# imjaegyun/super_resolution

Measured on AMD Instinct MI355X. Metric: SR output megapixels/sec, HAT-S x4, 1280x720 LR in, higher is better.
Workload: dtype bf16; 1 GPU; HAT-S x4, one 3x720x1280 LR frame per GPU, full-frame forward; upscale=4, parallelism=dp1

## Files before the change

include/hat_mi355x.h:

```cpp
#ifndef HAT_MI355X_H
#define HAT_MI355X_H

#include <stdint.h>

#ifdef __cplusplus
extern "C" {
#endif

#define HAT_ABI_VERSION 2

enum { HAT_F32 = 0, HAT_BF16 = 1 };
enum { HAT_EINVAL = -1, HAT_ELDS = -2, HAT_EUNSUPPORTED = -3 };

enum { HAT_ACT_NONE = 0, HAT_ACT_GELU = 1 , HAT_ACT_LRELU = 2 ,
       HAT_ACT_LRELU02 = 3  };
enum { HAT_X_NHWC_T = 0, HAT_X_NHWC_F32 = 1, HAT_X_NCHW_F32_MEAN = 2 };
enum { HAT_O_NHWC_T = 0, HAT_O_NHWC_F32 = 1, HAT_O_PIXSHUF_T = 2, HAT_O_NCHW_F32 = 3 };

typedef struct HatConvDesc {
    const void* x;
    const void* x0;
    const void* w;
    const float* bias;
    void* out;
// ... 21 lines not shown
    float* gap_out;
    void* n16_out;
    int32_t gap_c;
    int32_t reserved0;
} HatConvDesc;

int hat_conv_occupancy(const HatConvDesc* d, int32_t* wgs_per_cu);
int hat_conv_tiles(const HatConvDesc* d, int32_t* tiles_out);
int hat_conv_plan(const HatConvDesc* d, int32_t* waves, int32_t* rows_per_wave, int32_t* tiles, int64_t* lds_bytes);
int hat_conv(const HatConvDesc* d, void* stream);

int hat_linear(const HatConvDesc* d, void* stream);

int hat_conv3x3_small_groups(const HatConvDesc* d, int32_t* groups_out);
int hat_conv3x3_small(const HatConvDesc* d, void* stream);

typedef struct HatCabFoldDesc {
    const void* c1;
    const float* c1_colsum;
    const float* w2;
    const float* b2;
    const float* wk;
    const float* bias_in;
    float* scale;
    void* wf;
    float* bias_out;
    float* tmp;
    int32_t B, H, W, C, mid, ld1, tiles, ldcs, k, ld_scale, dtype;
    float conv_scale;
    const float* stats;
    const float* w2f;
} HatCabFoldDesc;
int hat_cab_fold(const HatCabFoldDesc* d, void* stream);

typedef struct HatAggrCabDesc {
    HatConvDesc lin;
    const void* c1;
    const void* wf;
    const float* bias_b;
} HatAggrCabDesc;
int hat_aggr_cab(const HatAggrCabDesc* d, void* stream);

int hat_layernorm_blocks(void);
int hat_layernorm(const float* x, void* y, const float* gamma, const float* beta, float* gap_partial,
                  int32_t B, int64_t npix, int32_t C, int32_t ldy, int32_t out_f32, int32_t gap_c,
                  int32_t dtype, void* stream);

int hat_add_f32(const float* a, const float* c, float* out, int32_t B, int64_t n, int64_t c_bstride, void* stream);

int hat_esc_weights(const float* gap_partial, int32_t nblk, int64_t npix, const float* w1, const float* b1,
                    const float* w2, const float* b2, const float* plk_packed, void* w_out, int32_t B,
                    int32_t pdim, int32_t ksize, int32_t Kpad, int32_t dtype, void* stream);

int hat_esc_conv13(const void* x, int32_t ldx, const void* wp, int32_t Kpad, void* y16, int32_t B, int32_t H, int32_t W,
                   int32_t dtype, void* stream);

int hat_eca_scale(const float* colsum, int32_t tiles, int32_t ldc, int64_t npix, const float* wk, int32_t k,
                  float conv_scale, float* tmp, float* scale, int32_t B, int32_t C, void* stream);

int hat_dwconv_gate(const void* u, const float* wdw, const float* bdw, void* out, int32_t B, int32_t H,
                    int32_t W, int32_t hid, int32_t ldu, int32_t ldo, int32_t dtype, void* stream);

typedef struct HatMlpDesc {
    const void* x;
    const void* w1f;
    const float* b1;
    const void* w2f;
    const float* b2;
    const float* r1;
    void* out;
    int32_t B, H, W, C, hidden;
    int32_t ldx, ldr1, ldo;
    int32_t out_f32, dtype;
} HatMlpDesc;
int hat_ocab_mlp(const HatMlpDesc* d, void* stream);
int hat_ocab_qkv(const HatMlpDesc* d, void* stream);

int hat_ocab_keybias(const void* sal, int32_t ldsal, const void* kv, int32_t ldkv, float* kb, int32_t B, int32_t H, int32_t W,
                     int32_t C, int32_t ws, int32_t wse, int32_t pad, int32_t k_keep, int32_t dtype, void* stream);
int hat_ocab_attention_kb(const void* q, const void* kv, const float* bias_rot, const float* kb, void* out, int32_t B, int32_t H,
                          int32_t W, int32_t C, int32_t heads, int32_t ws, int32_t wse, int32_t pad, int32_t ldq, int32_t ldkv,
                          int32_t ldo, int32_t dtype, void* stream);

int hat_sgfn_gate(const void* u, const float* wdw, const float* bdw, void* out, int32_t B, int32_t H, int32_t W,
                  int32_t half, int32_t ldu, int32_t ldo, int32_t dtype, void* stream);

int hat_ocab_attention(const void* q, const void* kv, const float* bias_rot, void* out, int32_t B, int32_t H,
                       int32_t W, int32_t C, int32_t heads, int32_t ws, int32_t wse, int32_t ldq,
// ... 96 lines not shown
    float* gap_out;
    int32_t B, H, W, C;
    int32_t chunks;
    int32_t ldn, gap_c;
    int32_t dtype;
    int32_t ldm_in;
    const void* m_in;
    void* n16_out;
} HatFfnDesc;

int hat_ffn_tiles(const HatFfnDesc* d, int32_t* tiles_out);
int hat_ffn(const HatFfnDesc* d, void* stream);

int hat_ffn2(const HatFfnDesc* d, void* stream);

typedef struct HatHabTailDesc {
    HatFfnDesc ffn;
    const void* n;
    const void* y16;
    const void* c1;
    const void* w_aggr;
    const void* wf;
    const float* bias_b;
    int32_t ldn_in;
    int32_t ldr2;
    const void* r2;
    const float* r2scale;
    int32_t r2scale_bstride;
    int32_t reserved1;
} HatHabTailDesc;
int hat_hab_tail(const HatHabTailDesc* d, void* stream);

int hat_hab_tail3(const HatHabTailDesc* d, void* stream);

typedef struct hat_plan hat_plan;
int hat_plan_load(const char* path, hat_plan** out);
int hat_plan_info(const hat_plan* plan, int32_t* dims8, int64_t* n_calls, int64_t* device_bytes);
int hat_plan_forward(const hat_plan* plan, const float* x, float* y, void* stream);
void hat_plan_free(hat_plan* plan);
int hat_plan_forward_u8(const hat_plan* plan, const uint8_t* src, int64_t src_pitch, int32_t h, int32_t w, uint8_t* dst,
                        int64_t dst_pitch, int32_t flags, void* stream);
int hat_plan_forward_yuv420(const hat_plan* plan, const uint8_t* src_y, int64_t src_y_pitch, int64_t src_y_bstride, const uint8_t* src_cb,
                            const uint8_t* src_cr, int64_t src_c_pitch, int32_t src_c_step, int64_t src_c_bstride, int32_t h, int32_t w,
                            uint8_t* dst_y, int64_t dst_y_pitch, int64_t dst_y_bstride, uint8_t* dst_cb, uint8_t* dst_cr, int64_t dst_c_pitch,
                            int32_t dst_c_step, int64_t dst_c_bstride, const float* to_rgb12, const float* from_rgb12, void* stream);
int hat_plan_forward_yuv420_deep(const hat_plan* plan, const void* src_y, int64_t src_y_pitch, int64_t src_y_bstride, const void* src_cb,
                                 const void* src_cr, int64_t src_c_pitch, int32_t src_c_step, int64_t src_c_bstride, int32_t src_depth,
                                 int32_t src_msb, int32_t h, int32_t w, void* dst_y, int64_t dst_y_pitch, int64_t dst_y_bstride, void* dst_cb,
                                 void* dst_cr, int64_t dst_c_pitch, int32_t dst_c_step, int64_t dst_c_bstride, int32_t dst_depth,
                                 int32_t dst_msb, const float* to_rgb12, const float* from_rgb12, void* stream);
int hat_plan_forward_yuv(const hat_plan* plan, const HatYuvSurface* src, const HatYuvSurface* dst, int32_t h, int32_t w,
                         const float* to_rgb12, const float* from_rgb12, void* stream);
int hat_plan_forward_yuv_sited(const hat_plan* plan, const HatYuvSurface* src, int32_t src_siting, const HatYuvSurface* dst,
                               int32_t dst_siting, int32_t h, int32_t w, const float* to_rgb12, const float* from_rgb12, void* stream);

int hat_rect_sum(const void* x, int32_t dtype, int32_t ld, int32_t C, int32_t W, int32_t r0, int32_t r1, int32_t c0, int32_t c1,
                 int64_t bstride, int32_t B, float* out, int32_t ldo, float* tmp, uint32_t* counter, void* stream);

int hat_dihedral_f32(const float* src, float* dst, int32_t planes, int32_t H, int32_t W, int32_t op, int32_t inverse, float alpha,
                     int32_t accumulate, void* stream);

int hat_abi_version(void);
const char* hat_target_arch(void);

int hat_niqe_workspace_bytes(int32_t B, int32_t h, int32_t w, int32_t crop_border, int32_t* H96, int32_t* W96, int64_t* bytes);
int hat_niqe_y_u8(const uint8_t* src, int64_t pitch, int64_t bstride, int32_t B, int32_t h, int32_t w, int32_t crop_border, int32_t bgr,
// ... 79 lines not shown
```

super_resolution_amd/_lib.py:

```python
from __future__ import annotations

import ctypes as C
import os
import threading

_HERE = os.path.dirname(os.path.abspath(__file__))
LIB_PATH = os.environ.get("HAT_MI355X_LIB") or os.path.join(_HERE, "libhat_mi355x.so")

ABI_VERSION = 2
HAT_F32, HAT_BF16 = 0, 1
ACT_NONE, ACT_GELU, ACT_LRELU, ACT_LRELU02 = 0, 1, 2, 3
X_NHWC_T, X_NHWC_F32, X_NCHW_F32_MEAN = 0, 1, 2
O_NHWC_T, O_NHWC_F32, O_PIXSHUF_T, O_NCHW_F32 = 0, 1, 2, 3
METRICS_Y, METRICS_BGR, METRICS_PSNR, METRICS_SSIM = 1, 2, 4, 8

_ERRORS = {-1: "HAT_EINVAL (bad argument)", -2: "HAT_ELDS (tile does not fit in 160 KiB LDS)",
           -3: "HAT_EUNSUPPORTED (shape not instantiated)"}


class HatConvDesc(C.Structure):
    _fields_ = [
        ("x", C.c_void_p), ("x0", C.c_void_p), ("w", C.c_void_p), ("bias", C.c_void_p),
        ("out", C.c_void_p), ("r1", C.c_void_p), ("r2", C.c_void_p), ("r2scale", C.c_void_p), ("colsum", C.c_void_p),
        ("B", C.c_int32), ("H", C.c_int32), ("W", C.c_int32),
# ... 21 lines not shown
        ("r1", C.c_void_p), ("out", C.c_void_p),
        ("B", C.c_int32), ("H", C.c_int32), ("W", C.c_int32), ("C", C.c_int32), ("hidden", C.c_int32),
        ("ldx", C.c_int32), ("ldr1", C.c_int32), ("ldo", C.c_int32),
        ("out_f32", C.c_int32), ("dtype", C.c_int32),
    ]


class HatFfnDesc(C.Structure):
    _fields_ = [
        ("t_in", C.c_void_p), ("t_out", C.c_void_p), ("ln_g", C.c_void_p), ("ln_b", C.c_void_p),
        ("w1f", C.c_void_p), ("b1", C.c_void_p), ("dww", C.c_void_p), ("dwb", C.c_void_p),
        ("w2f", C.c_void_p), ("b2", C.c_void_p), ("ln1_g", C.c_void_p), ("ln1_b", C.c_void_p),
        ("n_out", C.c_void_p), ("gap_out", C.c_void_p),
        ("B", C.c_int32), ("H", C.c_int32), ("W", C.c_int32), ("C", C.c_int32),
        ("chunks", C.c_int32), ("ldn", C.c_int32), ("gap_c", C.c_int32), ("dtype", C.c_int32),
        ("ldm_in", C.c_int32), ("m_in", C.c_void_p), ("n16_out", C.c_void_p),
    ]


class HatHabTailDesc(C.Structure):
    _fields_ = [("ffn", HatFfnDesc), ("n", C.c_void_p), ("y16", C.c_void_p), ("c1", C.c_void_p), ("w_aggr", C.c_void_p),
                ("wf", C.c_void_p), ("bias_b", C.c_void_p), ("ldn_in", C.c_int32), ("ldr2", C.c_int32), ("r2", C.c_void_p),
                ("r2scale", C.c_void_p), ("r2scale_bstride", C.c_int32), ("reserved1", C.c_int32)]


class HatCabFoldDesc(C.Structure):
    _fields_ = [
        ("c1", C.c_void_p), ("c1_colsum", C.c_void_p), ("w2", C.c_void_p), ("b2", C.c_void_p), ("wk", C.c_void_p),
        ("bias_in", C.c_void_p), ("scale", C.c_void_p), ("wf", C.c_void_p), ("bias_out", C.c_void_p), ("tmp", C.c_void_p),
        ("B", C.c_int32), ("H", C.c_int32), ("W", C.c_int32), ("C", C.c_int32), ("mid", C.c_int32), ("ld1", C.c_int32),
        ("tiles", C.c_int32), ("ldcs", C.c_int32), ("k", C.c_int32), ("ld_scale", C.c_int32), ("dtype", C.c_int32),
        ("conv_scale", C.c_float), ("stats", C.c_void_p), ("w2f", C.c_void_p),
    ]


class HatAggrCabDesc(C.Structure):
    _fields_ = [("lin", HatConvDesc), ("c1", C.c_void_p), ("wf", C.c_void_p), ("bias_b", C.c_void_p)]


class HatYuvSurface(C.Structure):
    _fields_ = [("y", C.c_void_p), ("y_pitch", C.c_int64), ("y_bstride", C.c_int64), ("cb", C.c_void_p), ("cr", C.c_void_p),
                ("c_pitch", C.c_int64), ("c_step", C.c_int32), ("c_bstride", C.c_int64),
                ("sub_x", C.c_int32), ("sub_y", C.c_int32), ("depth", C.c_int32), ("msb", C.c_int32)]


class HatNafHalfDesc(C.Structure):
    _fields_ = [("r_in", C.c_void_p), ("gprev", C.c_void_p), ("wf", C.c_void_p), ("bf", C.c_void_p), ("r_out", C.c_void_p),
                ("w1", C.c_void_p), ("b1", C.c_void_p), ("dww", C.c_void_p), ("dwb", C.c_void_p), ("g_out", C.c_void_p),
                ("partials", C.c_void_p), ("wf_bstride", C.c_int64), ("bf_bstride", C.c_int32),
                ("B", C.c_int32), ("H", C.c_int32), ("W", C.c_int32), ("C", C.c_int32), ("ldr", C.c_int32), ("ldg", C.c_int32),
                ("ldo", C.c_int32), ("dtype", C.c_int32), ("reserved0", C.c_int32)]


class HatNafFoldDesc(C.Structure):
    _fields_ = [("partials", C.c_void_p), ("wsca", C.c_void_p), ("bsca", C.c_void_p), ("w2", C.c_void_p), ("b2", C.c_void_p),
                ("beta", C.c_void_p), ("wf", C.c_void_p), ("bf", C.c_void_p), ("npix", C.c_int64),
                ("B", C.c_int32), ("tiles", C.c_int32), ("C", C.c_int32), ("dtype", C.c_int32)]


class HatEscConvFfnDesc(C.Structure):
    _fields_ = [("x", C.c_void_p), ("ln_g", C.c_void_p), ("ln_b", C.c_void_p), ("w1", C.c_void_p), ("b1", C.c_void_p),
                ("dww", C.c_void_p), ("dwb", C.c_void_p), ("w2", C.c_void_p), ("b2", C.c_void_p), ("r", C.c_void_p),
                ("out", C.c_void_p), ("partials", C.c_void_p), ("ln_eps", C.c_float),
                ("B", C.c_int32), ("H", C.c_int32), ("W", C.c_int32), ("hid_p", C.c_int32), ("ldx", C.c_int32), ("ldr", C.c_int32),
                ("ldo", C.c_int32), ("out_f32", C.c_int32), ("dtype", C.c_int32), ("reserved0", C.c_int32)]


_YUV_BLOCK = [C.c_void_p, C.c_int64, C.c_int64, C.c_void_p, C.c_void_p, C.c_int64, C.c_int32, C.c_int64]

SIGNATURES = {
    "hat_abi_version": (C.c_int, []),
    "hat_target_arch": (C.c_char_p, []),
    "hat_conv_tiles": (C.c_int, [C.POINTER(HatConvDesc), C.POINTER(C.c_int32)]),
    "hat_ocab_mlp": (C.c_int, [C.POINTER(HatMlpDesc), C.c_void_p]),
    "hat_ocab_qkv": (C.c_int, [C.POINTER(HatMlpDesc), C.c_void_p]),
    "hat_conv_occupancy": (C.c_int, [C.POINTER(HatConvDesc), C.POINTER(C.c_int32)]),
    "hat_conv_plan": (C.c_int, [C.POINTER(HatConvDesc), C.POINTER(C.c_int32), C.POINTER(C.c_int32), C.POINTER(C.c_int32),
                                C.POINTER(C.c_int64)]),
    "hat_conv": (C.c_int, [C.POINTER(HatConvDesc), C.c_void_p]),
    "hat_linear": (C.c_int, [C.POINTER(HatConvDesc), C.c_void_p]),
    "hat_conv3x3_small_groups": (C.c_int, [C.POINTER(HatConvDesc), C.POINTER(C.c_int32)]),
    "hat_conv3x3_small": (C.c_int, [C.POINTER(HatConvDesc), C.c_void_p]),
    "hat_cab_fold": (C.c_int, [C.POINTER(HatCabFoldDesc), C.c_void_p]),
    "hat_aggr_cab": (C.c_int, [C.POINTER(HatAggrCabDesc), C.c_void_p]),
    "hat_ffn_tiles": (C.c_int, [C.POINTER(HatFfnDesc), C.POINTER(C.c_int32)]),
    "hat_ffn": (C.c_int, [C.POINTER(HatFfnDesc), C.c_void_p]),
    "hat_ffn2": (C.c_int, [C.POINTER(HatFfnDesc), C.c_void_p]),
    "hat_hab_tail": (C.c_int, [C.POINTER(HatHabTailDesc), C.c_void_p]),
    "hat_hab_tail3": (C.c_int, [C.POINTER(HatHabTailDesc), C.c_void_p]),
    "hat_plan_load": (C.c_int, [C.c_char_p, C.POINTER(C.c_void_p)]),
    "hat_plan_info": (C.c_int, [C.c_void_p, C.POINTER(C.c_int32), C.POINTER(C.c_int64), C.POINTER(C.c_int64)]),
    "hat_plan_forward": (C.c_int, [C.c_void_p, C.c_void_p, C.c_void_p, C.c_void_p]),
    "hat_plan_free": (None, [C.c_void_p]),
    "hat_layernorm_blocks": (C.c_int, []),
    "hat_layernorm": (C.c_int, [C.c_void_p, C.c_void_p, C.c_void_p, C.c_void_p, C.c_void_p, C.c_int32, C.c_int64,
                                C.c_int32, C.c_int32, C.c_int32, C.c_int32, C.c_int32, C.c_void_p]),
    "hat_rect_sum": (C.c_int, [C.c_void_p, C.c_int32, C.c_int32, C.c_int32, C.c_int32, C.c_int32, C.c_int32, C.c_int32, C.c_int32,
                               C.c_int64, C.c_int32, C.c_void_p, C.c_int32, C.c_void_p, C.c_void_p, C.c_void_p]),
    "hat_add_f32": (C.c_int, [C.c_void_p, C.c_void_p, C.c_void_p, C.c_int32, C.c_int64, C.c_int64, C.c_void_p]),
    "hat_esc_weights": (C.c_int, [C.c_void_p, C.c_int32, C.c_int64, C.c_void_p, C.c_void_p, C.c_void_p, C.c_void_p,
                                  C.c_void_p, C.c_void_p, C.c_int32, C.c_int32, C.c_int32, C.c_int32, C.c_int32, C.c_void_p]),
    "hat_esc_conv13": (C.c_int, [C.c_void_p, C.c_int32, C.c_void_p, C.c_int32, C.c_void_p, C.c_int32, C.c_int32, C.c_int32, C.c_int32, C.c_void_p]),
    "hat_eca_scale": (C.c_int, [C.c_void_p, C.c_int32, C.c_int32, C.c_int64, C.c_void_p, C.c_int32, C.c_float,
                                C.c_void_p, C.c_void_p, C.c_int32, C.c_int32, C.c_void_p]),
    "hat_dwconv_gate": (C.c_int, [C.c_void_p, C.c_void_p, C.c_void_p, C.c_void_p, C.c_int32, C.c_int32, C.c_int32,
                                  C.c_int32, C.c_int32, C.c_int32, C.c_int32, C.c_void_p]),
    "hat_ocab_keybias": (C.c_int, [C.c_void_p, C.c_int32, C.c_void_p, C.c_int32, C.c_void_p] + [C.c_int32] * 9 + [C.c_void_p]),
    "hat_ocab_attention_kb": (C.c_int, [C.c_void_p] * 5 + [C.c_int32] * 12 + [C.c_void_p]),
    "hat_sgfn_gate": (C.c_int, [C.c_void_p, C.c_void_p, C.c_void_p, C.c_void_p, C.c_int32, C.c_int32, C.c_int32,
                                C.c_int32, C.c_int32, C.c_int32, C.c_int32, C.c_void_p]),
    "hat_ocab_attention": (C.c_int, [C.c_void_p, C.c_void_p, C.c_void_p, C.c_void_p, C.c_int32, C.c_int32, C.c_int32,
                                     C.c_int32, C.c_int32, C.c_int32, C.c_int32, C.c_int32, C.c_int32, C.c_int32,
                                     C.c_int32, C.c_void_p]),
    "hat_ocab_attention_log2": (C.c_int, [C.c_void_p, C.c_void_p, C.c_void_p, C.c_void_p, C.c_int32, C.c_int32, C.c_int32,
                                     C.c_int32, C.c_int32, C.c_int32, C.c_int32, C.c_int32, C.c_int32, C.c_int32,
                                     C.c_int32, C.c_void_p]),
    "hat_cab_squeeze_units": (C.c_int, [C.c_int32, C.c_int32, C.c_void_p, C.c_void_p]),
    "hat_cab_squeeze": (C.c_int, [C.c_void_p, C.c_void_p, C.c_void_p, C.c_void_p, C.c_void_p, C.c_int32, C.c_int32, C.c_int32,
                                  C.c_int32, C.c_int32, C.c_int32, C.c_void_p]),
    "hat_conv3x3_to_planes": (C.c_int, [C.c_void_p, C.c_void_p, C.c_void_p, C.c_void_p, C.c_int32, C.c_int32, C.c_int32, C.c_int32,
                                        C.c_int32, C.c_int32, C.c_float, C.c_void_p, C.c_int32, C.c_void_p]),
    "hat_u8_to_planes": (C.c_int, [C.c_void_p, C.c_int64, C.c_int64, C.c_void_p, C.c_int32, C.c_int32, C.c_int32, C.c_int32, C.c_int32,
# ... 103 lines not shown
```

super_resolution_amd/build.py:

```python
from __future__ import annotations

import os
import subprocess
import sys
from concurrent.futures import ThreadPoolExecutor

HERE = os.path.dirname(os.path.abspath(__file__))
CSRC = os.path.join(HERE, "csrc")
LIB = os.path.join(HERE, "libhat_mi355x.so")
SOURCES = ["hat_conv.hip", "hat_conv64r.hip", "hat_attn.hip", "hat_misc.hip", "hat_ffn.hip", "hat_ffn2.hip", "hat_tail3.hip", "hat_tail3l.hip", "hat_pw.hip", "hat_mlp.hip", "hat_cabsq.hip", "hat_esc13.hip", "hat_u8.hip", "hat_yuv.hip", "hat_resize.hip", "hat_metrics.hip", "hat_dihedral.hip", "hat_niqe.hip", "hat_naf.hip", "hat_esc.hip", "hat_escreal.hip", "hat_plan.cpp"]
HEADERS = [os.path.join(CSRC, "hat_common.h"), os.path.join(CSRC, "hat_yuv_check.h"), os.path.join(os.path.dirname(HERE), "include", "hat_mi355x.h")]
FLAGS = ["-O3", "--offload-arch=gfx950", "-fPIC", "-std=c++17", "-Wall", "-Wno-unused-function"]


def _hipcc() -> str:
    for c in (os.environ.get("HIPCC"), "/opt/rocm/bin/hipcc", "hipcc"):
        if c and (os.path.isabs(c) and os.path.exists(c) or not os.path.isabs(c)):
            return c
    raise RuntimeError("hipcc not found")


def _stale(target: str, deps) -> bool:
    if not os.path.exists(target):
        return True
    t = os.path.getmtime(target)
    return any(os.path.getmtime(d) > t for d in deps)


def build(force: bool = False, verbose: bool = True) -> str:
    hipcc = _hipcc()
    objs, jobs = [], []
    for src in SOURCES:
        s = os.path.join(CSRC, src)
        o = os.path.join(CSRC, os.path.splitext(src)[0] + ".o")
        objs.append(o)
        if force or _stale(o, [s] + HEADERS):
            jobs.append([hipcc, *FLAGS, "-c", s, "-o", o])

    def run(cmd):
        if verbose:
            print(" ".join(cmd), flush=True)
        r = subprocess.run(cmd, capture_output=True, text=True)
        if r.returncode != 0:
            raise RuntimeError(f"hipcc failed:\n{' '.join(cmd)}\n{r.stdout}\n{r.stderr}")
# ... 13 lines not shown
```

super_resolution_amd/csrc/hat_cabsq.hip:

```cpp
#include <cstdlib>
#include <type_traits>

#include "hat_common.h"
#include "hat_yuv_check.h"

__device__ __attribute__((aligned(16))) unsigned hat_cabsq_zero_page[80] = {};

namespace {

struct SweepEpi { float out_scale; float mean[4]; int nst; };
struct SweepEpiU8 { float out_scale; float mean[4]; int h_out, w_out, bgr; long long pitch, bstride; };
template <int SX, int SY, bool GREY> struct SweepEpiYUVT {
    float out_scale; float mean[4]; int h_out, w_out, c_step; long long pitch, bstride, c_pitch, c_bstride;
    uint8_t* cb; uint8_t* cr; HatCsc k;
};
template <int SX, int SY, bool GREY> struct SweepEpiYUV16T {
    float out_scale; float mean[4]; int h_out, w_out, c_step; long long pitch, bstride, c_pitch, c_bstride;
    uint8_t* cb; uint8_t* cr; HatCsc k; int shift; float scale, maxcode;
};
using SweepEpiYUV = SweepEpiYUVT<1, 1, false>;
using SweepEpiYUV16 = SweepEpiYUV16T<1, 1, false>;
template <typename E> struct SweepYuvTraits { static constexpr bool yuv = false, deep = false, grey = false; static constexpr int sx = 1, sy = 1; };
template <int SX, int SY, bool G> struct SweepYuvTraits<SweepEpiYUVT<SX, SY, G>> {
    static constexpr bool yuv = true, deep = false, grey = G; static constexpr int sx = SX, sy = SY;
};
template <int SX, int SY, bool G> struct SweepYuvTraits<SweepEpiYUV16T<SX, SY, G>> {
    static constexpr bool yuv = true, deep = true, grey = G; static constexpr int sx = SX, sy = SY;
};

template <int KS, bool NCHW, typename Epi = SweepEpi>
__global__ __launch_bounds__(256, KS > 2 ? 2 : 3) void cab_squeeze_kernel(const bf16_t* __restrict__ x, const bf16_t* __restrict__ wpk,
                                                             const float* __restrict__ bias, void* __restrict__ outv,
                                                             float* __restrict__ colsum, int H, int W, int C, int ldx,
                                                             int rows, int strips, int units, Epi epi) {
    constexpr bool U8 = std::is_same<Epi, SweepEpiU8>::value;
    using YT = SweepYuvTraits<Epi>;
    constexpr bool YUV16 = YT::deep, YUV = YT::yuv;
    constexpr bool C420 = YUV && !YT::grey && YT::sx == 1 && YT::sy == 1, C422 = YUV && !YT::grey && YT::sx == 1 && YT::sy == 0;
    constexpr bool C444 = YUV && !YT::grey && YT::sx == 0;
    static_assert((!U8 && !YUV) || NCHW, "the byte epilogues convert the conv_last value");
    using M = MT<bf16_t>;
    using frag_t = M::frag_t;
    const int lane = threadIdx.x & 63, wave = threadIdx.x >> 6, g = lane >> 4, c16 = lane & 15;
    const int u = blockIdx.x * 4 + wave;
    const int b = blockIdx.y;
    if (u >= units) return;
    const int band = u / strips, strip = u - band * strips;
    const int x0 = strip * 14 - 1, y0 = band * rows, y1 = min(y0 + rows, H);
    const bf16_t* xb = x + (size_t)b * H * W * ldx;
    bf16_t* ob = reinterpret_cast<bf16_t*>(outv) + (size_t)b * H * W * 8;
    float* of = nullptr;
    uint8_t* o8 = nullptr;
    if constexpr (U8 || YUV) o8 = reinterpret_cast<uint8_t*>(outv) + (size_t)b * epi.bstride;
    else of = reinterpret_cast<float*>(outv) + (size_t)b * epi.nst * H * W;
    [[maybe_unused]] float ctop_b = 0.f, ctop_r = 0.f;

    frag_t A[6][KS];
#pragma unroll
    for (int t = 0; t < 6; ++t)
#pragma unroll
        for (int ks = 0; ks < KS; ++ks) A[t][ks] = M::load(wpk + ((size_t)(t * KS + ks) * 64 + lane) * 8);
    const f32x4 bs = *reinterpret_cast<const f32x4*>(bias + 4 * (g & 1));

    const int xx = x0 + c16;
    const bool xin = xx >= 0 && xx < W;
    const bf16_t* cbase = xin ? xb + (size_t)xx * ldx : reinterpret_cast<const bf16_t*>(hat_cabsq_zero_page);
    const unsigned cstride = xin ? (unsigned)W * (unsigned)ldx : 0u;
// ... 107 lines not shown
                }
            } else if constexpr (NCHW) {
#pragma unroll
                for (int i = 0; i < 4; ++i)
                    if (4 * g + i < epi.nst) of[((size_t)(4 * g + i) * H + y) * W + xx] = v[i] * epi.out_scale + epi.mean[(4 * g + i) & 3];
            } else {
#pragma unroll
                for (int i = 0; i < 4; ++i) v[i] = gelu_erf_fast(v[i]);
                Vec4<bf16_t>::store(ob + ((size_t)y * W + xx) * 8 + 4 * g, v);
                csum += as_stored<bf16_t>(v);
            }
        }
        S2 = f32x4{0.f, 0.f, 0.f, 0.f};
#pragma unroll
        for (int i = 0; i < 4; ++i) S0[i] = g < 2 ? S0[i] : 0.f;
    };

#pragma unroll
    for (int nb = 0; nb < NB; ++nb) load_row(y0 - 1 + nb, Bc[nb]);
    for (int r = y0 - 1; r <= y1; r += 3) {
        step(r, ring[1], ring[2], ring[0], Bc[0]);
        step(r + 1, ring[2], ring[0], ring[1], Bc[1]);
        step(r + 2, ring[0], ring[1], ring[2], Bc[2]);
    }
    if (!NCHW && colsum != nullptr) {
#pragma unroll
        for (int i = 0; i < 4; ++i) {
            const float s = row_sum16(csum[i]);
            if (c16 == 0) colsum[((size_t)b * units + u) * 16 + 4 * g + i] = g < 2 ? s : 0.f;
        }
    }
}

}

static int sweep_units(int H, int W, int slots, int* rows_out, int* units_out, bool even_rows = false) {
    const int strips = (W + 13) / 14;
    int bands = slots / strips;
    bands = bands < 1 ? 1 : bands;
    int rows = (H + bands - 1) / bands;
    rows = rows < 8 ? 8 : rows;
    if (even_rows) rows += rows & 1;
    *rows_out = rows;
    *units_out = strips * ((H + rows - 1) / rows);
    return 0;
}

extern "C" int hat_cab_squeeze_units(int32_t H, int32_t W, int32_t* rows_out, int32_t* units_out) {
    if (H < 1 || W < 16 || W % 16 || !rows_out || !units_out) return HAT_EINVAL;
    static const int slots = [] { const char* e = getenv("HAT_SQUEEZE_SLOTS"); const int v = e ? atoi(e) : 0; return v >= 256 ? v : 2048; }();
    return sweep_units(H, W, slots, rows_out, units_out);
}

extern "C" int hat_cab_squeeze(const void* x, const void* wpk, const float* bias, void* out, float* colsum, int32_t B,
                               int32_t H, int32_t W, int32_t C, int32_t ldx, int32_t dtype, void* stream) {
    if (!x || !wpk || !bias || !out || B < 1 || H < 1) return HAT_EINVAL;
    if (dtype != HAT_BF16) return HAT_EUNSUPPORTED;
    if (C % 8 || C > 160 || C <= 128 || ldx < C || ldx % 8) return HAT_EUNSUPPORTED;
    if ((reinterpret_cast<uintptr_t>(x) | reinterpret_cast<uintptr_t>(wpk)) % 16 || reinterpret_cast<uintptr_t>(out) % 8) return HAT_EINVAL;
    int32_t rows = 0, units = 0;
    const int rc = hat_cab_squeeze_units(H, W, &rows, &units);
    if (rc) return rc;
    HAT_LAUNCH((cab_squeeze_kernel<5, false>), dim3((units + 3) / 4, B), dim3(256), 0, reinterpret_cast<hipStream_t>(stream),
               reinterpret_cast<const bf16_t*>(x), reinterpret_cast<const bf16_t*>(wpk), bias, out, colsum, H, W, C, ldx, rows,
               (W + 13) / 14, units, SweepEpi{1.0f, {0.f, 0.f, 0.f, 0.f}, 8});
    return hat_check_launch();
}

extern "C" int hat_conv3x3_to_planes(const void* x, const void* wpk, const float* bias, float* out, int32_t B, int32_t H,
                                     int32_t W, int32_t C, int32_t ldx, int32_t n_out, float out_scale, const float* mean4,
                                     int32_t dtype, void* stream) {
    if (!x || !wpk || !bias || !out || !mean4 || B < 1 || H < 1 || W < 16 || W % 16 || n_out < 1 || n_out > 8) return HAT_EINVAL;
    if (dtype != HAT_BF16) return HAT_EUNSUPPORTED;
    if (C != 64 || ldx < C || ldx % 8) return HAT_EUNSUPPORTED;
    if ((reinterpret_cast<uintptr_t>(x) | reinterpret_cast<uintptr_t>(wpk)) % 16) return HAT_EINVAL;
    int rows = 0, units = 0;
    sweep_units(H, W, 3072, &rows, &units);
    HAT_LAUNCH((cab_squeeze_kernel<2, true>), dim3((units + 3) / 4, B), dim3(256), 0, reinterpret_cast<hipStream_t>(stream),
               reinterpret_cast<const bf16_t*>(x), reinterpret_cast<const bf16_t*>(wpk), bias, out, nullptr, H, W, C, ldx, rows,
               (W + 13) / 14, units, SweepEpi{out_scale, {mean4[0], mean4[1], mean4[2], mean4[3]}, n_out});
    return hat_check_launch();
}

extern "C" int hat_conv3x3_to_u8(const void* x, const void* wpk, const float* bias, uint8_t* dst, int64_t dst_pitch, int64_t dst_bstride,
                                 int32_t B, int32_t H, int32_t W, int32_t C, int32_t ldx, int32_t h_out, int32_t w_out, float out_scale,
                                 const float* mean4, int32_t bgr, int32_t dtype, void* stream) {
    if (!x || !wpk || !bias || !dst || !mean4 || B < 1 || H < 1 || W < 16 || W % 16 || h_out < 1 || w_out < 1 || h_out > H || w_out > W)
        return HAT_EINVAL;
    if (dst_pitch < 3 * (int64_t)w_out || (B > 1 && dst_bstride < dst_pitch * (int64_t)(h_out - 1) + 3 * (int64_t)w_out)) return HAT_EINVAL;
    if (dtype != HAT_BF16) return HAT_EUNSUPPORTED;
    if (C != 64 || ldx < C || ldx % 8) return HAT_EUNSUPPORTED;
    if ((reinterpret_cast<uintptr_t>(x) | reinterpret_cast<uintptr_t>(wpk)) % 16) return HAT_EINVAL;
    int rows = 0, units = 0;
    sweep_units(H, W, 3072, &rows, &units);
    HAT_LAUNCH((cab_squeeze_kernel<2, true, SweepEpiU8>), dim3((units + 3) / 4, B), dim3(256), 0, reinterpret_cast<hipStream_t>(stream),
               reinterpret_cast<const bf16_t*>(x), reinterpret_cast<const bf16_t*>(wpk), bias, dst, nullptr, H, W, C, ldx, rows, (W + 13) / 14, units,
               SweepEpiU8{out_scale, {mean4[0], mean4[1], mean4[2], mean4[3]}, h_out, w_out, bgr ? 1 : 0, (long long)dst_pitch,
                          (long long)dst_bstride});
// ... 80 lines not shown
```

super_resolution_amd/csrc/hat_esc13.hip:

```cpp
#include <cstdlib>

#include "hat_common.h"

namespace {

constexpr int E_TR = 32, E_TC = 32, E_HALO = 6;
constexpr int E_HR = E_TR + 2 * E_HALO, E_HC = E_TC + 2 * E_HALO;
constexpr int E_NFRAG = 7 * 13;
constexpr int E_X_OFF = E_NFRAG * 1024;
constexpr int E_LDS = E_X_OFF + E_HR * E_HC * 32 + 64;

__device__ __attribute__((aligned(16))) unsigned hat_esc13_zero_page[4] = {0, 0, 0, 0};

template <int RW>
__global__ __launch_bounds__((E_TR / RW) * 64) void esc13_kernel(const bf16_t* __restrict__ x, int ldx, const bf16_t* __restrict__ wp, int Kpad,
                                                             bf16_t* __restrict__ y16, int H, int W, int tiles_x, int ntiles) {
    typedef __bf16 bf8 __attribute__((ext_vector_type(8)));
    constexpr int E_WAVES = E_TR / RW;
    extern __shared__ __attribute__((aligned(16))) char smem[];
    typedef __attribute__((address_space(3))) char lds_char;
    const unsigned lds0 = (unsigned)(uintptr_t)(lds_char*)smem;
    const int tid = threadIdx.x, lane = tid & 63, g = lane >> 4, c16 = lane & 15;
    const int wave = __builtin_amdgcn_readfirstlane(tid >> 6);
    const int b = blockIdx.y;
    const bf16_t* xb = x + (size_t)b * H * W * ldx;
    bf16_t* yb = y16 + (size_t)b * H * W * 16;
    {
        const bf16_t* wrow = wp + ((size_t)b * 16 + c16) * Kpad;
        for (int s = wave; s < E_NFRAG; s += E_WAVES) {
            const int dxp = s / 13, dy = s - 13 * dxp, dx = 2 * dxp + (g >> 1);
            const char* src = dx <= 12 ? reinterpret_cast<const char*>(wrow + (dy * 13 + dx) * 16 + 8 * (g & 1))
                                       : reinterpret_cast<const char*>(hat_esc13_zero_page);
            __builtin_amdgcn_global_load_lds((const __attribute__((address_space(1))) void*)src,
                                             (__attribute__((address_space(3))) void*)(smem + s * 1024), 16, 0, 0);
        }
        if (tid < 4) *reinterpret_cast<u32x4*>(smem + E_LDS - 64 + tid * 16) = u32x4{0u, 0u, 0u, 0u};
    }
    const int r0 = RW * wave;
    unsigned xbase = lds0 + E_X_OFF + (unsigned)((r0 * E_HC + c16 + (g >> 1)) * 32 + (g & 1) * 16);
    unsigned abase = lds0 + (unsigned)lane * 16u, abase1 = abase + 60u * 1024u;
    asm volatile("" : "+v"(xbase), "+v"(abase), "+v"(abase1));

    constexpr int NPIECE = E_HR * E_HC * 2, NIT = (NPIECE + E_WAVES * 64 - 1) / (E_WAVES * 64);
    u32x4 pv[NIT];
    auto fetch = [&](int t) {
        const int tc = min(t, ntiles - 1);
        const int ty0 = (tc / tiles_x) * E_TR, tx0 = (tc - (tc / tiles_x) * tiles_x) * E_TC;
#pragma unroll
        for (int it = 0; it < NIT; ++it) {
            const int i = min(tid + it * E_WAVES * 64, NPIECE - 1);
            const int hp = i >> 1, half = i & 1;
            const int hy = hp / E_HC, hx = hp - hy * E_HC;
            const int y = ty0 - E_HALO + hy, xx = tx0 - E_HALO + hx;
            const bool in = y >= 0 && y < H && xx >= 0 && xx < W;
            const u32x4 v = *reinterpret_cast<const u32x4*>(xb + ((size_t)min(max(y, 0), H - 1) * W + min(max(xx, 0), W - 1)) * ldx + half * 8);
            pv[it] = in ? v : u32x4{0u, 0u, 0u, 0u};
        }
    };
    fetch(blockIdx.x);
    for (int t = blockIdx.x; t < ntiles; t += gridDim.x) {
        const int ty0 = (t / tiles_x) * E_TR, tx0 = (t - (t / tiles_x) * tiles_x) * E_TC;
#pragma unroll
        for (int it = 0; it < NIT; ++it) {
            const int i = tid + it * E_WAVES * 64;
            if (i < NPIECE) *reinterpret_cast<u32x4*>(smem + E_X_OFF + i * 16) = pv[it];
        }
        __syncthreads();
        fetch(t + gridDim.x);

        f32x4 acc[RW][2];
#pragma unroll
        for (int pt = 0; pt < RW; ++pt)
#pragma unroll
            for (int ct = 0; ct < 2; ++ct) acc[pt][ct] = f32x4{0.f, 0.f, 0.f, 0.f};
        auto ldb = [&](int rr, int dxp, int ct) {
            return __builtin_bit_cast(bf8, *(__attribute__((address_space(3))) const u32x4*)(uintptr_t)(xbase + (unsigned)((rr * E_HC) * 32 + dxp * 64 + ct * 512)));
        };
        auto lda = [&](int dxp, int dy) {
            const int sfr = dxp * 13 + dy;
            return __builtin_bit_cast(bf8, *(__attribute__((address_space(3))) const u32x4*)(uintptr_t)(sfr < 60 ? abase + (unsigned)(sfr * 1024) : abase1 + (unsigned)((sfr - 60) * 1024)));
        };
        bf8 rowf[7][RW + 12][2];
        bf8 afr[7][13];
        constexpr int PRE = RW < 2 ? RW : 2;
        afr[0][0] = lda(0, 0);
#pragma unroll
        for (int j = 0; j < PRE; ++j) { rowf[0][j][0] = ldb(j, 0, 0); rowf[0][j][1] = ldb(j, 0, 1); }
#pragma unroll
        for (int dxp = 0; dxp < 7; ++dxp) {
#pragma unroll
            for (int dy = 0; dy < 13; ++dy) {
                if (dy == 0) {
#pragma unroll
                    for (int j = PRE; j < RW; ++j) { rowf[dxp][j][0] = ldb(j, dxp, 0); rowf[dxp][j][1] = ldb(j, dxp, 1); }
                }
                if (dy < 12) {
                    afr[dxp][dy + 1] = lda(dxp, dy + 1);
                    rowf[dxp][dy + RW][0] = ldb(dy + RW, dxp, 0);
                    rowf[dxp][dy + RW][1] = ldb(dy + RW, dxp, 1);
                } else if (dxp < 6) {
                    afr[dxp + 1][0] = lda(dxp + 1, 0);
#pragma unroll
                    for (int j = 0; j < PRE; ++j) { rowf[dxp + 1][j][0] = ldb(j, dxp + 1, 0); rowf[dxp + 1][j][1] = ldb(j, dxp + 1, 1); }
                }
#pragma unroll
                for (int j = 0; j < RW; ++j)
#pragma unroll
                    for (int ct = 0; ct < 2; ++ct)
                        acc[j][ct] = __builtin_amdgcn_mfma_f32_16x16x32_bf16(afr[dxp][dy], rowf[dxp][dy + j][ct], acc[j][ct], 0, 0, 0);
                __builtin_amdgcn_sched_barrier(0);
            }
        }
#pragma unroll
        for (int pt = 0; pt < RW; ++pt)
#pragma unroll
            for (int ct = 0; ct < 2; ++ct) {
                const int y = ty0 + r0 + pt, xx = tx0 + ct * 16 + c16;
                if (y < H && xx < W) Vec4<bf16_t>::store(yb + ((size_t)y * W + xx) * 16 + 4 * g, acc[pt][ct]);
            }
        __syncthreads();
    }
}

}

extern "C" int hat_esc_conv13(const void* x, int32_t ldx, const void* wp, int32_t Kpad, void* y16, int32_t B, int32_t H, int32_t W,
                              int32_t dtype, void* stream) {
    if (!x || !wp || !y16 || B < 1 || H < 1 || W < 1 || ldx < 16 || ldx % 8 || Kpad < 169 * 16 || Kpad % 8) return HAT_EINVAL;
    if (dtype != HAT_BF16) return HAT_EUNSUPPORTED;
    const int tiles_x = (W + E_TC - 1) / E_TC, tiles_y = (H + E_TR - 1) / E_TR, ntiles = tiles_x * tiles_y;
    int gx = 256 / (B < 2 ? 1 : (B < 4 ? 2 : 4));
    if (gx > ntiles) gx = ntiles;
    static const int rw = [] { const char* e = getenv("HAT_ESC13_RW"); return e && atoi(e) == 2 ? 2 : 4; }();
    auto launch = [&](auto kern, int waves) -> int {
        hipError_t e = hipFuncSetAttribute(reinterpret_cast<const void*>(kern), hipFuncAttributeMaxDynamicSharedMemorySize, E_LDS);
        if (e != hipSuccess) return (int)e;
        HAT_LAUNCH(kern, dim3(gx, B), dim3(waves * 64), E_LDS, reinterpret_cast<hipStream_t>(stream), reinterpret_cast<const bf16_t*>(x), ldx,
                   reinterpret_cast<const bf16_t*>(wp), Kpad, reinterpret_cast<bf16_t*>(y16), H, W, tiles_x, ntiles);
        return hat_check_launch();
    };
    return rw == 2 ? launch(esc13_kernel<2>, 16) : launch(esc13_kernel<4>, 8);
}
```

super_resolution_amd/csrc/hat_misc.hip:

```cpp
#include "hat_common.h"

namespace {

constexpr int LN_BLOCKS = 1024;

template <typename OutT, int NV>
__global__ __launch_bounds__(256) void ln_kernel(const float* __restrict__ x, OutT* __restrict__ y,
                                                 const float* __restrict__ gamma, const float* __restrict__ beta,
                                                 float* __restrict__ gap_partial, long npix, int C, int ldy, int gap_c) {
    __shared__ float red[16][32];
    const int tid = threadIdx.x, j = tid & 15, grp = tid >> 4;
    const int b = blockIdx.y;
    const float* xb = x + (size_t)b * npix * C;
    OutT* yb = y + (size_t)b * npix * ldy;
    f32x4 gm[NV], bt[NV];
#pragma unroll
    for (int v = 0; v < NV; ++v) {
        const int c = 4 * j + 64 * v;
        gm[v] = f32x4{0.f, 0.f, 0.f, 0.f};
        bt[v] = gm[v];
        if (c < C) {
            gm[v] = *reinterpret_cast<const f32x4*>(gamma + c);
            bt[v] = *reinterpret_cast<const f32x4*>(beta + c);
        }
    }
    f32x4 gsum = {0.f, 0.f, 0.f, 0.f};
    const float invC = 1.0f / (float)C;
    for (long p0 = (long)blockIdx.x * 16; p0 < npix; p0 += (long)gridDim.x * 16) {
        const long p = p0 + grp;
        const bool pv = p < npix;
        f32x4 xv[NV];
        float s = 0.f;
#pragma unroll
// ... 102 lines not shown
        for (int k = 0; k < np; ++k) s += part[k * gs + tid];
        pmean[tid] = s * inv_npix;
    }
    __syncthreads();
    const int hdim = pdim / 2;
    if (tid < hdim) {
        float s = b1[tid];
        for (int ci = 0; ci < pdim; ++ci) s += w1[tid * pdim + ci] * pmean[ci];
        hid[tid] = gelu_erf(s);
    }
    __syncthreads();
    if (tid < 9) {
        const int t = co * 9 + tid;
        float s = b2[t];
        for (int m = 0; m < hdim; ++m) s += w2[t * hdim + m] * hid[m];
        dk[tid] = s;
    }
    __syncthreads();
    const int cin_p = (pdim + 7) & ~7;
    const int ctr = ksize / 2;
    const float* src = plk + (size_t)co * Kpad;
    T* dst = w_out + ((size_t)b * npad + co) * Kpad;
    for (int k = tid; k < Kpad; k += 1024) {
        float v = src[k];
        const int tap = k / cin_p, ci = k - tap * cin_p;
        if (ci == co && tap < ksize * ksize) {
            const int dy = tap / ksize - ctr, dx = tap % ksize - ctr;
            if (dy >= -1 && dy <= 1 && dx >= -1 && dx <= 1) v += dk[(dy + 1) * 3 + (dx + 1)];
        }
        dst[k] = to_T<T>(v);
    }
}

__global__ __launch_bounds__(256) void eca_reduce_kernel(const float* __restrict__ colsum, int tiles, int ldc,
                                                         float* __restrict__ tmp) {
    __shared__ float sub[256];
    int lw = 1;
    while (lw < ldc) lw <<= 1;
    const int nsub = 256 / lw;
    const int c = threadIdx.x % lw, sb = threadIdx.x / lw, part = blockIdx.x, b = blockIdx.y;
    const int per = (tiles + 31) / 32;
    const int t0 = part * per, t1 = min(tiles, t0 + per);
    float a[8] = {0.f, 0.f, 0.f, 0.f, 0.f, 0.f, 0.f, 0.f};
    if (c < ldc && t1 > t0) {
        for (int t = t0 + sb; t < t1; t += 8 * nsub) {
#pragma unroll
            for (int u = 0; u < 8; ++u) {
                const int tt = t + u * nsub;
                const float v = colsum[((size_t)b * tiles + min(tt, t1 - 1)) * ldc + c];
                a[u] += tt < t1 ? v : 0.f;
            }
        }
    }
    sub[threadIdx.x] = ((a[0] + a[1]) + (a[2] + a[3])) + ((a[4] + a[5]) + (a[6] + a[7]));
    __syncthreads();
    if (sb == 0 && c < ldc) {
        float s = 0.f;
        for (int i = 0; i < nsub; ++i) s += sub[i * lw + c];
        tmp[((size_t)b * 32 + part) * ldc + c] = s;
    }
}

__global__ __launch_bounds__(256) void eca_scale_kernel(const float* __restrict__ tmp, int ldc, float inv_npix,
                                                        const float* __restrict__ wk, int k, float conv_scale,
                                                        float* __restrict__ scale, int C) {
    __shared__ float mean[256];
    const int c = threadIdx.x, b = blockIdx.x;
    float s = 0.f;
    if (c < C) {
        for (int p = 0; p < 32; ++p) s += tmp[((size_t)b * 32 + p) * ldc + c];
    }
    mean[c] = s * inv_npix;
    __syncthreads();
    if (c < C) {
        float e = 0.f;
        for (int j = 0; j < k; ++j) {
            const int cc = c + j - k / 2;
            if (cc >= 0 && cc < C) e += wk[j] * mean[cc];
        }
        scale[(size_t)b * ldc + c] = conv_scale / (1.0f + expf(-e));
    }
}

template <typename T, bool DIRECT>
__global__ __launch_bounds__(256) void cab_fold_kernel(const HatCabFoldDesc d) {
    __shared__ float sm[256 * 5 + 256];
    float* red = sm;
    float (*part)[32] = reinterpret_cast<float (*)[32]>(sm + 256 * 5);
    float* mean = sm;
    float* scl = sm + 256;
    __shared__ float bord[4][8];
    __shared__ float S[9][8];
    const int tid = threadIdx.x, b = blockIdx.x;
    const int H = d.H, W = d.W, C = d.C, mid = d.mid;
    const T* c1 = reinterpret_cast<const T*>(d.c1) + (size_t)b * H * W * d.ld1;
    const float* st = d.stats ? d.stats + (size_t)b * 72 : nullptr;
    if (st != nullptr) {
        if (tid < 32) bord[tid >> 3][tid & 7] = st[8 + tid];
        __syncthreads();
    } else {
        float a[4][8];
#pragma unroll
        for (int line = 0; line < 4; ++line)
#pragma unroll
            for (int c = 0; c < 8; ++c) a[line][c] = 0.f;
        const int lmax = W > H ? W : H;
        constexpr int BU = sizeof(T) == 2 ? 5 : 2;
        for (int i0 = tid; i0 < lmax; i0 += 256 * BU) {
            typename MT<T>::frag_t v[BU][4];
#pragma unroll
            for (int u = 0; u < BU; ++u)
#pragma unroll
                for (int line = 0; line < 4; ++line) {
                    const int len = line < 2 ? W : H;
                    const int i = min(i0 + u * 256, len - 1);
                    const size_t pix = line == 0 ? (size_t)i : line == 1 ? (size_t)(H - 1) * W + i : line == 2 ? (size_t)i * W : (size_t)i * W + (W - 1);
                    v[u][line] = MT<T>::load(c1 + pix * d.ld1);
                }
#pragma unroll
            for (int u = 0; u < BU; ++u)
#pragma unroll
                for (int line = 0; line < 4; ++line) {
                    const bool in = i0 + u * 256 < (line < 2 ? W : H);
#pragma unroll
                    for (int c = 0; c < 8; ++c) a[line][c] += in ? to_f(v[u][line][c]) : 0.f;
                }
        }
#pragma unroll
        for (int pass = 0; pass < 8; ++pass) {
#pragma unroll
            for (int k = 0; k < 4; ++k) red[tid * 5 + k] = a[pass >> 1][(pass & 1) * 4 + k];
            __syncthreads();
            if (tid < 32) {
                const int v4 = tid & 3, pt = tid >> 2;
                float sp = 0.f;
                for (int i = 0; i < 32; ++i) sp += red[(pt * 32 + i) * 5 + v4];
                part[pt][pass * 4 + v4] = sp;
            }
            __syncthreads();
        }
        if (tid < 32) {
            float sp = 0.f;
            for (int i = 0; i < 8; ++i) sp += part[i][tid];
            bord[tid >> 3][tid & 7] = sp;
        }
        __syncthreads();
    }
    if (DIRECT && st == nullptr) {
        const int c = tid & 7, sb = tid >> 3;
        float a[8] = {0.f, 0.f, 0.f, 0.f, 0.f, 0.f, 0.f, 0.f};
        for (int t = sb; t < d.tiles; t += 256) {
#pragma unroll
            for (int u = 0; u < 8; ++u) {
                const int tt = t + 32 * u;
                const float v = d.c1_colsum[((size_t)b * d.tiles + min(tt, d.tiles - 1)) * d.ldcs + c];
                a[u] += tt < d.tiles ? v : 0.f;
            }
        }
        part[c][sb] = ((a[0] + a[1]) + (a[2] + a[3])) + ((a[4] + a[5]) + (a[6] + a[7]));
        __syncthreads();
    }
    if (tid < 72) {
        const int tap = tid >> 3, c = tid & 7;
        const int dy = tap / 3 - 1, dx = tap % 3 - 1;
        float tot = 0.f;
        if (st != nullptr) {
            tot = st[c];
        } else if constexpr (DIRECT) {
            for (int p = 0; p < 32; ++p) tot += part[c][p];
        } else {
            for (int p = 0; p < 32; ++p) tot += d.tmp[((size_t)b * 32 + p) * d.ldcs + c];
        }
        float v = tot;
        const int rl = dy == 1 ? 0 : dy == -1 ? 1 : -1, cl = dx == 1 ? 2 : dx == -1 ? 3 : -1;
        if (rl >= 0) v -= bord[rl][c];
        if (cl >= 0) v -= bord[cl][c];
        if (rl >= 0 && cl >= 0) {
            const size_t pix = (size_t)(rl == 0 ? 0 : H - 1) * W + (cl == 2 ? 0 : W - 1);
            v += st != nullptr ? st[40 + (rl * 2 + (cl - 2)) * 8 + c] : to_f(c1[pix * d.ld1 + c]);
        }
        S[tap][c] = c < mid ? v : 0.f;
    }
    __syncthreads();
    float m = 0.f;
    {
        const int co = tid < C ? tid : C - 1;
        float wv[72];
        if (d.w2f != nullptr) {
            const f32x4* wf4 = reinterpret_cast<const f32x4*>(d.w2f) + (size_t)(co >> 4) * (3 * 64 * 2);
            f32x4 w8[9][2];
#pragma unroll
            for (int tap = 0; tap < 9; ++tap) {
                const int e = ((tap >> 2) * 64 + (tap & 3) * 16 + (co & 15)) * 2;
                w8[tap][0] = wf4[e];
                w8[tap][1] = wf4[e + 1];
            }
#pragma unroll
            for (int q = 0; q < 72; ++q) { const int ci = q / 9, tap = q - ci * 9; wv[q] = w8[tap][ci >> 2][ci & 3]; }
        } else {
#pragma unroll
            for (int q = 0; q < 72; ++q) wv[q] = d.w2[(size_t)co * mid * 9 + min(q, mid * 9 - 1)];
        }
        const float bb = d.b2[co];
#pragma unroll
        for (int q = 0; q < 72; ++q) {
            const int ci = q / 9, tap = q - ci * 9;
            if (q < mid * 9) m += wv[q] * S[tap][ci < 8 ? ci : 7];
        }
        m = tid < C ? m / ((float)H * (float)W) + bb : 0.f;
    }
    mean[tid] = m;
    __syncthreads();
    float sc = 0.f;
    if (tid < C) {
        float e = 0.f;
        for (int j = 0; j < d.k; ++j) {
            const int cc = tid + j - d.k / 2;
            if (cc >= 0 && cc < C) e += d.wk[j] * mean[cc];
        }
        sc = d.conv_scale / (1.0f + expf(-e));
        d.scale[(size_t)b * d.ld_scale + tid] = sc;
    }
    scl[tid] = sc;
    __syncthreads();
    const int nt = (C + 15) / 16;
    for (int n = tid; n < nt * 16; n += 256) d.bias_out[(size_t)b * nt * 16 + n] = n < C ? d.bias_in[n] + scl[n] * d.b2[n] : 0.f;
    T* wf = reinterpret_cast<T*>(d.wf) + (size_t)b * nt * 3 * 512;
    if (d.w2f != nullptr) {
        constexpr int MAXS = 16;
        const int total4 = nt * 3 * 128;
        for (int base = 0; base < total4; base += 256 * MAXS) {
        f32x4 wq[MAXS];
#pragma unroll
        for (int st = 0; st < MAXS; ++st) wq[st] = reinterpret_cast<const f32x4*>(d.w2f)[min(base + tid + st * 256, total4 - 1)];
#pragma unroll
        for (int st = 0; st < MAXS; ++st) {
            const int i4 = base + tid + st * 256;
            if (i4 < total4) {
                const int i = 4 * i4, j = i & 7, lane = (i >> 3) & 63, ks = (i >> 9) % 3, t = i / (3 * 512);
                const int co = t * 16 + (lane & 15), tap = 4 * ks + (lane >> 4);
                const int cov = min(co, C - 1);
                const float sv = scl[cov];
                f32x4 v = wq[st] * f32x4{sv, sv, sv, sv};
                if (co < C && tap == 9 && j == 0) {
                    const float bfull = d.bias_in[cov] + sv * d.b2[cov];
                    v[0] = bfull;
                    v[1] = bfull - to_f(to_T<T>(bfull));
                }
                Vec4<T>::store(wf + i, v);
            }
        }
        }
        return;
    }
    constexpr int FU = 18;
    for (int i0 = tid; i0 < nt * 3 * 512; i0 += 256 * FU) {
        float wv[FU], bi[FU], b2v[FU];
        bool ok[FU];
        int cov[FU], bsel[FU];
#pragma unroll
        for (int u = 0; u < FU; ++u) {
            const int i = min(i0 + u * 256, nt * 3 * 512 - 1);
            const int j = i & 7, lane = (i >> 3) & 63, ks = (i >> 9) % 3, t = i / (3 * 512);
            const int co = t * 16 + (lane & 15), k = 32 * ks + 8 * (lane >> 4) + j;
            const int tap = k >> 3, ci = k & 7;
            ok[u] = co < C && tap < 9 && ci < mid;
            bsel[u] = (co < C && tap == 9 && ci < 2) ? 1 + ci : 0;
            cov[u] = min(co, C - 1);
            wv[u] = d.w2[((size_t)cov[u] * mid + min(ci, mid - 1)) * 9 + min(tap, 8)];
            bi[u] = d.bias_in[cov[u]];
            b2v[u] = d.b2[cov[u]];
        }
#pragma unroll
        for (int u = 0; u < FU; ++u) {
            const int i = i0 + u * 256;
            const float bfull = bi[u] + scl[cov[u]] * b2v[u];
            const float bhead = to_f(to_T<T>(bfull));
            const float v = bsel[u] == 1 ? bfull : (bsel[u] == 2 ? bfull - bhead : (ok[u] ? scl[cov[u]] * wv[u] : 0.f));
            if (i < nt * 3 * 512) wf[i] = to_T<T>(v);
        }
    }
}

template <typename T>
__global__ __launch_bounds__(256) void dwgate_kernel(const T* __restrict__ u, const float* __restrict__ wdw,
                                                     const float* __restrict__ bdw, T* __restrict__ out, int B, int H, int W,
                                                     int hid, int ldu, int ldo) {
    const int gpp = hid / 4;
    const size_t total = (size_t)B * H * W * gpp;
    for (size_t i = (size_t)blockIdx.x * 256 + threadIdx.x; i < total; i += (size_t)gridDim.x * 256) {
        const size_t pix = i / gpp;
        const int c = (int)(i - pix * gpp) * 4;
        const int x = (int)(pix % W);
        const int y = (int)((pix / W) % H);
        f32x4 a = *reinterpret_cast<const f32x4*>(bdw + c);
        f32x4 gt = *reinterpret_cast<const f32x4*>(bdw + hid + c);
#pragma unroll
        for (int dy = -1; dy <= 1; ++dy) {
            const int yy = y + dy;
            if (yy < 0 || yy >= H) continue;
#pragma unroll
            for (int dx = -1; dx <= 1; ++dx) {
                const int xx = x + dx;
                if (xx < 0 || xx >= W) continue;
                const T* up = u + (size_t)((long)pix + (long)dy * W + dx) * ldu;
                const int tap = (dy + 1) * 3 + (dx + 1);
                a += Vec4<T>::load(up + c) * *reinterpret_cast<const f32x4*>(wdw + (size_t)tap * 2 * hid + c);
                gt += Vec4<T>::load(up + hid + c) * *reinterpret_cast<const f32x4*>(wdw + (size_t)tap * 2 * hid + hid + c);
            }
        }
        f32x4 o;
#pragma unroll
        for (int r = 0; r < 4; ++r) o[r] = a[r] * (gt[r] / (1.0f + expf(-gt[r])));
        Vec4<T>::store(out + pix * ldo + c, o);
    }
// ... 34 lines not shown

}

extern "C" int hat_layernorm_blocks(void) { return LN_BLOCKS; }

extern "C" int hat_layernorm(const float* x, void* y, const float* gamma, const float* beta, float* gap_partial,
                             int32_t B, int64_t npix, int32_t C, int32_t ldy, int32_t out_f32, int32_t gap_c,
                             int32_t dtype, void* stream) {
    if (!x || !y || !gamma || !beta || B < 1 || npix < 1 || C < 4 || C % 4 || C > 256 || ldy < C || ldy % 4) return HAT_EINVAL;
    if (gap_c < 0 || gap_c > 32 || gap_c % 4 || (gap_c > 0 && !gap_partial)) return HAT_EINVAL;
    hipStream_t s = reinterpret_cast<hipStream_t>(stream);
    float* gp = gap_c > 0 ? gap_partial : nullptr;
    if (out_f32 || dtype == HAT_F32) return launch_ln<float>(x, y, gamma, beta, gp, B, npix, C, ldy, gap_c, s);
    if (dtype == HAT_BF16) return launch_ln<bf16_t>(x, y, gamma, beta, gp, B, npix, C, ldy, gap_c, s);
    return HAT_EINVAL;
}

extern "C" int hat_esc_weights(const float* gap_partial, int32_t nblk, int64_t npix, const float* w1, const float* b1,
                               const float* w2, const float* b2, const float* plk_packed, void* w_out, int32_t B,
                               int32_t pdim, int32_t ksize, int32_t Kpad, int32_t dtype, void* stream) {
    if (!gap_partial || !w1 || !b1 || !w2 || !b2 || !plk_packed || !w_out) return HAT_EINVAL;
    if (pdim < 2 || pdim > 32 || pdim % 4 || ksize < 3 || (ksize & 1) == 0 || B < 1 || nblk < 1) return HAT_EINVAL;
    hipStream_t s = reinterpret_cast<hipStream_t>(stream);
    dim3 grid(pdim > 16 ? 32 : 16, B), block(1024);
    const float inv = 1.0f / (float)npix;
    if (dtype == HAT_BF16)
        HAT_LAUNCH(esc_weights_kernel<bf16_t>, grid, block, 0, s, gap_partial, nblk, inv, w1, b1, w2, b2, plk_packed,
                           reinterpret_cast<bf16_t*>(w_out), pdim, ksize, Kpad);
    else if (dtype == HAT_F32)
        HAT_LAUNCH(esc_weights_kernel<float>, grid, block, 0, s, gap_partial, nblk, inv, w1, b1, w2, b2, plk_packed,
                           reinterpret_cast<float*>(w_out), pdim, ksize, Kpad);
    else
        return HAT_EINVAL;
    return hat_check_launch();
}

extern "C" int hat_eca_scale(const float* colsum, int32_t tiles, int32_t ldc, int64_t npix, const float* wk, int32_t k,
                             float conv_scale, float* tmp, float* scale, int32_t B, int32_t C, void* stream) {
    if (!colsum || !wk || !tmp || !scale || tiles < 1 || ldc < C || ldc > 256 || C < 1 || k < 1 || (k & 1) == 0 || B < 1) return HAT_EINVAL;
    hipStream_t s = reinterpret_cast<hipStream_t>(stream);
    HAT_LAUNCH(eca_reduce_kernel, dim3(32, B), dim3(256), 0, s, colsum, tiles, ldc, tmp);
    int rc = hat_check_launch();
    if (rc) return rc;
    HAT_LAUNCH(eca_scale_kernel, dim3(B), dim3(256), 0, s, tmp, ldc, 1.0f / (float)npix, wk, k, conv_scale, scale, C);
    return hat_check_launch();
}

extern "C" int hat_cab_fold(const HatCabFoldDesc* dp, void* stream) {
    if (!dp) return HAT_EINVAL;
    const HatCabFoldDesc& d = *dp;
    if (!d.w2 || !d.b2 || !d.wk || !d.bias_in || !d.scale || !d.wf || !d.bias_out) return HAT_EINVAL;
    if (!d.stats && (!d.c1 || !d.c1_colsum || !d.tmp)) return HAT_EINVAL;
    if (d.B < 1 || d.H < 2 || d.W < 2 || d.C < 1 || d.C > 256 || d.mid < 1 || d.mid > 8 || d.ld1 != 8 || d.tiles < 1 || d.ldcs < 8 ||
        d.ldcs > 256 || d.k < 1 || (d.k & 1) == 0 || d.ld_scale < d.C)
        return HAT_EINVAL;
    hipStream_t s = reinterpret_cast<hipStream_t>(stream);
    if (d.dtype != HAT_BF16 && d.dtype != HAT_F32) return HAT_EINVAL;
    if (d.tiles <= 2048 || d.stats) {
        if (d.dtype == HAT_BF16) HAT_LAUNCH((cab_fold_kernel<bf16_t, true>), dim3(d.B), dim3(256), 0, s, d);
        else HAT_LAUNCH((cab_fold_kernel<float, true>), dim3(d.B), dim3(256), 0, s, d);
        return hat_check_launch();
    }
    HAT_LAUNCH(eca_reduce_kernel, dim3(32, d.B), dim3(256), 0, s, d.c1_colsum, d.tiles, d.ldcs, d.tmp);
    int rc = hat_check_launch();
    if (rc) return rc;
    if (d.dtype == HAT_BF16) HAT_LAUNCH((cab_fold_kernel<bf16_t, false>), dim3(d.B), dim3(256), 0, s, d);
// ... 130 lines not shown
```

super_resolution_amd/csrc/hat_plan.cpp:

```cpp
#include <hip/hip_runtime.h>
#include <stdint.h>
#include <stdio.h>
#include <string.h>

#include <string>
#include <vector>

#include "../../include/hat_mi355x.h"
#include "hat_yuv_check.h"

namespace {

enum : uint32_t { ARG_INT = 0, ARG_FLOAT = 1, ARG_PTR = 2, ARG_STRUCT = 3, ARG_HOST = 4, ARG_STREAM = 5 };
enum : uint32_t { BUF_CONST = 0, BUF_SCRATCH = 1, BUF_INPUT = 2, BUF_OUTPUT = 3 };
constexpr uint32_t NULL_BUF = 0xFFFFFFFFu;

struct Fix { uint32_t field_off, buf; uint64_t off; };
struct Arg {
    uint32_t tag = 0;
    int64_t i = 0;
    double f = 0;
    uint32_t buf = NULL_BUF;
    uint64_t off = 0;
    std::vector<unsigned char> blob;
    std::vector<Fix> fix;
};
struct Call { uint32_t fn; std::vector<Arg> args; };
struct Buf { uint32_t kind; uint64_t nbytes; void* dev = nullptr; };

}

struct hat_plan {
    int32_t dims[8];
    std::vector<Buf> bufs;
    std::vector<Call> calls;
    int device = -1;
    mutable float* stage_in = nullptr;
    mutable float* stage_out = nullptr;
};

namespace {

struct Reader {
    FILE* f;
    bool ok = true;
    template <typename T> T get() { T v{}; if (fread(&v, sizeof(T), 1, f) != 1) ok = false; return v; }
    void bytes(void* p, size_t n) { if (n && fread(p, 1, n, f) != n) ok = false; }
};

const char* const FN_NAMES[] = {"hat_conv", "hat_linear", "hat_conv3x3_small", "hat_cab_fold", "hat_aggr_cab", "hat_ffn", "hat_ffn2",
                                "hat_hab_tail", "hat_layernorm", "hat_esc_weights", "hat_eca_scale", "hat_dwconv_gate", "hat_sgfn_gate",
                                "hat_ocab_attention", "hat_window_attention", "hat_cab_squeeze", "hat_conv3x3_to_planes", "hat_add_f32", "hat_esc_conv13", "hat_ocab_keybias", "hat_ocab_attention_kb", "hat_ocab_mlp", "hat_ocab_qkv", "hat_hab_tail3", "hat_ocab_attention_log2", "hat_naf_half",
                                "hat_naf_fold"};
constexpr uint32_t N_FN = sizeof(FN_NAMES) / sizeof(FN_NAMES[0]);

struct Resolved {
    const hat_plan* p;
    const Call* c;
    const void* x;
    void* y;
    void* stream;
    std::vector<std::vector<unsigned char>> tmp;
    void* ptr(uint32_t buf, uint64_t off) const {
        if (buf == NULL_BUF) return nullptr;
        const Buf& b = p->bufs[buf];
        char* base = b.kind == BUF_INPUT ? (char*)const_cast<void*>(x) : (b.kind == BUF_OUTPUT ? (char*)y : (char*)b.dev);
        return base + off;
    }
    int32_t I(size_t k) const { return (int32_t)c->args[k].i; }
    int64_t L(size_t k) const { return c->args[k].i; }
    float F(size_t k) const { return (float)c->args[k].f; }
    void* P(size_t k) {
        const Arg& a = c->args[k];
        if (a.tag == ARG_PTR) return ptr(a.buf, a.off);
        if (a.tag == ARG_STREAM) return stream;
        if (a.tag == ARG_STRUCT || a.tag == ARG_HOST) {
            tmp.emplace_back(a.blob);
            for (const Fix& fx : a.fix) {
                void* v = ptr(fx.buf, fx.off);
                memcpy(tmp.back().data() + fx.field_off, &v, sizeof(void*));
            }
            return tmp.back().data();
        }
        return nullptr;
    }
};
// ... 34 lines not shown
                                                r.I(11), r.I(12), r.I(13), r.I(14), r.P(15))
                           : HAT_EINVAL;
        case 14:
            return n == 16 ? hat_window_attention(r.P(0), r.P(1), (const float*)r.P(2), r.P(3), r.I(4), r.I(5), r.I(6), r.I(7), r.I(8), r.I(9), r.I(10),
                                                  r.I(11), r.I(12), r.I(13), r.I(14), r.P(15))
                           : HAT_EINVAL;
        case 15:
            return n == 12 ? hat_cab_squeeze(r.P(0), r.P(1), (const float*)r.P(2), r.P(3), (float*)r.P(4), r.I(5), r.I(6), r.I(7), r.I(8), r.I(9), r.I(10),
                                             r.P(11))
                           : HAT_EINVAL;
        case 16:
            return n == 14 ? hat_conv3x3_to_planes(r.P(0), r.P(1), (const float*)r.P(2), (float*)r.P(3), r.I(4), r.I(5), r.I(6), r.I(7), r.I(8), r.I(9),
                                                   r.F(10), (const float*)r.P(11), r.I(12), r.P(13))
                           : HAT_EINVAL;
        case 17: return n == 7 ? hat_add_f32((const float*)r.P(0), (const float*)r.P(1), (float*)r.P(2), r.I(3), r.L(4), r.L(5), r.P(6)) : HAT_EINVAL;
        case 18: return n == 10 ? hat_esc_conv13(r.P(0), r.I(1), r.P(2), r.I(3), r.P(4), r.I(5), r.I(6), r.I(7), r.I(8), r.P(9)) : HAT_EINVAL;
        case 19:
            return n == 15 ? hat_ocab_keybias(r.P(0), r.I(1), r.P(2), r.I(3), (float*)r.P(4), r.I(5), r.I(6), r.I(7), r.I(8), r.I(9), r.I(10), r.I(11), r.I(12),
                                              r.I(13), r.P(14))
                           : HAT_EINVAL;
        case 20:
            return n == 18 ? hat_ocab_attention_kb(r.P(0), r.P(1), (const float*)r.P(2), (const float*)r.P(3), r.P(4), r.I(5), r.I(6), r.I(7), r.I(8), r.I(9),
                                                   r.I(10), r.I(11), r.I(12), r.I(13), r.I(14), r.I(15), r.I(16), r.P(17))
                           : HAT_EINVAL;
        case 21: return n == 2 ? hat_ocab_mlp((const HatMlpDesc*)r.P(0), r.P(1)) : HAT_EINVAL;
        case 22: return n == 2 ? hat_ocab_qkv((const HatMlpDesc*)r.P(0), r.P(1)) : HAT_EINVAL;
        case 23: return n == 2 ? hat_hab_tail3((const HatHabTailDesc*)r.P(0), r.P(1)) : HAT_EINVAL;
        case 24:
            return n == 16 ? hat_ocab_attention_log2(r.P(0), r.P(1), (const float*)r.P(2), r.P(3), r.I(4), r.I(5), r.I(6), r.I(7), r.I(8), r.I(9), r.I(10),
                                                     r.I(11), r.I(12), r.I(13), r.I(14), r.P(15))
                           : HAT_EINVAL;
        case 25: return n == 2 ? hat_naf_half((const HatNafHalfDesc*)r.P(0), r.P(1)) : HAT_EINVAL;
        case 26: return n == 2 ? hat_naf_fold((const HatNafFoldDesc*)r.P(0), r.P(1)) : HAT_EINVAL;
        default: return HAT_EUNSUPPORTED;
    }
}

}

extern "C" void hat_plan_free(hat_plan* p) {
    if (!p) return;
    for (Buf& b : p->bufs)
        if (b.dev) (void)hipFree(b.dev);
    if (p->stage_in) (void)hipFree(p->stage_in);
    if (p->stage_out) (void)hipFree(p->stage_out);
    delete p;
}

static int plan_load_impl(const char* path, hat_plan** out);

extern "C" int hat_plan_load(const char* path, hat_plan** out) {
    if (!path || !out) return HAT_EINVAL;
    *out = nullptr;
    try {
        return plan_load_impl(path, out);
    } catch (...) {
        return HAT_EINVAL;
    }
}

namespace {
constexpr uint64_t MAX_BUF_BYTES = 1ull << 38;
bool ptr_ok(const std::vector<Buf>& bufs, uint32_t buf, uint64_t off) {
    if (buf == NULL_BUF) return true;
    return buf < bufs.size() && off <= bufs[buf].nbytes;
}
// ... 251 lines not shown
```

super_resolution_amd/csrc/hat_tail3.hip:

```cpp
#include "hat_common.h"

#ifndef T3_ISSUE_ALL
#define T3_ISSUE_ALL 0
#endif
#ifndef T3_APF
#define T3_APF 1
#endif
#ifndef T3_S0RD
#define T3_S0RD 8
#endif
#ifndef T3_ABL
#define T3_ABL 0
#endif
#ifndef T3_USTORE_IL
#define T3_USTORE_IL 1
#endif
#ifndef T3_DMA_LATE
#define T3_DMA_LATE 0
#endif

namespace {

typedef _Float16 h2 __attribute__((ext_vector_type(2)));
typedef _Float16 h8 __attribute__((ext_vector_type(8)));
typedef __bf16 bf8 __attribute__((ext_vector_type(8)));

constexpr int T3_C = 144, T3_NT = 9, T3_KS = 5, T3_WAVES = 4, T3_ROWS = 8, T3_HW = 18;
constexpr int T3_NPH = (T3_ROWS + 2) * T3_HW;
constexpr int T3_US_ROWB = 160;
constexpr int T3_W1_OFF = T3_NPH * T3_US_ROWB;
constexpr int T3_W1_BYTES = 4 * T3_KS * 1024;
constexpr int T3_W2_OFF = T3_W1_OFF + 2 * T3_W1_BYTES;
constexpr int T3_WD_OFF = T3_W2_OFF + T3_NT * 1024;
constexpr int T3_WD_REC = 2048;
constexpr int T3_LDS = T3_WD_OFF + T3_WD_REC;
constexpr int T3_B2_OFF = 73728;

typedef __attribute__((address_space(3))) char lds_char;

__device__ __forceinline__ u32x4 lds_rd16(unsigned addr) { return *(__attribute__((address_space(3))) const u32x4*)(uintptr_t)addr; }
__device__ __forceinline__ h2 as_h2(unsigned v) { return __builtin_bit_cast(h2, v); }
__device__ __forceinline__ unsigned as_u(h2 v) { return __builtin_bit_cast(unsigned, v); }
__device__ __forceinline__ void dma1k(const char* src, unsigned lane_off, char* dst) {
    __builtin_amdgcn_global_load_lds((const __attribute__((address_space(1))) void*)(src + lane_off),
                                     (__attribute__((address_space(3))) void*)dst, 16, 0, 0);
}

struct T3Aggr {
    const bf16_t* n;
    const bf16_t* y16;
    const bf16_t* c1;
    const char* wl;
    const char* wf;
    const float* bias_b;
    int ldn;
};
__device__ __attribute__((aligned(16))) unsigned hat_tail3_zero_page[4] = {0, 0, 0, 0};
__device__ __attribute__((aligned(16))) unsigned hat_tail3_ones_page[4] = {0x3F803F80u, 0, 0, 0};

template <int DBG, int TH = 0>
__global__ __launch_bounds__(256, 2) void tail3_kernel(const HatFfnDesc d, const T3Aggr ag) {
    constexpr int C = T3_C, NT = T3_NT, KS = T3_KS, NPH = T3_NPH, HALO_W = T3_HW;
    extern __shared__ __attribute__((aligned(16))) char smem[];
    const unsigned lds0 = (unsigned)(uintptr_t)(lds_char*)smem;

    const int tid = threadIdx.x, lane = tid & 63, g = lane >> 4, c16 = lane & 15;
    const int wave = __builtin_amdgcn_readfirstlane(tid >> 6);
    const int b = blockIdx.z, x0 = blockIdx.x * 16, y0 = blockIdx.y * T3_ROWS;
    const int H = d.H, W = d.W;
    const float* tin = d.t_in + (size_t)b * H * W * C;
    const _Float16* tinh = reinterpret_cast<const _Float16*>(d.t_in) + (size_t)b * H * W * C;

    long long tph[12] = {0, 0, 0, 0, 0, 0, 0, 0, 0, 0, 0, 0};
    long long tlast = 0;
    auto stamp = [&](int slot) {
        if constexpr (DBG & 64) {
            const long long now = (long long)__builtin_amdgcn_s_memtime();
            tph[slot] += now - tlast;
            tlast = now;
        }
    };
    if constexpr (DBG & 64) tlast = (long long)__builtin_amdgcn_s_memtime();

    const char* w1g = reinterpret_cast<const char*>(d.w1f);
    const char* w2g = reinterpret_cast<const char*>(d.w2f);
    const char* wdg = reinterpret_cast<const char*>(d.dww);
    const unsigned lane16 = (unsigned)lane * 16u;
    auto dma_fc1 = [&](int chunk, int buf) {
#pragma unroll
        for (int j = 0; j < 5; ++j) {
            const int f = wave * 5 + j;
            dma1k(w1g + ((size_t)chunk * T3_W1_BYTES + f * 1024), lane16, smem + T3_W1_OFF + buf * T3_W1_BYTES + f * 1024);
        }
    };
// ... 356 lines not shown
#pragma unroll
                    for (int nt = 2; nt + 1 < NT; nt += 2) store_pair_bf16_if(nout, nt * 16, g, lnv(nt), lnv(nt + 1), valid);
                    if (valid) Vec4<bf16_t>::store(nout + (NT - 1) * 16 + 4 * g, lnv(NT - 1));
                } else if (valid) {
                    Vec4<bf16_t>::store(nout + 4 * g, o0);
#pragma unroll
                    for (int nt = 1; nt < NT; ++nt) Vec4<bf16_t>::store(nout + nt * 16 + 4 * g, lnv(nt));
                }
            }
        }
    }
    if constexpr (DBG & 64) {
        stamp(7);
        if (lane == 0) {
            const size_t wg = ((size_t)blockIdx.z * gridDim.y + blockIdx.y) * gridDim.x + blockIdx.x;
            for (int i = 0; i < 12; ++i) d.gap_out[(wg * T3_WAVES + wave) * 12 + i] = (float)tph[i];
        }
        return;
    }
    if (do_ln && d.gap_out != nullptr) {
        float* red = reinterpret_cast<float*>(smem + T3_WD_OFF);
#pragma unroll
        for (int r = 0; r < 4; ++r) {
            float s = gapv[r];
            s = row_sum16(s);
            if (c16 == 0) red[wave * 16 + 4 * g + r] = s;
        }
        __syncthreads();
        if (tid < 16) {
            float s = 0.f;
#pragma unroll
            for (int w = 0; w < T3_WAVES; ++w) s += red[w * 16 + tid];
            const size_t tile = (size_t)blockIdx.y * gridDim.x + blockIdx.x;
            d.gap_out[((size_t)b * gridDim.x * gridDim.y + tile) * 16 + tid] = tid < d.gap_c ? s : 0.f;
        }
    }
}

}

#ifndef HAT_TAIL3_NO_ENTRY
int hat_tail3_launch_c180(const HatHabTailDesc& h, void* stream);

extern "C" int hat_hab_tail3(const HatHabTailDesc* dp, void* stream) {
    if (!dp) return HAT_EINVAL;
    const HatHabTailDesc& h = *dp;
    const HatFfnDesc& d = h.ffn;
    if (!d.t_in || !d.t_out || d.t_in == d.t_out || !d.w1f || !d.dww || !d.w2f || !d.b2) return HAT_EINVAL;
    if (d.B < 1 || d.H < 1 || d.W < 1 || d.chunks < 1 || d.m_in) return HAT_EINVAL;
    if (d.dtype != HAT_BF16) return HAT_EUNSUPPORTED;
    if (d.C == 180) return (d.chunks == 12 && h.reserved1 == 0) ? hat_tail3_launch_c180(h, stream) : HAT_EINVAL;
    if (d.C != T3_C) return HAT_EUNSUPPORTED;
    if (d.ln1_g && (!d.ln1_b || !d.n_out || d.ldn < d.C || d.ldn % 4 || d.gap_c < 0 || d.gap_c > 16 || d.gap_c % 4)) return HAT_EINVAL;
    if (!h.n || !h.y16 || !h.c1 || !h.w_aggr || !h.wf || !h.bias_b || h.ldn_in < T3_C || h.ldn_in % 8) return HAT_EINVAL;
    const T3Aggr ag{reinterpret_cast<const bf16_t*>(h.n), reinterpret_cast<const bf16_t*>(h.y16), reinterpret_cast<const bf16_t*>(h.c1),
                    reinterpret_cast<const char*>(h.w_aggr), reinterpret_cast<const char*>(h.wf), h.bias_b, h.ldn_in};
    const int th = h.reserved1 & 3;
    if ((h.reserved1 & ~3) != 0) return HAT_EINVAL;
    if ((th & 1) && reinterpret_cast<uintptr_t>(d.t_in) % 8) return HAT_EINVAL;
    if ((th & 2) && reinterpret_cast<uintptr_t>(d.t_out) % 16) return HAT_EINVAL;
    void (*kern)(const HatFfnDesc, const T3Aggr) = th == 0 ? tail3_kernel<0, 0> : th == 1 ? tail3_kernel<0, 1> : th == 2 ? tail3_kernel<0, 2> : tail3_kernel<0, 3>;
    hipError_t e = hipFuncSetAttribute(reinterpret_cast<const void*>(kern), hipFuncAttributeMaxDynamicSharedMemorySize, T3_LDS);
    if (e != hipSuccess) return (int)e;
    dim3 grid((d.W + 15) / 16, (d.H + T3_ROWS - 1) / T3_ROWS, d.B);
    HAT_LAUNCH(kern, grid, dim3(256), T3_LDS, reinterpret_cast<hipStream_t>(stream), d, ag);
    return hat_check_launch();
}
#endif
```

super_resolution_amd/engine.py:

```python
from __future__ import annotations

import collections
import dataclasses
import math
import os
import threading
from typing import Dict, Optional

import torch

from . import ops
from .ops import (ACT_GELU, ACT_LRELU, ACT_NONE, O_NCHW_F32, O_NHWC_F32, O_NHWC_T, O_PIXSHUF_T, X_NCHW_F32_MEAN, X_NHWC_F32, X_NHWC_T)

RGB_MEAN = (0.4488, 0.4371, 0.4040)


def _r8(x: int) -> int:
    return (x + 7) // 8 * 8


def _r4(x: int) -> int:
    return (x + 3) // 4 * 4


@dataclasses.dataclass(frozen=True)
class Options:
    no_n16: bool = False
    no_t16: bool = False
    emu_t16: Optional[torch.dtype] = None
    no_fused_ffn: bool = False
    ffn_v1: bool = False
    no_hab_tail: bool = False
    tail_v2: bool = False
    no_cab_fold: bool = False
    no_cab_sweep: bool = False
    no_esc13: bool = False
    esc_side: bool = False
    one_stream: bool = False
    no_attn_log2: bool = False
    no_ocab_mlp: bool = False
    no_ocab_qkv: bool = False
    no_bf16_conv_in: bool = False
    no_conv_ln: bool = False

    @classmethod
    def from_env(cls, env=None) -> "Options":
        env = os.environ if env is None else env
        get = lambda name: env.get("HAT_" + name.upper(), "")
        any_value = ("no_cab_fold", "no_cab_sweep", "no_ocab_mlp", "no_ocab_qkv", "no_bf16_conv_in", "no_conv_ln")
        kw = {k.name: (get(k.name) != "" if k.name in any_value else get(k.name) == "1") for k in dataclasses.fields(cls)}
        return cls(**dict(kw, emu_t16={"fp16": torch.float16, "bf16": torch.bfloat16}.get(get("emu_t16"))))


class _ESC:

    def __init__(self, sd, core: str, plk_key: str, pdim: int, ksize: int, C: int, dtype: int, dev):
        f32 = dict(dtype=torch.float32, device=dev)
        self.pdim, self.ksize = pdim, ksize
        self.w1 = sd[core + ".plk.dwc_proj.1.weight"].detach().reshape(pdim // 2, pdim).to(**f32).contiguous()
        self.b1 = sd[core + ".plk.dwc_proj.1.bias"].detach().to(**f32).contiguous()
        self.w2 = sd[core + ".plk.dwc_proj.3.weight"].detach().reshape(pdim * 9, pdim // 2).to(**f32).contiguous()
        self.b2 = sd[core + ".plk.dwc_proj.3.bias"].detach().to(**f32).contiguous()
        lk = ops.pack_conv_weight(sd[plk_key], None, ops.HAT_F32, dev, nt=1)
        kc = ops.KC[dtype] * 3
        self.kpad = -(-(ksize * ksize * _r8(pdim)) // kc) * kc
        self.npad = 16 if pdim <= 16 else 32
        plk = torch.zeros(self.npad, self.kpad, **f32)
        plk[:lk.w.shape[0], :min(self.kpad, lk.kpad)] = lk.w[:self.npad, :min(self.kpad, lk.kpad)]
        self.plk = plk.contiguous()
        self.zero_bias = torch.zeros(self.npad, **f32)
        self.aggr = None
        self.aggr_keys = (core + ".aggr.weight", core + ".aggr.bias")
        self.conv13 = False


class _Packed:

    def __getitem__(self, key):
        try:
            return getattr(self, key)
        except AttributeError:
            raise KeyError(key) from None


class _Hab(_Packed):
    fold = ffn = ffn3 = fc1 = fc2 = bias256 = None
    tail = "aggr"
    next_ln = None
    out16 = False


class _Ocab(_Packed):
    qkvf = mlpf = esc = fh0 = fh2 = None


class _Naf(_Packed):

    def __init__(self, c, head, blocks, tail):
        self.c, self.head, self.blocks, self.tail = c, head, blocks, tail


class _Group(_Packed):
    to_conv = ocab16 = out16 = False
    conv_ln = None

    def __init__(self, heads, habs, ocab, conv):
        self.heads, self.habs, self.ocab, self.conv = heads, habs, ocab, conv


class _Fwd:

    def __init__(self, eng, w, B, H, W, band, one_stream):
        self.B, self.H, self.W, self.N = B, H, W, H * W
        self.C, self.dt, self.ldc = eng.C, eng.dtype, _r8(eng.C)
        self.geo = dict(B=B, H=H, W=W, dtype=eng.dtype)
        self.w, self.band, self.one_stream = w, band, one_stream
        self.t = self.gin = w["tA"]
        self.have_n = self.have_n16 = False
        self.nblk = ops.layernorm_blocks()

    def ln(self, src, dst, gb, out_f32=False, gap_c=0):
        ops.layernorm(src, dst, gb[0], gb[1], B=self.B, npix=self.N, C_=self.C, ldy=(self.C if out_f32 else self.ldc),
                      out_f32=out_f32, dtype=self.dt, gap=(self.w["gap"] if gap_c else None), gap_c=gap_c)

    def pooled(self, src, ld, C_, dst, off=0, r0=None, r1=None, c0=0, c1=None):
        bd, w = self.band, self.w
        ops.rect_sum(src, dst, w["rs_tmp"], w["rs_cnt"], B=self.B, W=self.W, ld=ld, C_=C_, r0=(bd.lo if r0 is None else r0),
                     r1=(bd.lo + bd.own if r1 is None else r1), c0=c0, c1=c1, out_off=off)

    def gstat(self, esc):
        gs = 32 if esc.pdim > 16 else 16
        return tuple(self.w[k].view(-1)[:self.B * gs].view(self.B, gs) for k in ("gstat_l", "gstat_g"))


class _Sink:
    kind = band_refusal = None
    fusable = True

    def __init__(self, eng, out, size):
        self.eng, self.out, self.size = eng, out, size

    def _count(self, how):
        name = f"{self.kind}_{how}_calls"
        setattr(self.eng, name, getattr(self.eng, name) + 1)


class _U8Sink(_Sink):
    kind, band_refusal = "u8", "a row band hands its rows over as fp32: the 8-bit output is the unsharded forward's"

    def __init__(self, eng, out, bgr):
        super().__init__(eng, out, tuple(out.shape[1:3]))
# ... 55 lines not shown
        self._lock = threading.Lock()
        self._s1 = None
        ops._lib.load()
        self.hatx = cfg.get("variant", "hat") == "hatx"
        self.topk = float(cfg.get("kv_topk_ratio", 1.0)) if self.hatx else 1.0
        self.focus = bool(cfg.get("use_focus_bias", False)) if self.hatx else False
        self.fuse_ffn = not self.hatx and ops.ffn_supported(self.C) and not self.opt.no_fused_ffn
        self._pack(state_dict)
        self._resolve()

    def _lin(self, sd, wkey, bkey, scale=1.0):
        w = sd[wkey]
        b = sd.get(bkey) if bkey else None
        o, i = w.shape[0], w.reshape(w.shape[0], -1).shape[1]

        pack = lambda wm, bias: ops.pack_pointwise(wm, bias, self.dtype, self.dev, scale=scale)
        w2 = w.reshape(o, -1)
        if w2.shape[1] == i and i > 512 and i % 16 == 0 and not ops.linear_supported(o, i, self.dtype):
            h1, h2 = pack(w2[:, :i // 2].contiguous(), b), pack(w2[:, i // 2:].contiguous(), None)
            h1.ksplit = h2
            return h1
        return pack(w, b)

    def _c3(self, sd, wkey, bkey):
        w = sd[wkey]
        if w.shape[0] > 16 and ops.conv3x3_small_supported(w.shape[0], w.shape[1], self.dtype):
            return ops.pack_linear_weight(w, sd[bkey], self.dtype, self.dev)
        return ops.pack_conv_weight(w, sd[bkey], self.dtype, self.dev)

    def _esc(self, sd, core, plk_key, pdim, ksize):
        esc = _ESC(sd, core, plk_key, pdim, ksize, self.C, self.dtype, self.dev)
        esc.aggr = self._lin(sd, *esc.aggr_keys)
        esc.conv13 = ops.esc_conv13_supported(pdim, ksize, self.dtype) and not self.opt.no_esc13
        return esc

    def _run_lin(self, pw, x, out, **kw):
        h2 = getattr(pw, "ksplit", None)
        if h2 is not None:
            if kw.get("out_mode") != O_NHWC_F32 or kw.get("act", ACT_NONE) != ACT_NONE:
                raise NotImplementedError("a K-split linear accumulates through its fp32 output")
            (ops.linear if pw.frag else ops.conv)(pw, x, out, **kw)
            (ops.linear if h2.frag else ops.conv)(h2, x.reshape(-1)[pw.cin:], out, **dict(kw, r1=out, ldr1=kw["ldo"]))
            return
        (ops.linear if pw.frag else ops.conv)(pw, x, out, **kw)

    def _pack(self, sd):
        cfg, dev = self.cfg, self.dev
        f32 = dict(dtype=torch.float32, device=dev)
        P = lambda w, b=None, **kw: ops.pack_conv_weight(sd[w], None if b is None else sd[b], self.dtype, dev, **kw)
        vec = lambda k: sd[k].detach().to(**f32).contiguous()
        self.naf = self._pack_naf(sd) if cfg.get("naf") else None
        self.conv_first = P("conv_first.weight", "conv_first.bias")
        self.pe_norm = (vec("patch_embed.norm.weight"), vec("patch_embed.norm.bias")) if cfg.get("patch_norm", True) else None
        self.ape = vec("absolute_pos_embed").reshape(-1) if cfg.get("ape", False) else None
        self.layers = []
        for g, (depth, heads) in enumerate(zip(cfg["depths"], cfg["num_heads"])):
            habs = [self._pack_hab(sd, f"layers.{g}.residual_group.blocks.{i}") for i in range(depth)]
            ocab = self._pack_ocab(sd, f"layers.{g}.residual_group.overlap_attn", heads)
            self.layers.append(_Group(heads, habs, ocab, None if self.identity else P(f"layers.{g}.conv.weight", f"layers.{g}.conv.bias")))
        self.norm = (vec("norm.weight"), vec("norm.bias"))
        self.conv_after_body = None if self.identity else P("conv_after_body.weight", "conv_after_body.bias")
        self.conv_before_up = P("conv_before_upsample.0.weight", "conv_before_upsample.0.bias")
        self.ups = []
        s = self.scale
        if s & (s - 1) == 0:
            for i in range(int(math.log2(s))):
# ... 89 lines not shown
        if ops.ocab_mlp_supported(C, sd[p + ".mlp.0.weight"].shape[0], dt) and _r8(C) == C and not self.opt.no_ocab_mlp:
            oc.mlpf = ops.pack_ocab_mlp(sd[p + ".mlp.0.weight"], sd[p + ".mlp.0.bias"], sd[p + ".mlp.2.weight"], sd[p + ".mlp.2.bias"], dev)
        oc.bias_rot = table[rot].t().contiguous().to(dev)
        oc.qlog2 = qlog2
        if C == 144 and dt == ops.HAT_BF16 and not cfg.get("ocab_esc_enable", False) and not self.opt.no_ocab_qkv:
            oc.qkvf = ops.pack_ocab_qkv(sd[p + ".q_proj.weight"], sd.get(p + ".q_proj.bias"), sd[p + ".kv_proj.weight"],
                                        sd.get(p + ".kv_proj.bias"), qscale, dev)
        if cfg.get("ocab_esc_enable", False):
            oc.esc = self._esc(sd, p + ".esc_core", p + ".esc_plk", cfg["ocab_esc_pdim"], cfg["ocab_esc_kernel"])
        if self.focus:
            oc.fh0 = ops.pack_conv_weight(sd[p + ".focus_head.0.weight"], sd[p + ".focus_head.0.bias"], dt, dev)
            oc.fh2 = ops.pack_conv_weight(sd[p + ".focus_head.2.weight"], sd[p + ".focus_head.2.bias"], dt, dev)
        return oc

    def _pack_ps(self, sd, key, r):
        w = sd[key + ".weight"]
        o = w.shape[0]
        cps = o // (r * r)
        n = torch.arange(o)
        perm = (n % cps) * (r * r) + n // cps
        return ops.pack_conv_weight(w, sd[key + ".bias"], self.dtype, self.dev, out_perm=perm)

    def _resolve(self):
        layers, dt, C = self.layers, self.dtype, self.C
        escs = [hb.esc for G in layers for hb in G.habs] + [G.ocab.esc for G in layers if G.ocab.esc is not None]
        wide = any(e.npad > 16 for e in escs)
        for gi, G in enumerate(layers):
            oc = G.ocab
            for i, hb in enumerate(G.habs):
                nh = G.habs[i + 1] if i + 1 < len(G.habs) else None
                hb.next_ln = (nh.n1, nh.esc.pdim) if nh is not None else (oc.n1, oc.esc.pdim if oc.esc is not None else 0)
                if hb.fold is not None:
                    hb.tail = "fused144" if hb.tail144_ok and not wide else "aggr_cab"
                else:
                    hb.tail = "fused180" if hb.tail180_ok and hb.next_ln[1] <= 16 else "aggr"
            G.to_conv = bool(G.conv is not None and dt == ops.HAT_BF16 and _r8(C) == C and oc.mlp2.frag and not self.opt.no_bf16_conv_in)
            cv = G.conv
            if cv is not None and dt == ops.HAT_BF16 and not self.opt.no_conv_ln and cv.n_slices == 1 and cv.nout == cv.nt * 16:
                if gi + 1 < len(layers):
                    nhs = layers[gi + 1].habs
                    nxt, gap_c = (nhs[0].n1, nhs[0].esc.pdim) if nhs else (None, 0)
                else:
                    nxt, gap_c = (self.norm, 0) if self.conv_after_body is not None else (None, 0)
                G.conv_ln = (nxt, gap_c) if nxt is not None and gap_c in (0, 4, 8, 12, 16) else None
        self._resolve_stream16()
        self.u8_fused = self.conv_last_sweep is not None and self.conv_last_sweep[2] == 3
        hab0 = layers[0].habs[0] if layers and layers[0].habs else None
        self._hab0 = hab0
        self._yw = max([16] + [e.npad for e in escs])
        self._kpad = max([hab0.esc.kpad if hab0 else 0] + [G.ocab.esc.kpad for G in layers if G.ocab.esc is not None])

    def _resolve_stream16(self):
        if not self.t16:
            return
        layers = self.layers
        tail16 = lambda hb: hb.tail == "fused144" and hb.ffn3 is not None and hb.ffn3.C == 144
        conv16 = lambda G: bool(G.conv is not None and not G.conv.frag and G.conv.ksize > 1 and G.conv.nt == 9
                                and G.conv.n_slices == 1 and G.conv.nout == 144)
        for G in layers:
            oc = G.ocab
            G.ocab16 = bool(G.habs and tail16(G.habs[-1]) and G.to_conv and oc.mlpf is not None and oc.proj.frag
                            and oc.proj.nt == 9 and getattr(oc.proj, "ksplit", None) is None and oc.esc is None)
            for i, hb in enumerate(G.habs):
                hb.out16 = tail16(hb) and (G.ocab16 if i + 1 == len(G.habs) else tail16(G.habs[i + 1]))
        for gi, G in enumerate(layers):
            if not conv16(G) or G.conv_ln is None:
# ... 16 lines not shown
        hid2 = 2 * int(C * self.cfg["mlp_ratio"])
        z = lambda *shape, dtype=T: torch.zeros(*shape, dtype=dtype, device=dev)
        f = torch.float32
        w = {
            "f0": z(B, N, C, dtype=f), "tA": z(B, N, C, dtype=f), "tB": z(B, N, C, dtype=f), "tC": z(B, N, C, dtype=f),
            "hA": (z(B, N, C, dtype=torch.float16) if self.t16 else None),
            "hB": (z(B, N, C, dtype=torch.float16) if self.t16 else None), "hC": (z(B, N, C, dtype=torch.float16) if self.t16 else None),
            "n": z(B, N, _r8(C)), "n2b": z(B, N, _r8(C)), "c1": z(B, N, _r8(mid)), "c2": z(B, N, _r8(C)), "m2": z(B, N, ops.ffn_m_ld(C)),
            "y16": z(B, N, yw), "n16": z(B, N, 16), "u": z(B, N, _r8(max(hid2, 2 * C))), "g": z(B, N, _r8(max(hid2 // 2, 2 * C))),
            "q": z(B, N, _r8(C)), "kv": z(B, N, _r8(2 * C)), "ao": z(B, N, _r8(C)),
            "fb": z(B, N, 64),
            "gap": z(B, max(ops.layernorm_blocks(), -(-H // 4) * -(-W // 16)), yw, dtype=f),
            "scale": z(B, 256, dtype=f), "eca_tmp": z(B, 32, 256, dtype=f),
        }
        if any(G.ocab.qkvf is not None for G in self.layers):
            w["qkv"] = z(B, N, 432)
        w["weff"] = z(B, yw, max(self._kpad, 64))
        if any(G.ocab.esc is not None for G in self.layers):
            w["yesc"] = z(B, N, _r8(C))
        if self.focus:
            w["fh"], w["sal"] = z(B, N, _r8(C // 4)), z(B, N, 8, dtype=f)
        if self.focus or self.topk < 1.0:
            w["kb"] = z(B, (H // self.ws) * (W // self.ws), -(-(self.wse * self.wse) // 16) * 16, dtype=f)
        if hab0 is not None:
            cab2 = hab0.cab2
            tiles = ops.conv3x3_small_groups(cab2, B, H, W, self.dtype) if cab2.frag else ops.conv_tiles(cab2, H, W, self.dtype)
            w["tiles"] = tiles
            w["colsum"] = z(B, tiles, cab2.npad, dtype=f)
        if hab0 is not None and hab0.fold is not None:
            cab0 = hab0.cab0
            w["sweep"] = "sq" in hab0.fold and W % 16 == 0 and cab0.npad == 16
            w["tiles1"] = ops.cab_squeeze_units(H, W) if w["sweep"] else ops.conv_tiles(cab0, H, W, self.dtype)
            w["colsum1"] = z(B, w["tiles1"], cab0.npad, dtype=f)
            w["wf"] = z(B, hab0.esc.aggr.nt * 3 * 512)
            w["bias_b"] = z(B, hab0.esc.aggr.npad, dtype=f)
        if tag is not None:
            w["gstat_l"], w["gstat_g"] = z(B, yw, dtype=f), z(B, yw, dtype=f)
            w["cstat_l"], w["cstat_g"] = z(B, 72, dtype=f), z(B, 72, dtype=f)
            w["estat_l"], w["estat_g"] = z(B, 256, dtype=f), z(B, 256, dtype=f)
            w["rs_tmp"], w["rs_cnt"] = z(B, 64, 256, dtype=f), torch.zeros(B, dtype=torch.int32, device=dev)
        if self.naf is not None:
            c = self.naf.c
            w["naf_sA"], w["naf_sB"], w["naf_gA"], w["naf_gB"] = z(B, N, c, dtype=f), z(B, N, c, dtype=f), z(B, N, c), z(B, N, c)
            w["naf_part"], w["naf_wf"], w["naf_bf"] = z(B, ops.naf_tiles(H, W), c, dtype=f), z(B, c * c), z(B, c, dtype=f)
            w["x_naf"] = z(B, self.cfg["in_chans"], H, W, dtype=f)
        h, wd = H, W
        w["ups"] = []
        for _, r in self.ups:
            h, wd = h * r, wd * r
            w["ups"].append(z(B, h * wd, 64))
        w["bytes"] = sum(t.numel() * t.element_size() for v in w.values() for t in (v if isinstance(v, list) else [v])
                         if isinstance(t, torch.Tensor))
        self._ws_cache[key] = w
        self.ws_allocations += 1
        while len(self._ws_cache) > 1 and (len(self._ws_cache) > self._ws_max
                                           or sum(v["bytes"] for v in self._ws_cache.values()) > self._ws_max_bytes):
            self._ws_cache.popitem(last=False)
        return w

    def _esc_w(self, esc: _ESC, w, B, H, W, nblk, gap=None):
        ops.esc_weights(w["gap"] if gap is None else gap, nblk, H * W, esc.w1, esc.b1, esc.w2, esc.b2, esc.plk, w["weff"], B=B,
                        pdim=esc.pdim, ksize=esc.ksize, kpad=esc.kpad, dtype=self.dtype)

    def _esc_conv(self, esc: _ESC, w, n, B, H, W, n16=None):
        if esc.conv13:
            src, ldx = (n16, 16) if n16 is not None else (n, _r8(self.C))
# ... 331 lines not shown
            else:
                f.pooled(w["n"], f.ldc, esc.pdim, gst[0])
        if hb.fold is not None:
            yield from self._prologue_fold(f, hb, gst)
        else:
            yield from self._prologue_plain(f, hb, gst)

    def _squeeze_chain(self, f: _Fwd, hb: _Hab):
        w, fo = f.w, hb.fold
        if w["sweep"]:
            ops.cab_squeeze(w["n"], fo["sq"][0], fo["sq"][1], w["c1"], w["colsum1"], B=f.B, H=f.H, W=f.W, C_=self.C, ldx=f.ldc, dtype=f.dt)
        else:
            ops.conv(hb.cab0, w["n"], w["c1"], **f.geo, ldx=f.ldc, ldo=8, act=ACT_GELU, n_store=8, colsum=w["colsum1"])
        if f.band is None:
            ops.cab_fold(w["c1"], w["colsum1"], w["tiles1"], hb.cab0.npad, fo["w2"], fo["b2"], hb.eca_w, hb.eca_w.numel(),
                         fo["ba"], float(self.cfg["conv_scale"]), w["scale"], w["wf"], w["bias_b"], w["eca_tmp"], B=f.B, H=f.H,
                         W=f.W, C_=self.C, mid=hb.cab0.nout, dtype=f.dt, w2f=fo["w2f"])

    def _prologue_fold(self, f: _Fwd, hb: _Hab, gst):
        w, esc, B, H, W = f.w, hb.esc, f.B, f.H, f.W
        n16 = w["n16"] if f.have_n16 else None
        s0 = torch.cuda.current_stream(self.dev)
        s1 = self._side_stream(f)
        if f.band is not None:
            yield from self._fold_band(f, hb, gst)
            self._esc_w(esc, w, B, f.band.Hfull, W, 1, gap=gst[1])
            self._esc_conv(esc, w, w["n"], B, H, W, n16=n16)
        elif self.opt.esc_side:
            self._esc_w(esc, w, B, H, W, f.nblk)
            s1.wait_stream(s0)
            with torch.cuda.stream(s1):
                self._esc_conv(esc, w, w["n"], B, H, W, n16=n16)
            self._squeeze_chain(f, hb)
        else:
            s1.wait_stream(s0)
            with torch.cuda.stream(s1):
                self._squeeze_chain(f, hb)
            self._esc_w(esc, w, B, H, W, f.nblk)
            self._esc_conv(esc, w, w["n"], B, H, W, n16=n16)
        s0.wait_stream(s1)

    def _fold_band(self, f: _Fwd, hb: _Hab, gst):
        w, bd, W, fo = f.w, f.band, f.W, hb.fold
        self._squeeze_chain(f, hb)
        st, c1, lo, own = w["cstat_l"], w["c1"], bd.lo, bd.own
        f.pooled(c1, 8, 8, st, 0)
        f.pooled(c1, 8, 8, st, 24, c0=0, c1=1)
        f.pooled(c1, 8, 8, st, 32, c0=W - 1, c1=W)
        if bd.r0 == 0:
            f.pooled(c1, 8, 8, st, 8, r0=lo, r1=lo + 1)
            f.pooled(c1, 8, 8, st, 40, r0=lo, r1=lo + 1, c0=0, c1=1)
            f.pooled(c1, 8, 8, st, 48, r0=lo, r1=lo + 1, c0=W - 1, c1=W)
        if bd.r1 == bd.Hfull:
            f.pooled(c1, 8, 8, st, 16, r0=lo + own - 1, r1=lo + own)
            f.pooled(c1, 8, 8, st, 56, r0=lo + own - 1, r1=lo + own, c0=0, c1=1)
            f.pooled(c1, 8, 8, st, 64, r0=lo + own - 1, r1=lo + own, c0=W - 1, c1=W)
        yield ("reduce", [(gst[0], gst[1], hb.esc.pdim), (st, w["cstat_g"], 72)])
        ops.cab_fold(None, None, 1, hb.cab0.npad, fo["w2"], fo["b2"], hb.eca_w, hb.eca_w.numel(), fo["ba"],
                     float(self.cfg["conv_scale"]), w["scale"], w["wf"], w["bias_b"], None, B=f.B, H=bd.Hfull, W=W, C_=self.C,
                     mid=hb.cab0.nout, dtype=f.dt, stats=w["cstat_g"], w2f=fo["w2f"])

    def _prologue_plain(self, f: _Fwd, hb: _Hab, gst):
        w, esc, bd, B, H, W, C, ldc = f.w, hb.esc, f.band, f.B, f.H, f.W, self.C, f.ldc
        mid = hb.cab0.nout
        c3 = ops.conv3x3_small if hb.cab0.frag else ops.conv
        c3(hb.cab0, w["n"], w["c1"], **f.geo, ldx=ldc, ldo=_r8(mid), act=ACT_GELU, n_store=_r4(mid))
        c3 = ops.conv3x3_small if hb.cab2.frag else ops.conv
        c3(hb.cab2, w["c1"], w["c2"], **f.geo, ldx=_r8(mid), ldo=ldc, colsum=w["colsum"])
        if bd is None:
            ops.eca_scale(w["colsum"], w["tiles"], hb.cab2.npad, f.N, hb.eca_w, hb.eca_w.numel(),
                          float(self.cfg["conv_scale"]), w["eca_tmp"], w["scale"], B=B, C_=C)
            self._esc_lk(esc, w, w["n"], B, H, W, f.nblk)
            return
        npd = hb.cab2.npad
        el, eg = (w[k].view(-1)[:B * npd].view(B, npd) for k in ("estat_l", "estat_g"))
        f.pooled(w["c2"], ldc, C, el)
        yield ("reduce", [(gst[0], gst[1], esc.pdim), (el, eg, _r4(C))])
        ops.eca_scale(eg, 1, npd, bd.Hfull * W, hb.eca_w, hb.eca_w.numel(), float(self.cfg["conv_scale"]), w["eca_tmp"],
                      w["scale"], B=B, C_=C)
        self._esc_w(esc, w, B, bd.Hfull, W, 1, gap=gst[1])
        self._esc_conv(esc, w, w["n"], B, H, W)

    def _tail_fused144(self, f: _Fwd, hb: _Hab):
        w, t = f.w, f.t
        if hb.out16:
            tout = w["hB"] if t is not w["hB"] else w["hC"]
        else:
            tout = w["tB"] if t is not w["tB"] else w["tC"]
        nxt, gap_c = hb.next_ln
        ops.hab_tail(hb.ffn3 if hb.ffn3 is not None else hb.ffn, hb.esc.aggr, t, tout, hb.n2[0], hb.n2[1], n=w["n"], ldn_in=f.ldc,
                     y16=w["y16"], c1=w["c1"], wf=w["wf"], bias_b=w["bias_b"], B=f.B, H=f.H, W=f.W, dtype=f.dt, ln1=nxt,
                     n_out=w["n2b"], ldn=f.ldc, gap_out=w["gap"], gap_c=gap_c, n16_out=(w["n16"] if self.use_n16 else None))
        w["n"], w["n2b"] = w["n2b"], w["n"]
        if self.opt.emu_t16 is not None:
            tout.copy_(tout.to(self.opt.emu_t16).to(torch.float32))
        f.t, f.have_n, f.have_n16, f.nblk = tout, True, self.use_n16, ops.ffn_tiles(hb.ffn, f.H, f.W, f.dt)

    def _tail_fused180(self, f: _Fwd, hb: _Hab):
        w, t = f.w, f.t
        tout = w["tB"] if t is not w["tB"] else w["tC"]
        nxt, gap_c = hb.next_ln
        ops.hab_tail(hb.ffn3, hb.esc.aggr, t, tout, hb.n2[0], hb.n2[1], n=w["n"], ldn_in=f.ldc, y16=w["y16"], bias_b=hb.bias256,
                     B=f.B, H=f.H, W=f.W, dtype=f.dt, ln1=nxt, n_out=w["n2b"], ldn=f.ldc, gap_out=w["gap"], gap_c=gap_c,
                     n16_out=(w["n16"] if self.use_n16 else None), r2=w["c2"], ldr2=f.ldc, r2scale=w["scale"],
                     r2scale_bstride=hb.cab2.npad)
        w["n"], w["n2b"] = w["n2b"], w["n"]
        f.t, f.have_n, f.have_n16, f.nblk = tout, True, self.use_n16, -(-f.H // 8) * -(-f.W // 16)

    def _tail_aggr_cab(self, f: _Fwd, hb: _Hab):
        w = f.w
        ops.aggr_cab(hb.esc.aggr, w["n"], w["tB"], w["c1"], w["wf"], w["bias_b"], **f.geo, ldx=f.ldc, ldo=self.C, x0=w["y16"],
                     c_split=hb.esc.pdim, ldx0=w["y16"].shape[2], r1=f.t, ldr1=self.C)
        self._ffn(f, hb)

    def _tail_aggr(self, f: _Fwd, hb: _Hab):
        w = f.w
        self._run_lin(hb.esc.aggr, w["n"], w["tB"], **f.geo, ldx=f.ldc, ldo=self.C, out_mode=O_NHWC_F32, x0=w["y16"],
                      c_split=hb.esc.pdim, ldx0=w["y16"].shape[2], r1=f.t, ldr1=self.C, r2=w["c2"], ldr2=f.ldc,
                      r2scale=w["scale"], r2scale_bstride=hb.cab2.npad)
        self._ffn(f, hb)

    def _ffn(self, f: _Fwd, hb: _Hab):
        w, C, ldc = f.w, self.C, f.ldc
        tB, tC = w["tB"], w["tC"]
        if hb.ffn is not None:
# ... 154 lines not shown
```

super_resolution_amd/ops.py:

```python
from __future__ import annotations

import collections
import ctypes as C
from typing import Optional

import torch

from . import _lib
from ._lib import (ACT_GELU, ACT_LRELU, ACT_LRELU02, ACT_NONE, HAT_BF16, HAT_F32, O_NCHW_F32, O_NHWC_F32, O_NHWC_T, O_PIXSHUF_T,
                   X_NCHW_F32_MEAN, X_NHWC_F32, X_NHWC_T, HatAggrCabDesc, HatCabFoldDesc, HatConvDesc, HatFfnDesc, HatHabTailDesc, HatMlpDesc, HatNafFoldDesc,
                   HatNafHalfDesc, HatEscConvFfnDesc)
from .packing import (ESC_HID_PAD, FP16_SAFE, KC, NAF_WIDTHS, TORCH_DTYPE, PackedConv, PackedEscFfn, PackedFFN, PackedMlp, PackedNafBlock, choose_nt,
                      esc_geo_ensemble, pack_esc_convffn, PackedEscRealSkip, dysample_fold, pack_escreal_skip, pack_nearest_conv,
                      choose_nt_linear, naf_ffn_fold, naf_frags, pack_naf_block,
                      ffn_fp16_range_bound, pack_cab_squeeze, pack_cab_w2f, pack_conv_weight, pack_ffn, pack_ffn2, pack_ffn3,
                      pack_linear_weight, pack_ocab_mlp, pack_ocab_qkv, pack_pointwise)

DTYPE_CODE = {"f32": HAT_F32, "fp32": HAT_F32, "float32": HAT_F32, "bf16": HAT_BF16, "bfloat16": HAT_BF16}


def _ptr(t: Optional[torch.Tensor]) -> Optional[int]:
    if t is None:
        return None
    if not t.is_cuda:
        raise RuntimeError("HAT HIP ops need device tensors (no CPU path exists)")
    if not t.is_contiguous():
        raise RuntimeError("HAT HIP ops need contiguous tensors")
    return t.data_ptr()


def _stream() -> int:
    return torch.cuda.current_stream().cuda_stream


_prof = None


class profile:

    def __enter__(self):
        global _prof
        _prof = []
        return _prof

    def __exit__(self, *exc):
        global _prof
        _prof = None
        return False
# ... 92 lines not shown
    lib = _lib.load()
    cb = n if c_bstride is None else c_bstride
    _timed("add_f32_kernel", 0.0, lambda: _lib.check(lib.hat_add_f32(_ptr(a), _ptr(c), _ptr(out), B, n, cb, _stream()), "hat_add_f32"))


def rect_sum(x: torch.Tensor, out: torch.Tensor, tmp: torch.Tensor, counter: torch.Tensor, *, B: int, W: int, ld: int, C_: int, r0: int,
             r1: int, c0: int = 0, c1: Optional[int] = None, out_off: int = 0, dtype: Optional[int] = None):
    lib = _lib.load()
    dt = dtype if dtype is not None else (HAT_BF16 if x.dtype == torch.bfloat16 else HAT_F32)
    o = out.view(B, -1)
    bstride = x.numel() // B
    _timed("rect_sum_kernel", 0.0, lambda: _lib.check(
        lib.hat_rect_sum(_ptr(x), dt, ld, C_, W, r0, r1, c0, (W if c1 is None else c1), bstride, B, o.data_ptr() + 4 * out_off, o.shape[1],
                         _ptr(tmp), _ptr(counter), _stream()), "hat_rect_sum"))


def esc_weights(gap: torch.Tensor, nblk: int, npix: int, w1, b1, w2, b2, plk_packed, w_out, *, B: int, pdim: int,
                ksize: int, kpad: int, dtype: int):
    lib = _lib.load()
    _timed("esc_weights_kernel", 0.0, lambda: _lib.check(
        lib.hat_esc_weights(_ptr(gap), nblk, npix, _ptr(w1), _ptr(b1), _ptr(w2), _ptr(b2), _ptr(plk_packed), _ptr(w_out), B,
                            pdim, ksize, kpad, dtype, _stream()), "hat_esc_weights"))


def esc_conv13_supported(pdim: int, ksize: int, dtype: int) -> bool:
    return pdim == 16 and ksize == 13 and dtype == HAT_BF16


def esc_conv13(x, wp, y16, *, B: int, H: int, W: int, ldx: int, kpad: int, dtype: int):
    lib = _lib.load()
    _timed("esc13_kernel", 2.0 * B * H * W * 169 * 256 + 2.0 * 9 * 16 * B * H * W, lambda: _lib.check(
        lib.hat_esc_conv13(_ptr(x), ldx, _ptr(wp), kpad, _ptr(y16), B, H, W, dtype, _stream()), "hat_esc_conv13"),
        tag=f"k13 16->16 {H}x{W} resident")


def eca_scale(colsum, tiles: int, ldc: int, npix: int, wk, k: int, conv_scale: float, tmp, scale, *, B: int, C_: int):
    lib = _lib.load()
    _timed("eca_reduce+scale", 0.0, lambda: _lib.check(
        lib.hat_eca_scale(_ptr(colsum), tiles, ldc, npix, _ptr(wk), k, conv_scale, _ptr(tmp), _ptr(scale), B, C_, _stream()),
        "hat_eca_scale"))


def dwconv_gate(u, wdw, bdw, out, *, B: int, H: int, W: int, hid: int, ldu: int, ldo: int, dtype: int):
    lib = _lib.load()
    _timed(f"dwgate_kernel<{_TNAME[dtype]}>", 2.0 * 9 * 2 * hid * B * H * W, lambda: _lib.check(
        lib.hat_dwconv_gate(_ptr(u), _ptr(wdw), _ptr(bdw), _ptr(out), B, H, W, hid, ldu, ldo, dtype, _stream()),
        "hat_dwconv_gate"))


def ocab_keybias(sal, kv, kb, *, B: int, H: int, W: int, C_: int, ws: int, wse: int, pad: int, k_keep: int, ldsal: int, ldkv: int,
                 dtype: int):
    lib = _lib.load()
    _timed("keybias_kernel", 0.0, lambda: _lib.check(
        lib.hat_ocab_keybias(_ptr(sal), ldsal, _ptr(kv), ldkv, _ptr(kb), B, H, W, C_, ws, wse, pad, k_keep, dtype, _stream()), "hat_ocab_keybias"))


def ocab_attention_kb(q, kv, bias_rot, kb, out, *, B: int, H: int, W: int, C_: int, heads: int, ws: int, wse: int, pad: int, ldq: int,
                      ldkv: int, ldo: int, dtype: int):
    lib = _lib.load()
    _timed(f"ocab_attn_kernel<{_TNAME[dtype]}, kb>", 2.0 * 2 * wse * wse * C_ * B * H * W, lambda: _lib.check(
        lib.hat_ocab_attention_kb(_ptr(q), _ptr(kv), _ptr(bias_rot), _ptr(kb), _ptr(out), B, H, W, C_, heads, ws, wse, pad, ldq, ldkv, ldo,
                                  dtype, _stream()), "hat_ocab_attention_kb"))


def ocab_mlp_supported(C_: int, hidden: int, dtype: int) -> bool:
    return C_ == 144 and hidden == 288 and dtype == HAT_BF16
# ... 663 lines not shown
        d.m_in, d.ldm_in = _ptr(m_in), ldm_in
    d.w1f, d.b1, d.dww, d.dwb, d.w2f, d.b2 = _ptr(pf.w1f), _ptr(pf.b1), _ptr(pf.dww), _ptr(pf.dwb), _ptr(pf.w2f), _ptr(pf.b2)
    if ln1 is not None:
        d.ln1_g, d.ln1_b, d.n_out, d.ldn = _ptr(ln1[0]), _ptr(ln1[1]), _ptr(n_out), ldn
        d.gap_out, d.gap_c = (_ptr(gap_out) if gap_c else None), gap_c
        d.n16_out = _ptr(n16_out)


def ffn(pf: PackedFFN, t_in, t_out, ln_g, ln_b, *, B: int, H: int, W: int, dtype: int, ln1=None, n_out=None, ldn: int = 0,
        gap_out=None, gap_c: int = 0, m_in=None, ldm_in: int = 0):
    lib = _lib.load()
    d = _ffn_desc(pf, B, H, W, dtype)
    _fill_ffn(d, pf, t_in, t_out, ln_g, ln_b, ln1, n_out, ldn, gap_out, gap_c, m_in, ldm_in)
    flops = B * H * W * (2.0 * pf.C * 2 * pf.hid + 2.0 * 9 * 2 * pf.hid + 2.0 * pf.hid * pf.C)
    es = 2 if dtype == HAT_BF16 else 4
    nbytes = B * H * W * (4.0 * pf.C + 4.0 * pf.C + (es * ldn if ln1 is not None else 0) + (es * ldm_in if m_in is not None else 0))
    if pf.layout == "tail3":
        raise RuntimeError("a hat_hab_tail3-packed FFN has no stand-alone launch: pack with pack_ffn2 for hat_ffn2")
    if pf.layout == "ffn2":
        _timed("ffn2_kernel", flops, lambda: _lib.check(lib.hat_ffn2(C.byref(d), _stream()), "hat_ffn2"), nbytes=nbytes)
        return
    _timed(f"ffn_kernel<{_TNAME[dtype]}>", flops, lambda: _lib.check(lib.hat_ffn(C.byref(d), _stream()), "hat_ffn"),
           nbytes=nbytes)


def hab_tail_supported(pf: PackedFFN, aggr: PackedConv, mid: int, dtype: int) -> bool:
    if pf.C == 180:
        return pf.layout == "tail3" and aggr.frag and aggr.nt == 12 and aggr.n_slices == 1 and aggr.kpad == 192 and dtype == HAT_BF16
    return pf.layout in ("ffn2", "tail3") and aggr.frag and aggr.nt == 9 and aggr.n_slices == 1 and aggr.kpad == 160 and mid <= 8 and dtype == HAT_BF16


def hab_tail(pf: PackedFFN, aggr: PackedConv, t_in, t_out, ln_g, ln_b, *, n, ldn_in: int, y16, c1=None, wf=None, bias_b, B: int, H: int,
             W: int, dtype: int, ln1=None, n_out=None, ldn: int = 0, gap_out=None, gap_c: int = 0, n16_out=None,
             r2=None, ldr2: int = 0, r2scale=None, r2scale_bstride: int = 0):
    lib = _lib.load()
    h = HatHabTailDesc()
    d = h.ffn
    d.B, d.H, d.W, d.C, d.chunks, d.dtype = B, H, W, pf.C, pf.chunks, dtype
    _fill_ffn(d, pf, t_in, t_out, ln_g, ln_b, ln1, n_out, ldn, gap_out, gap_c, n16_out=n16_out)
    h.n, h.y16, h.c1, h.w_aggr, h.wf, h.bias_b, h.ldn_in = _ptr(n), _ptr(y16), _ptr(c1), _ptr(aggr.w), _ptr(wf), _ptr(bias_b), ldn_in
    h.r2, h.ldr2, h.r2scale, h.r2scale_bstride = _ptr(r2), ldr2, _ptr(r2scale), r2scale_bstride
    in_half, out_half = t_in.dtype == torch.float16, t_out.dtype == torch.float16
    if (in_half or out_half) and not (pf.C == 144 and pf.layout == "tail3"):
        raise RuntimeError("an FP16 residual stream is only instantiated for hat_hab_tail3 at embed_dim 144")
    if (not in_half and t_in.dtype != torch.float32) or (not out_half and t_out.dtype != torch.float32):
        raise RuntimeError("hab_tail: t_in / t_out must be fp32 or FP16 rows")
    h.reserved1 = (1 if in_half else 0) | (2 if out_half else 0)
    if pf.C == 180:
        flops = B * H * W * (2.0 * pf.C * pf.C + 2.0 * pf.C * 2 * pf.hid + 2.0 * 9 * 2 * pf.hid + 2.0 * pf.hid * pf.C)
        nbytes = B * H * W * (2.0 * ldn_in + 32 + 2.0 * ldr2 + 4.0 * pf.C + 4.0 * pf.C + (2 * ldn if ln1 is not None else 0))
        _timed("tail3l_kernel", flops, lambda: _lib.check(lib.hat_hab_tail3(C.byref(h), _stream()), "hat_hab_tail3"), nbytes=nbytes)
        return
    flops = B * H * W * (2.0 * pf.C * (pf.C + 72) + 2.0 * pf.C * 2 * pf.hid + 2.0 * 9 * 2 * pf.hid + 2.0 * pf.hid * pf.C)
    nbytes = B * H * W * (2.0 * ldn_in + 32 + 16 + (2.0 if in_half else 4.0) * pf.C + (2.0 if out_half else 4.0) * pf.C + (2 * ldn if ln1 is not None else 0))
    if pf.layout == "tail3":
        _timed("tail3_kernel", flops, lambda: _lib.check(lib.hat_hab_tail3(C.byref(h), _stream()), "hat_hab_tail3"), nbytes=nbytes)
        return
    _timed("ffn2_kernel<aggr>", flops, lambda: _lib.check(lib.hat_hab_tail(C.byref(h), _stream()), "hat_hab_tail"), nbytes=nbytes)


_PW_SHAPES = {(9, 5), (18, 5), (9, 9), (12, 6), (23, 6), (12, 12), (4, 1), (4, 2)}


def linear_supported(nout: int, cin: int, dtype: int) -> bool:
    nt, _ = choose_nt_linear(nout, cin, dtype)
    ks = -(-cin // 32)
    lds = nt * ks * 64 * 8 * (2 if dtype == HAT_BF16 else 4)
    return (nt, ks) in _PW_SHAPES and lds <= 163840 and cin % 4 == 0


def linear(pw: PackedConv, x: torch.Tensor, out: torch.Tensor, *, B: int, H: int, W: int, dtype: int, ldx: int, ldo: int,
           out_mode: int = O_NHWC_T, act: int = ACT_NONE, n_store: Optional[int] = None, x0: Optional[torch.Tensor] = None,
           c_split: int = 0, ldx0: int = 0, r1: Optional[torch.Tensor] = None, ldr1: int = 0, r2: Optional[torch.Tensor] = None,
           ldr2: int = 0, r2scale: Optional[torch.Tensor] = None, r2scale_bstride: int = 0, ln=None,
           ln_out: Optional[torch.Tensor] = None, ld_ln: int = 0, ln_ones: bool = False):
    lib = _lib.load()
    d = HatConvDesc()
    d.x, d.x0, d.w, d.bias, d.out = _ptr(x), _ptr(x0), _ptr(pw.w), _ptr(pw.bias), _ptr(out)
    d.r1, d.r2, d.r2scale = _ptr(r1), _ptr(r2), _ptr(r2scale)
    if ln is not None:
        d.ln_g, d.ln_b, d.ln_out, d.ld_ln, d.ln_ones = _ptr(ln[0]), _ptr(ln[1]), _ptr(ln_out), ld_ln, int(ln_ones)
    d.B, d.H, d.W, d.Cin, d.ldx, d.x_mode = B, H, W, pw.cin, ldx, X_NHWC_T
    d.c_split, d.ldx0, d.ksize, d.Kpad, d.nt, d.n_slices = c_split, ldx0, 1, pw.kpad, pw.nt, pw.n_slices
    d.n_store = pw.nout if n_store is None else n_store
    d.ldo, d.out_mode, d.act, d.ldr1, d.ldr2, d.r2scale_bstride, d.dtype = ldo, out_mode, act, ldr1, ldr2, r2scale_bstride, dtype
    d.reserved0 = _stream16(r1, out, out_mode)
    flops = 2.0 * B * H * W * pw.cin * pw.nout
# ... 17 lines not shown
    d.B, d.H, d.W, d.Cin, d.ldx, d.x_mode = B, H, W, pw.cin, ldx, X_NHWC_T
    d.ksize, d.Kpad, d.nt, d.n_slices, d.dtype = 3, pw.kpad, pw.nt, 1, dtype
    return d


def conv3x3_small_groups(pw: PackedConv, B: int, H: int, W: int, dtype: int) -> int:
    lib = _lib.load()
    d = _c3_desc(pw, B, H, W, dtype, 8)
    n = C.c_int32(0)
    _lib.check(lib.hat_conv3x3_small_groups(C.byref(d), C.byref(n)), "hat_conv3x3_small_groups")
    return n.value


def conv3x3_small(pw: PackedConv, x, out, *, B: int, H: int, W: int, dtype: int, ldx: int, ldo: int, act: int = ACT_NONE,
                  n_store: Optional[int] = None, out_mode: int = O_NHWC_T, colsum=None):
    lib = _lib.load()
    d = _c3_desc(pw, B, H, W, dtype, ldx)
    d.x, d.w, d.bias, d.out, d.colsum = _ptr(x), _ptr(pw.w), _ptr(pw.bias), _ptr(out), _ptr(colsum)
    d.n_store = pw.nout if n_store is None else n_store
    d.ldo, d.out_mode, d.act = ldo, out_mode, act
    flops = 2.0 * B * H * W * 9 * pw.cin * pw.nout
    _timed(f"tap3_kernel<{_TNAME[dtype]}, {pw.nt}>", flops,
           lambda: _lib.check(lib.hat_conv3x3_small(C.byref(d), _stream()), f"hat_conv3x3_small(Cin={pw.cin}, N={pw.nout})"),
           tag=f"c3s {pw.cin}->{pw.nout} {H}x{W}")


def aggr_cab_supported(C_: int, mid: int, dtype: int) -> bool:
    return C_ == 144 and mid <= 8 and dtype == HAT_BF16


def cab_fold(c1, c1_colsum, tiles: int, ldcs: int, w2, b2, wk, k: int, bias_in, conv_scale: float, scale, wf, bias_out, tmp, *,
             B: int, H: int, W: int, C_: int, mid: int, dtype: int, stats=None, w2f=None):
    lib = _lib.load()
    d = HatCabFoldDesc()
    d.stats = _ptr(stats)
    d.w2f = _ptr(w2f)
    d.c1, d.c1_colsum, d.w2, d.b2, d.wk, d.bias_in = _ptr(c1), _ptr(c1_colsum), _ptr(w2), _ptr(b2), _ptr(wk), _ptr(bias_in)
    d.scale, d.wf, d.bias_out, d.tmp = _ptr(scale), _ptr(wf), _ptr(bias_out), _ptr(tmp)
    d.B, d.H, d.W, d.C, d.mid, d.ld1, d.tiles, d.ldcs, d.k, d.ld_scale, d.dtype = B, H, W, C_, mid, 8, tiles, ldcs, k, scale.shape[1], dtype
    d.conv_scale = conv_scale
    _timed("cab_fold", 0.0, lambda: _lib.check(lib.hat_cab_fold(C.byref(d), _stream()), "hat_cab_fold"))


def aggr_cab(pw: PackedConv, x, out, c1, wf, bias_b, *, B: int, H: int, W: int, dtype: int, ldx: int, ldo: int, x0=None,
             c_split: int = 0, ldx0: int = 0, r1=None, ldr1: int = 0):
    lib = _lib.load()
    dd = HatAggrCabDesc()
    d = dd.lin
    d.x, d.x0, d.w, d.bias, d.out, d.r1 = _ptr(x), _ptr(x0), _ptr(pw.w), _ptr(pw.bias), _ptr(out), _ptr(r1)
    d.B, d.H, d.W, d.Cin, d.ldx, d.x_mode = B, H, W, pw.cin, ldx, X_NHWC_T
    d.c_split, d.ldx0, d.ksize, d.Kpad, d.nt, d.n_slices, d.n_store = c_split, ldx0, 1, pw.kpad, pw.nt, pw.n_slices, pw.nout
    d.ldo, d.out_mode, d.act, d.ldr1, d.dtype = ldo, O_NHWC_F32, ACT_NONE, ldr1, dtype
    dd.c1, dd.wf, dd.bias_b = _ptr(c1), _ptr(wf), _ptr(bias_b)
    flops = 2.0 * B * H * W * pw.nout * (pw.cin + 9 * 8)
    _timed("aggr_cab_kernel", flops, lambda: _lib.check(lib.hat_aggr_cab(C.byref(dd), _stream()), "hat_aggr_cab"),
           tag=f"aggr+cab {pw.cin}+72->{pw.nout} {H}x{W}")
```

super_resolution_amd/packing.py:

```python
from __future__ import annotations

from typing import Optional

import torch

from ._lib import HAT_BF16, HAT_F32

TORCH_DTYPE = {HAT_F32: torch.float32, HAT_BF16: torch.bfloat16}
KC = {HAT_F32: 32, HAT_BF16: 64}


class PackedConv:
    __slots__ = ("w", "bias", "ksize", "cin", "kpad", "nt", "n_slices", "nout", "w_bstride", "frag", "ksplit")

    def __init__(self, w, bias, ksize, cin, kpad, nt, n_slices, nout, w_bstride=0, frag=False):
        self.w, self.bias, self.ksize, self.cin, self.kpad = w, bias, ksize, cin, kpad
        self.nt, self.n_slices, self.nout, self.w_bstride = nt, n_slices, nout, w_bstride
        self.frag = frag
        self.ksplit = None

    @property
    def npad(self):
        return self.nt * 16 * self.n_slices

# ... 118 lines not shown
def pack_ocab_qkv(q_w, q_b, kv_w, kv_b, qscale: float, device) -> PackedMlp:
    Wq, Wkv = _f32(q_w) * qscale, _f32(kv_w)
    bq = (torch.zeros(Wq.shape[0]) if q_b is None else _f32(q_b)) * qscale
    bkv = torch.zeros(Wkv.shape[0]) if kv_b is None else _f32(kv_b)
    W = torch.cat([Wq, Wkv], 0)
    assert W.shape == (432, 144)
    p = PackedMlp()
    p.w1f = _pack_fc1_frags(W).to(torch.bfloat16).contiguous().to(device)
    p.b1 = torch.cat([bq, bkv]).contiguous().to(device)
    p.w2f = p.b2 = None
    p.C, p.hidden = 144, 432
    return p


def pack_cab_squeeze(weight: torch.Tensor, bias: torch.Tensor, device):
    w = _f32(weight)
    mid, cin = w.shape[0], w.shape[1]
    A = torch.zeros(6, 16, 32 * -(-cin // 32))
    for kx in range(3):
        A[2 * kx, 0:mid, :cin] = w[:, :, 0, kx]
        A[2 * kx, 8:8 + mid, :cin] = w[:, :, 1, kx]
        A[2 * kx + 1, 0:mid, :cin] = w[:, :, 2, kx]
    return frags(A.reshape(96, -1)).to(torch.bfloat16).contiguous().to(device), _pad(_f32(bias), 8).to(device)


def pack_cab_w2f(w2: torch.Tensor, device) -> torch.Tensor:
    w = _f32(w2)
    C_, mid = w.shape[0], w.shape[1]
    full = torch.zeros(-(-C_ // 16) * 16, 12, 8)
    full[:C_, :9, :mid] = w.reshape(C_, mid, 9).permute(0, 2, 1)
    return frags(full.reshape(-1, 96)).contiguous().to(device)


FP16_SAFE = 6.0e4


def ffn_fp16_range_bound(fc1_w, fc1_b, dw_w, dw_b, ln_g, ln_b) -> float:
    f = lambda t: t.detach().to(torch.float64).cpu()
    W1, b1, Wd, bd, g_, b_ = f(fc1_w), f(fc1_b), f(dw_w).reshape(-1, 9), f(dw_b), f(ln_g), f(ln_b)
    C_ = W1.shape[1]
    hid = W1.shape[0] // 2
    U = (C_ ** 0.5) * (W1 * g_[None, :]).norm(dim=1) + (W1 @ b_ + b1).abs()
    A = Wd.abs().sum(1) * U + bd.abs()
    return float(max(U.max(), A.max(), (A[:hid] * A[hid:]).max()))


def _halves(m: torch.Tensor, hid_p: int) -> torch.Tensor:
    hid = m.shape[0] // 2
    return torch.cat([_pad(m[:hid], hid_p), _pad(m[hid:], hid_p)])


def _ffn_rows(chunks: int, unit_order: bool) -> torch.Tensor:
    nl = torch.arange(64)
    q = 8 * ((nl & 15) >> 2) + 4 * ((nl >> 4) & 1) + (nl & 3) if unit_order else nl & 31
    return (nl >> 5)[None, :] * (32 * chunks) + torch.arange(chunks)[:, None] * 32 + q[None, :]


def _ffn_fc1(W1, b1, chunks: int, ks: int, unit_order: bool) -> torch.Tensor:
    M = _pad(_halves(W1, 32 * chunks), 64 * chunks, 32 * ks)
    if b1 is not None:
        M[:, W1.shape[1]] = _halves(b1, 32 * chunks)
    return frags(M[_ffn_rows(chunks, unit_order).reshape(-1)]).reshape(chunks, 4, ks, 64, 8)


def _ffn_fc2(W2, nt: int, chunks: int, order: str) -> torch.Tensor:
    return frags(_pad(W2, 16 * nt, 32 * chunks), order).permute(1, 0, 2, 3)
# ... 175 lines not shown
```

super_resolution_amd/plan.py:

```python
from __future__ import annotations

import argparse
import bisect
import ctypes as C
import struct
import threading
from typing import List, Tuple

import torch

from . import _lib

FN_IDS = ["hat_conv", "hat_linear", "hat_conv3x3_small", "hat_cab_fold", "hat_aggr_cab", "hat_ffn", "hat_ffn2", "hat_hab_tail",
          "hat_layernorm", "hat_esc_weights", "hat_eca_scale", "hat_dwconv_gate", "hat_sgfn_gate", "hat_ocab_attention",
          "hat_window_attention", "hat_cab_squeeze", "hat_conv3x3_to_planes", "hat_add_f32", "hat_esc_conv13", "hat_ocab_keybias", "hat_ocab_attention_kb", "hat_ocab_mlp", "hat_ocab_qkv", "hat_hab_tail3", "hat_ocab_attention_log2", "hat_naf_half",
          "hat_naf_fold"]
ARG_INT, ARG_FLOAT, ARG_PTR, ARG_STRUCT, ARG_HOST, ARG_STREAM = range(6)
BUF_CONST, BUF_SCRATCH, BUF_INPUT, BUF_OUTPUT = range(4)
NULL_BUF = 0xFFFFFFFF
_EXPORT_LOCK = threading.Lock()


class _Recorder:

    def __init__(self, lib):
        self._lib, self.calls = lib, []
        self._tid = threading.get_ident()

    def __getattr__(self, name):
        fn = getattr(self._lib, name)
        if name not in FN_IDS:
            return fn

        def call(*args):
            if threading.get_ident() == self._tid:
                self.calls.append((name, [_snapshot(a) for a in args]))
            return fn(*args)
        return call


def _snapshot(a):
    obj = getattr(a, "_obj", None)
    if isinstance(obj, C.Structure):
        return ("struct", type(obj), bytes(memoryview(obj)))
    if isinstance(a, C.Array):
        return ("host", bytes(memoryview(a)))
    return a


# ... 233 lines not shown
```

Baseline: 347.8 MP/s.

## Fuse CAB fold into squeeze and ESC dynamic-kernel weights into tail and conv13

Adds a cab_squeeze_fold kernel that runs the CAB fold in whichever block finishes last for each sample, using an atomic ticket counter, so a separate fold launch is no longer needed. It also splits ESC weight generation so only the 3x3 dynamic-kernel delta is computed: either in an epilogue of tail3 (tail3_dk) or in a small esc_dk kernel. The conv13 kernel then loads pre-packed static plk fragments and patches the center taps with plk_ctr+dk in LDS, rather than reading per-sample packed weights. The aim is fewer launches and less weight-packing traffic, at the cost of last-block serialization and added counter state.

New measurement: 348.1 MP/s, median of 2. Within noise of the previous version (+0.1%).

```diff
diff --git a/include/hat_mi355x.h b/include/hat_mi355x.h
--- a/include/hat_mi355x.h
+++ b/include/hat_mi355x.h
@@ -77,6 +77,8 @@
     const float* w2f;
 } HatCabFoldDesc;
 int hat_cab_fold(const HatCabFoldDesc* d, void* stream);
+int hat_cab_squeeze_fold(const void* x, const void* wpk, const float* bias, void* out, float* colsum, const HatCabFoldDesc* fold,
+                         uint32_t* counter, int32_t B, int32_t H, int32_t W, int32_t C, int32_t ldx, int32_t dtype, void* stream);
 
 typedef struct HatAggrCabDesc {
     HatConvDesc lin;
@@ -99,6 +101,10 @@
 
 int hat_esc_conv13(const void* x, int32_t ldx, const void* wp, int32_t Kpad, void* y16, int32_t B, int32_t H, int32_t W,
                    int32_t dtype, void* stream);
+int hat_esc_conv13_dk(const void* x, int32_t ldx, const void* wfrag, const float* plk_ctr, const float* dk, void* y16, int32_t B,
+                      int32_t H, int32_t W, int32_t dtype, void* stream);
+int hat_esc_dk(const float* gap_partial, int32_t nblk, int64_t npix, const float* w1, const float* b1, const float* w2,
+               const float* b2, float* dk_out, int32_t B, int32_t pdim, void* stream);
 
 int hat_eca_scale(const float* colsum, int32_t tiles, int32_t ldc, int64_t npix, const float* wk, int32_t k,
                   float conv_scale, float* tmp, float* scale, int32_t B, int32_t C, void* stream);
@@ -261,6 +267,13 @@
 int hat_hab_tail(const HatHabTailDesc* d, void* stream);
 
 int hat_hab_tail3(const HatHabTailDesc* d, void* stream);
+typedef struct HatEscDkDesc {
+    const float* w1; const float* b1; const float* w2; const float* b2;
+    float* dk_out;
+    uint32_t* counter;
+    int32_t pdim;
+} HatEscDkDesc;
+int hat_hab_tail3_dk(const HatHabTailDesc* d, const HatEscDkDesc* e, void* stream);
 
 typedef struct hat_plan hat_plan;
 int hat_plan_load(const char* path, hat_plan** out);
diff --git a/super_resolution_amd/_lib.py b/super_resolution_amd/_lib.py
--- a/super_resolution_amd/_lib.py
+++ b/super_resolution_amd/_lib.py
@@ -77,6 +77,11 @@
         ("tiles", C.c_int32), ("ldcs", C.c_int32), ("k", C.c_int32), ("ld_scale", C.c_int32), ("dtype", C.c_int32),
         ("conv_scale", C.c_float), ("stats", C.c_void_p), ("w2f", C.c_void_p),
     ]
+
+
+class HatEscDkDesc(C.Structure):
+    _fields_ = [("w1", C.c_void_p), ("b1", C.c_void_p), ("w2", C.c_void_p), ("b2", C.c_void_p), ("dk_out", C.c_void_p),
+                ("counter", C.c_void_p), ("pdim", C.c_int32)]
 
 
 class HatAggrCabDesc(C.Structure):
@@ -133,6 +138,13 @@
     "hat_ffn2": (C.c_int, [C.POINTER(HatFfnDesc), C.c_void_p]),
     "hat_hab_tail": (C.c_int, [C.POINTER(HatHabTailDesc), C.c_void_p]),
     "hat_hab_tail3": (C.c_int, [C.POINTER(HatHabTailDesc), C.c_void_p]),
+    "hat_hab_tail3_dk": (C.c_int, [C.POINTER(HatHabTailDesc), C.POINTER(HatEscDkDesc), C.c_void_p]),
+    "hat_esc_dk": (C.c_int, [C.c_void_p, C.c_int32, C.c_int64, C.c_void_p, C.c_void_p, C.c_void_p, C.c_void_p, C.c_void_p, C.c_int32,
+                             C.c_int32, C.c_void_p]),
+    "hat_esc_conv13_dk": (C.c_int, [C.c_void_p, C.c_int32, C.c_void_p, C.c_void_p, C.c_void_p, C.c_void_p, C.c_int32, C.c_int32, C.c_int32,
+                                    C.c_int32, C.c_void_p]),
+    "hat_cab_squeeze_fold": (C.c_int, [C.c_void_p, C.c_void_p, C.c_void_p, C.c_void_p, C.c_void_p, C.POINTER(HatCabFoldDesc), C.c_void_p,
+                                       C.c_int32, C.c_int32, C.c_int32, C.c_int32, C.c_int32, C.c_int32, C.c_void_p]),
     "hat_plan_load": (C.c_int, [C.c_char_p, C.POINTER(C.c_void_p)]),
     "hat_plan_info": (C.c_int, [C.c_void_p, C.POINTER(C.c_int32), C.POINTER(C.c_int64), C.POINTER(C.c_int64)]),
     "hat_plan_forward": (C.c_int, [C.c_void_p, C.c_void_p, C.c_void_p, C.c_void_p]),
diff --git a/super_resolution_amd/build.py b/super_resolution_amd/build.py
--- a/super_resolution_amd/build.py
+++ b/super_resolution_amd/build.py
@@ -9,7 +9,7 @@
 CSRC = os.path.join(HERE, "csrc")
 LIB = os.path.join(HERE, "libhat_mi355x.so")
 SOURCES = ["hat_conv.hip", "hat_conv64r.hip", "hat_attn.hip", "hat_misc.hip", "hat_ffn.hip", "hat_ffn2.hip", "hat_tail3.hip", "hat_tail3l.hip", "hat_pw.hip", "hat_mlp.hip", "hat_cabsq.hip", "hat_esc13.hip", "hat_u8.hip", "hat_yuv.hip", "hat_resize.hip", "hat_metrics.hip", "hat_dihedral.hip", "hat_niqe.hip", "hat_naf.hip", "hat_esc.hip", "hat_escreal.hip", "hat_plan.cpp"]
-HEADERS = [os.path.join(CSRC, "hat_common.h"), os.path.join(CSRC, "hat_yuv_check.h"), os.path.join(os.path.dirname(HERE), "include", "hat_mi355x.h")]
+HEADERS = [os.path.join(CSRC, "hat_common.h"), os.path.join(CSRC, "hat_yuv_check.h"), os.path.join(CSRC, "hat_prologue.h"), os.path.join(os.path.dirname(HERE), "include", "hat_mi355x.h")]
 FLAGS = ["-O3", "--offload-arch=gfx950", "-fPIC", "-std=c++17", "-Wall", "-Wno-unused-function"]
 
 
diff --git a/super_resolution_amd/csrc/hat_cabsq.hip b/super_resolution_amd/csrc/hat_cabsq.hip
--- a/super_resolution_amd/csrc/hat_cabsq.hip
+++ b/super_resolution_amd/csrc/hat_cabsq.hip
@@ -2,6 +2,7 @@
 #include <type_traits>
 
 #include "hat_common.h"
+#include "hat_prologue.h"
 #include "hat_yuv_check.h"
 
 __device__ __attribute__((aligned(16))) unsigned hat_cabsq_zero_page[80] = {};
@@ -29,10 +30,10 @@
 };
 
 template <int KS, bool NCHW, typename Epi = SweepEpi>
-__global__ __launch_bounds__(256, KS > 2 ? 2 : 3) void cab_squeeze_kernel(const bf16_t* __restrict__ x, const bf16_t* __restrict__ wpk,
-                                                             const float* __restrict__ bias, void* __restrict__ outv,
-                                                             float* __restrict__ colsum, int H, int W, int C, int ldx,
-                                                             int rows, int strips, int units, Epi epi) {
+__device__ __forceinline__ void cab_squeeze_wave(const bf16_t* __restrict__ x, const bf16_t* __restrict__ wpk,
+                                                 const float* __restrict__ bias, void* __restrict__ outv,
+                                                 float* __restrict__ colsum, int H, int W, int C, int ldx,
+                                                 int rows, int strips, int units, Epi epi) {
     constexpr bool U8 = std::is_same<Epi, SweepEpiU8>::value;
     using YT = SweepYuvTraits<Epi>;
     constexpr bool YUV16 = YT::deep, YUV = YT::yuv;
@@ -206,6 +207,32 @@
     }
 }
 
+template <int KS, bool NCHW, typename Epi = SweepEpi>
+__global__ __launch_bounds__(256, KS > 2 ? 2 : 3) void cab_squeeze_kernel(const bf16_t* __restrict__ x, const bf16_t* __restrict__ wpk,
+                                                             const float* __restrict__ bias, void* __restrict__ outv,
+                                                             float* __restrict__ colsum, int H, int W, int C, int ldx,
+                                                             int rows, int strips, int units, Epi epi) {
+    cab_squeeze_wave<KS, NCHW, Epi>(x, wpk, bias, outv, colsum, H, W, C, ldx, rows, strips, units, epi);
+}
+
+__global__ __launch_bounds__(256, 2) void cab_squeeze_fold_kernel(const bf16_t* x, const bf16_t* wpk, const float* bias, void* outv,
+                                                                  float* colsum, int H, int W, int C, int ldx, int rows, int strips,
+                                                                  int units, const HatCabFoldDesc fd, unsigned* counter) {
+    __shared__ unsigned last;
+    cab_squeeze_wave<5, false>(x, wpk, bias, outv, colsum, H, W, C, ldx, rows, strips, units, SweepEpi{1.0f, {0.f, 0.f, 0.f, 0.f}, 8});
+    asm volatile("s_waitcnt vmcnt(0)" ::: "memory");
+    __syncthreads();
+    if (threadIdx.x == 0) {
+        __builtin_amdgcn_fence(__ATOMIC_RELEASE, "agent");
+        asm volatile("s_waitcnt vmcnt(0)" ::: "memory");
+        last = hat_last_ticket(counter + blockIdx.y, gridDim.x) ? 1u : 0u;
+    }
+    __syncthreads();
+    if (last == 0u) return;
+    hat_cab_fold_sample<bf16_t, true>(fd, blockIdx.y);
+    if (threadIdx.x == 0) __hip_atomic_store(counter + blockIdx.y, 0u, __ATOMIC_RELAXED, __HIP_MEMORY_SCOPE_AGENT);
+}
+
 }
 
 static int sweep_units(int H, int W, int slots, int* rows_out, int* units_out, bool even_rows = false) {
@@ -238,6 +265,26 @@
     HAT_LAUNCH((cab_squeeze_kernel<5, false>), dim3((units + 3) / 4, B), dim3(256), 0, reinterpret_cast<hipStream_t>(stream),
                reinterpret_cast<const bf16_t*>(x), reinterpret_cast<const bf16_t*>(wpk), bias, out, colsum, H, W, C, ldx, rows,
                (W + 13) / 14, units, SweepEpi{1.0f, {0.f, 0.f, 0.f, 0.f}, 8});
+    return hat_check_launch();
+}
+
+extern "C" int hat_cab_squeeze_fold(const void* x, const void* wpk, const float* bias, void* out, float* colsum, const HatCabFoldDesc* fold,
+                                    uint32_t* counter, int32_t B, int32_t H, int32_t W, int32_t C, int32_t ldx, int32_t dtype, void* stream) {
+    if (!x || !wpk || !bias || !out || !colsum || !fold || !counter || B < 1 || H < 2) return HAT_EINVAL;
+    if (dtype != HAT_BF16) return HAT_EUNSUPPORTED;
+    if (C % 8 || C > 160 || C <= 128 || ldx < C || ldx % 8) return HAT_EUNSUPPORTED;
+    if ((reinterpret_cast<uintptr_t>(x) | reinterpret_cast<uintptr_t>(wpk)) % 16 || reinterpret_cast<uintptr_t>(out) % 8) return HAT_EINVAL;
+    int32_t rows = 0, units = 0;
+    const int rc = hat_cab_squeeze_units(H, W, &rows, &units);
+    if (rc) return rc;
+    const HatCabFoldDesc& d = *fold;
+    if (!d.w2 || !d.b2 || !d.wk || !d.bias_in || !d.scale || !d.wf || !d.bias_out || d.stats) return HAT_EINVAL;
+    if (d.c1 != out || d.c1_colsum != colsum || d.B != B || d.H != H || d.W != W || d.C != C || d.tiles != units || d.ldcs != 16) return HAT_EINVAL;
+    if (d.mid < 1 || d.mid > 8 || d.ld1 != 8 || d.k < 1 || (d.k & 1) == 0 || d.ld_scale < d.C || d.dtype != HAT_BF16) return HAT_EINVAL;
+    if (units > 2048) return HAT_EUNSUPPORTED;
+    HAT_LAUNCH(cab_squeeze_fold_kernel, dim3((units + 3) / 4, B), dim3(256), 0, reinterpret_cast<hipStream_t>(stream),
+               reinterpret_cast<const bf16_t*>(x), reinterpret_cast<const bf16_t*>(wpk), bias, out, colsum, H, W, C, ldx, rows, (W + 13) / 14,
+               units, d, counter);
     return hat_check_launch();
 }
 
diff --git a/super_resolution_amd/csrc/hat_esc13.hip b/super_resolution_amd/csrc/hat_esc13.hip
--- a/super_resolution_amd/csrc/hat_esc13.hip
+++ b/super_resolution_amd/csrc/hat_esc13.hip
@@ -12,9 +12,10 @@
 
 __device__ __attribute__((aligned(16))) unsigned hat_esc13_zero_page[4] = {0, 0, 0, 0};
 
-template <int RW>
+template <int RW, bool STATIC = false>
 __global__ __launch_bounds__((E_TR / RW) * 64) void esc13_kernel(const bf16_t* __restrict__ x, int ldx, const bf16_t* __restrict__ wp, int Kpad,
-                                                             bf16_t* __restrict__ y16, int H, int W, int tiles_x, int ntiles) {
+                                                             bf16_t* __restrict__ y16, int H, int W, int tiles_x, int ntiles,
+                                                             const float* __restrict__ plk_ctr, const float* __restrict__ dk) {
     typedef __bf16 bf8 __attribute__((ext_vector_type(8)));
     constexpr int E_WAVES = E_TR / RW;
     extern __shared__ __attribute__((aligned(16))) char smem[];
@@ -25,7 +26,12 @@
     const int b = blockIdx.y;
     const bf16_t* xb = x + (size_t)b * H * W * ldx;
     bf16_t* yb = y16 + (size_t)b * H * W * 16;
-    {
+    if constexpr (STATIC) {
+        for (int s = wave; s < E_NFRAG; s += E_WAVES)
+            __builtin_amdgcn_global_load_lds((const __attribute__((address_space(1))) void*)(reinterpret_cast<const char*>(wp) + s * 1024 + lane * 16),
+                                             (__attribute__((address_space(3))) void*)(smem + s * 1024), 16, 0, 0);
+        if (tid < 4) *reinterpret_cast<u32x4*>(smem + E_LDS - 64 + tid * 16) = u32x4{0u, 0u, 0u, 0u};
+    } else {
         const bf16_t* wrow = wp + ((size_t)b * 16 + c16) * Kpad;
         for (int s = wave; s < E_NFRAG; s += E_WAVES) {
             const int dxp = s / 13, dy = s - 13 * dxp, dx = 2 * dxp + (g >> 1);
@@ -58,6 +64,17 @@
         }
     };
     fetch(blockIdx.x);
+    if constexpr (STATIC) {
+        float v = 0.f;
+        if (tid < 144) v = plk_ctr[tid] + dk[(size_t)b * 144 + tid];
+        asm volatile("s_waitcnt vmcnt(0)" ::: "memory");
+        __syncthreads();
+        if (tid < 144) {
+            const int co = tid / 9, t9 = tid - 9 * co, dy = 5 + t9 / 3, dx = 5 + t9 % 3;
+            const int sfr = (dx >> 1) * 13 + dy, ln = ((dx & 1) * 2 + (co >> 3)) * 16 + co;
+            *reinterpret_cast<bf16_t*>(smem + sfr * 1024 + ln * 16 + (co & 7) * 2) = to_T<bf16_t>(v);
+        }
+    }
     for (int t = blockIdx.x; t < ntiles; t += gridDim.x) {
         const int ty0 = (t / tiles_x) * E_TR, tx0 = (t - (t / tiles_x) * tiles_x) * E_TC;
 #pragma unroll
@@ -124,10 +141,8 @@
 
 }
 
-extern "C" int hat_esc_conv13(const void* x, int32_t ldx, const void* wp, int32_t Kpad, void* y16, int32_t B, int32_t H, int32_t W,
-                              int32_t dtype, void* stream) {
-    if (!x || !wp || !y16 || B < 1 || H < 1 || W < 1 || ldx < 16 || ldx % 8 || Kpad < 169 * 16 || Kpad % 8) return HAT_EINVAL;
-    if (dtype != HAT_BF16) return HAT_EUNSUPPORTED;
+static int esc13_launch(const void* x, int ldx, const void* wp, int Kpad, const float* plk_ctr, const float* dk, void* y16, int B, int H,
+                        int W, void* stream) {
     const int tiles_x = (W + E_TC - 1) / E_TC, tiles_y = (H + E_TR - 1) / E_TR, ntiles = tiles_x * tiles_y;
     int gx = 256 / (B < 2 ? 1 : (B < 4 ? 2 : 4));
     if (gx > ntiles) gx = ntiles;
@@ -136,8 +151,24 @@
         hipError_t e = hipFuncSetAttribute(reinterpret_cast<const void*>(kern), hipFuncAttributeMaxDynamicSharedMemorySize, E_LDS);
         if (e != hipSuccess) return (int)e;
         HAT_LAUNCH(kern, dim3(gx, B), dim3(waves * 64), E_LDS, reinterpret_cast<hipStream_t>(stream), reinterpret_cast<const bf16_t*>(x), ldx,
-                   reinterpret_cast<const bf16_t*>(wp), Kpad, reinterpret_cast<bf16_t*>(y16), H, W, tiles_x, ntiles);
+                   reinterpret_cast<const bf16_t*>(wp), Kpad, reinterpret_cast<bf16_t*>(y16), H, W, tiles_x, ntiles, plk_ctr, dk);
         return hat_check_launch();
     };
+    if (dk) return rw == 2 ? launch(esc13_kernel<2, true>, 16) : launch(esc13_kernel<4, true>, 8);
     return rw == 2 ? launch(esc13_kernel<2>, 16) : launch(esc13_kernel<4>, 8);
 }
+
+extern "C" int hat_esc_conv13(const void* x, int32_t ldx, const void* wp, int32_t Kpad, void* y16, int32_t B, int32_t H, int32_t W,
+                              int32_t dtype, void* stream) {
+    if (!x || !wp || !y16 || B < 1 || H < 1 || W < 1 || ldx < 16 || ldx % 8 || Kpad < 169 * 16 || Kpad % 8) return HAT_EINVAL;
+    if (dtype != HAT_BF16) return HAT_EUNSUPPORTED;
+    return esc13_launch(x, ldx, wp, Kpad, nullptr, nullptr, y16, B, H, W, stream);
+}
+
+extern "C" int hat_esc_conv13_dk(const void* x, int32_t ldx, const void* wfrag, const float* plk_ctr, const float* dk, void* y16, int32_t B,
+                                 int32_t H, int32_t W, int32_t dtype, void* stream) {
+    if (!x || !wfrag || !plk_ctr || !dk || !y16 || B < 1 || H < 1 || W < 1 || ldx < 16 || ldx % 8) return HAT_EINVAL;
+    if (reinterpret_cast<uintptr_t>(wfrag) % 16) return HAT_EINVAL;
+    if (dtype != HAT_BF16) return HAT_EUNSUPPORTED;
+    return esc13_launch(x, ldx, wfrag, 0, plk_ctr, dk, y16, B, H, W, stream);
+}
diff --git a/super_resolution_amd/csrc/hat_misc.hip b/super_resolution_amd/csrc/hat_misc.hip
--- a/super_resolution_amd/csrc/hat_misc.hip
+++ b/super_resolution_amd/csrc/hat_misc.hip
@@ -1,4 +1,5 @@
 #include "hat_common.h"
+#include "hat_prologue.h"
 
 namespace {
 
@@ -167,6 +168,14 @@
     }
 }
 
+__global__ __launch_bounds__(256) void esc_dk_kernel(const float* gap_partial, int nblk, float inv_npix, const float* __restrict__ w1,
+                                                     const float* __restrict__ b1, const float* __restrict__ w2,
+                                                     const float* __restrict__ b2, float* dk_out, int pdim) {
+    __shared__ float lds[1024 + 32 + 16];
+    const int b = blockIdx.x;
+    hat_esc_dk_sample(gap_partial + (size_t)b * nblk * 16, nblk, inv_npix, w1, b1, w2, b2, dk_out + (size_t)b * 144, pdim, lds, threadIdx.x);
+}
+
 __global__ __launch_bounds__(256) void eca_reduce_kernel(const float* __restrict__ colsum, int tiles, int ldc,
                                                          float* __restrict__ tmp) {
     __shared__ float sub[256];
@@ -218,204 +227,7 @@
 }
 
 template <typename T, bool DIRECT>
-__global__ __launch_bounds__(256) void cab_fold_kernel(const HatCabFoldDesc d) {
-    __shared__ float sm[256 * 5 + 256];
-    float* red = sm;
-    float (*part)[32] = reinterpret_cast<float (*)[32]>(sm + 256 * 5);
-    float* mean = sm;
-    float* scl = sm + 256;
-    __shared__ float bord[4][8];
-    __shared__ float S[9][8];
-    const int tid = threadIdx.x, b = blockIdx.x;
-    const int H = d.H, W = d.W, C = d.C, mid = d.mid;
-    const T* c1 = reinterpret_cast<const T*>(d.c1) + (size_t)b * H * W * d.ld1;
-    const float* st = d.stats ? d.stats + (size_t)b * 72 : nullptr;
-    if (st != nullptr) {
-        if (tid < 32) bord[tid >> 3][tid & 7] = st[8 + tid];
-        __syncthreads();
-    } else {
-        float a[4][8];
-#pragma unroll
-        for (int line = 0; line < 4; ++line)
-#pragma unroll
-            for (int c = 0; c < 8; ++c) a[line][c] = 0.f;
-        const int lmax = W > H ? W : H;
-        constexpr int BU = sizeof(T) == 2 ? 5 : 2;
-        for (int i0 = tid; i0 < lmax; i0 += 256 * BU) {
-            typename MT<T>::frag_t v[BU][4];
-#pragma unroll
-            for (int u = 0; u < BU; ++u)
-#pragma unroll
-                for (int line = 0; line < 4; ++line) {
-                    const int len = line < 2 ? W : H;
-                    const int i = min(i0 + u * 256, len - 1);
-                    const size_t pix = line == 0 ? (size_t)i : line == 1 ? (size_t)(H - 1) * W + i : line == 2 ? (size_t)i * W : (size_t)i * W + (W - 1);
-                    v[u][line] = MT<T>::load(c1 + pix * d.ld1);
-                }
-#pragma unroll
-            for (int u = 0; u < BU; ++u)
-#pragma unroll
-                for (int line = 0; line < 4; ++line) {
-                    const bool in = i0 + u * 256 < (line < 2 ? W : H);
-#pragma unroll
-                    for (int c = 0; c < 8; ++c) a[line][c] += in ? to_f(v[u][line][c]) : 0.f;
-                }
-        }
-#pragma unroll
-        for (int pass = 0; pass < 8; ++pass) {
-#pragma unroll
-            for (int k = 0; k < 4; ++k) red[tid * 5 + k] = a[pass >> 1][(pass & 1) * 4 + k];
-            __syncthreads();
-            if (tid < 32) {
-                const int v4 = tid & 3, pt = tid >> 2;
-                float sp = 0.f;
-                for (int i = 0; i < 32; ++i) sp += red[(pt * 32 + i) * 5 + v4];
-                part[pt][pass * 4 + v4] = sp;
-            }
-            __syncthreads();
-        }
-        if (tid < 32) {
-            float sp = 0.f;
-            for (int i = 0; i < 8; ++i) sp += part[i][tid];
-            bord[tid >> 3][tid & 7] = sp;
-        }
-        __syncthreads();
-    }
-    if (DIRECT && st == nullptr) {
-        const int c = tid & 7, sb = tid >> 3;
-        float a[8] = {0.f, 0.f, 0.f, 0.f, 0.f, 0.f, 0.f, 0.f};
-        for (int t = sb; t < d.tiles; t += 256) {
-#pragma unroll
-            for (int u = 0; u < 8; ++u) {
-                const int tt = t + 32 * u;
-                const float v = d.c1_colsum[((size_t)b * d.tiles + min(tt, d.tiles - 1)) * d.ldcs + c];
-                a[u] += tt < d.tiles ? v : 0.f;
-            }
-        }
-        part[c][sb] = ((a[0] + a[1]) + (a[2] + a[3])) + ((a[4] + a[5]) + (a[6] + a[7]));
-        __syncthreads();
-    }
-    if (tid < 72) {
-        const int tap = tid >> 3, c = tid & 7;
-        const int dy = tap / 3 - 1, dx = tap % 3 - 1;
-        float tot = 0.f;
-        if (st != nullptr) {
-            tot = st[c];
-        } else if constexpr (DIRECT) {
-            for (int p = 0; p < 32; ++p) tot += part[c][p];
-        } else {
-            for (int p = 0; p < 32; ++p) tot += d.tmp[((size_t)b * 32 + p) * d.ldcs + c];
-        }
-        float v = tot;
-        const int rl = dy == 1 ? 0 : dy == -1 ? 1 : -1, cl = dx == 1 ? 2 : dx == -1 ? 3 : -1;
-        if (rl >= 0) v -= bord[rl][c];
-        if (cl >= 0) v -= bord[cl][c];
-        if (rl >= 0 && cl >= 0) {
-            const size_t pix = (size_t)(rl == 0 ? 0 : H - 1) * W + (cl == 2 ? 0 : W - 1);
-            v += st != nullptr ? st[40 + (rl * 2 + (cl - 2)) * 8 + c] : to_f(c1[pix * d.ld1 + c]);
-        }
-        S[tap][c] = c < mid ? v : 0.f;
-    }
-    __syncthreads();
-    float m = 0.f;
-    {
-        const int co = tid < C ? tid : C - 1;
-        float wv[72];
-        if (d.w2f != nullptr) {
-            const f32x4* wf4 = reinterpret_cast<const f32x4*>(d.w2f) + (size_t)(co >> 4) * (3 * 64 * 2);
-            f32x4 w8[9][2];
-#pragma unroll
-            for (int tap = 0; tap < 9; ++tap) {
-                const int e = ((tap >> 2) * 64 + (tap & 3) * 16 + (co & 15)) * 2;
-                w8[tap][0] = wf4[e];
-                w8[tap][1] = wf4[e + 1];
-            }
-#pragma unroll
-            for (int q = 0; q < 72; ++q) { const int ci = q / 9, tap = q - ci * 9; wv[q] = w8[tap][ci >> 2][ci & 3]; }
-        } else {
-#pragma unroll
-            for (int q = 0; q < 72; ++q) wv[q] = d.w2[(size_t)co * mid * 9 + min(q, mid * 9 - 1)];
-        }
-        const float bb = d.b2[co];
-#pragma unroll
-        for (int q = 0; q < 72; ++q) {
-            const int ci = q / 9, tap = q - ci * 9;
-            if (q < mid * 9) m += wv[q] * S[tap][ci < 8 ? ci : 7];
-        }
-        m = tid < C ? m / ((float)H * (float)W) + bb : 0.f;
-    }
-    mean[tid] = m;
-    __syncthreads();
-    float sc = 0.f;
-    if (tid < C) {
-        float e = 0.f;
-        for (int j = 0; j < d.k; ++j) {
-            const int cc = tid + j - d.k / 2;
-            if (cc >= 0 && cc < C) e += d.wk[j] * mean[cc];
-        }
-        sc = d.conv_scale / (1.0f + expf(-e));
-        d.scale[(size_t)b * d.ld_scale + tid] = sc;
-    }
-    scl[tid] = sc;
-    __syncthreads();
-    const int nt = (C + 15) / 16;
-    for (int n = tid; n < nt * 16; n += 256) d.bias_out[(size_t)b * nt * 16 + n] = n < C ? d.bias_in[n] + scl[n] * d.b2[n] : 0.f;
-    T* wf = reinterpret_cast<T*>(d.wf) + (size_t)b * nt * 3 * 512;
-    if (d.w2f != nullptr) {
-        constexpr int MAXS = 16;
-        const int total4 = nt * 3 * 128;
-        for (int base = 0; base < total4; base += 256 * MAXS) {
-        f32x4 wq[MAXS];
-#pragma unroll
-        for (int st = 0; st < MAXS; ++st) wq[st] = reinterpret_cast<const f32x4*>(d.w2f)[min(base + tid + st * 256, total4 - 1)];
-#pragma unroll
-        for (int st = 0; st < MAXS; ++st) {
-            const int i4 = base + tid + st * 256;
-            if (i4 < total4) {
-                const int i = 4 * i4, j = i & 7, lane = (i >> 3) & 63, ks = (i >> 9) % 3, t = i / (3 * 512);
-                const int co = t * 16 + (lane & 15), tap = 4 * ks + (lane >> 4);
-                const int cov = min(co, C - 1);
-                const float sv = scl[cov];
-                f32x4 v = wq[st] * f32x4{sv, sv, sv, sv};
-                if (co < C && tap == 9 && j == 0) {
-                    const float bfull = d.bias_in[cov] + sv * d.b2[cov];
-                    v[0] = bfull;
-                    v[1] = bfull - to_f(to_T<T>(bfull));
-                }
-                Vec4<T>::store(wf + i, v);
-            }
-        }
-        }
-        return;
-    }
-    constexpr int FU = 18;
-    for (int i0 = tid; i0 < nt * 3 * 512; i0 += 256 * FU) {
-        float wv[FU], bi[FU], b2v[FU];
-        bool ok[FU];
-        int cov[FU], bsel[FU];
-#pragma unroll
-        for (int u = 0; u < FU; ++u) {
-            const int i = min(i0 + u * 256, nt * 3 * 512 - 1);
-            const int j = i & 7, lane = (i >> 3) & 63, ks = (i >> 9) % 3, t = i / (3 * 512);
-            const int co = t * 16 + (lane & 15), k = 32 * ks + 8 * (lane >> 4) + j;
-            const int tap = k >> 3, ci = k & 7;
-            ok[u] = co < C && tap < 9 && ci < mid;
-            bsel[u] = (co < C && tap == 9 && ci < 2) ? 1 + ci : 0;
-            cov[u] = min(co, C - 1);
-            wv[u] = d.w2[((size_t)cov[u] * mid + min(ci, mid - 1)) * 9 + min(tap, 8)];
-            bi[u] = d.bias_in[cov[u]];
-            b2v[u] = d.b2[cov[u]];
-        }
-#pragma unroll
-        for (int u = 0; u < FU; ++u) {
-            const int i = i0 + u * 256;
-            const float bfull = bi[u] + scl[cov[u]] * b2v[u];
-            const float bhead = to_f(to_T<T>(bfull));
-            const float v = bsel[u] == 1 ? bfull : (bsel[u] == 2 ? bfull - bhead : (ok[u] ? scl[cov[u]] * wv[u] : 0.f));
-            if (i < nt * 3 * 512) wf[i] = to_T<T>(v);
-        }
-    }
-}
+__global__ __launch_bounds__(256) void cab_fold_kernel(const HatCabFoldDesc d) { hat_cab_fold_sample<T, DIRECT>(d, blockIdx.x); }
 
 template <typename T>
 __global__ __launch_bounds__(256) void dwgate_kernel(const T* __restrict__ u, const float* __restrict__ wdw,
@@ -516,6 +328,15 @@
                            reinterpret_cast<float*>(w_out), pdim, ksize, Kpad);
     else
         return HAT_EINVAL;
+    return hat_check_launch();
+}
+
+extern "C" int hat_esc_dk(const float* gap_partial, int32_t nblk, int64_t npix, const float* w1, const float* b1, const float* w2,
+                          const float* b2, float* dk_out, int32_t B, int32_t pdim, void* stream) {
+    if (!gap_partial || !w1 || !b1 || !w2 || !b2 || !dk_out || B < 1 || nblk < 1 || npix < 1) return HAT_EINVAL;
+    if (pdim != 16) return HAT_EUNSUPPORTED;
+    HAT_LAUNCH(esc_dk_kernel, dim3(B), dim3(256), 0, reinterpret_cast<hipStream_t>(stream), gap_partial, nblk, 1.0f / (float)npix, w1, b1,
+               w2, b2, dk_out, pdim);
     return hat_check_launch();
 }
 
diff --git a/super_resolution_amd/csrc/hat_plan.cpp b/super_resolution_amd/csrc/hat_plan.cpp
--- a/super_resolution_amd/csrc/hat_plan.cpp
+++ b/super_resolution_amd/csrc/hat_plan.cpp
@@ -51,7 +51,7 @@
 const char* const FN_NAMES[] = {"hat_conv", "hat_linear", "hat_conv3x3_small", "hat_cab_fold", "hat_aggr_cab", "hat_ffn", "hat_ffn2",
                                 "hat_hab_tail", "hat_layernorm", "hat_esc_weights", "hat_eca_scale", "hat_dwconv_gate", "hat_sgfn_gate",
                                 "hat_ocab_attention", "hat_window_attention", "hat_cab_squeeze", "hat_conv3x3_to_planes", "hat_add_f32", "hat_esc_conv13", "hat_ocab_keybias", "hat_ocab_attention_kb", "hat_ocab_mlp", "hat_ocab_qkv", "hat_hab_tail3", "hat_ocab_attention_log2", "hat_naf_half",
-                                "hat_naf_fold"};
+                                "hat_naf_fold", "hat_hab_tail3_dk", "hat_esc_dk", "hat_esc_conv13_dk", "hat_cab_squeeze_fold"};
 constexpr uint32_t N_FN = sizeof(FN_NAMES) / sizeof(FN_NAMES[0]);
 
 struct Resolved {
@@ -152,6 +152,19 @@
                            : HAT_EINVAL;
         case 25: return n == 2 ? hat_naf_half((const HatNafHalfDesc*)r.P(0), r.P(1)) : HAT_EINVAL;
         case 26: return n == 2 ? hat_naf_fold((const HatNafFoldDesc*)r.P(0), r.P(1)) : HAT_EINVAL;
+        case 27: return n == 3 ? hat_hab_tail3_dk((const HatHabTailDesc*)r.P(0), (const HatEscDkDesc*)r.P(1), r.P(2)) : HAT_EINVAL;
+        case 28:
+            return n == 11 ? hat_esc_dk((const float*)r.P(0), r.I(1), r.L(2), (const float*)r.P(3), (const float*)r.P(4), (const float*)r.P(5),
+                                        (const float*)r.P(6), (float*)r.P(7), r.I(8), r.I(9), r.P(10))
+                           : HAT_EINVAL;
+        case 29:
+            return n == 11 ? hat_esc_conv13_dk(r.P(0), r.I(1), r.P(2), (const float*)r.P(3), (const float*)r.P(4), r.P(5), r.I(6), r.I(7), r.I(8),
+                                               r.I(9), r.P(10))
+                           : HAT_EINVAL;
+        case 30:
+            return n == 14 ? hat_cab_squeeze_fold(r.P(0), r.P(1), (const float*)r.P(2), r.P(3), (float*)r.P(4), (const HatCabFoldDesc*)r.P(5),
+                                                  (uint32_t*)r.P(6), r.I(7), r.I(8), r.I(9), r.I(10), r.I(11), r.I(12), r.P(13))
+                           : HAT_EINVAL;
         default: return HAT_EUNSUPPORTED;
     }
 }
diff --git a/super_resolution_amd/csrc/hat_prologue.h b/super_resolution_amd/csrc/hat_prologue.h
--- /dev/null
+++ b/super_resolution_amd/csrc/hat_prologue.h
@@ -0,0 +1,272 @@
+#pragma once
+#include "hat_common.h"
+
+__device__ __forceinline__ float hat_load_agent(const float* p) {
+    return __hip_atomic_load(const_cast<float*>(p), __ATOMIC_RELAXED, __HIP_MEMORY_SCOPE_AGENT);
+}
+__device__ __forceinline__ void hat_store_agent(float* p, float v) { __hip_atomic_store(p, v, __ATOMIC_RELAXED, __HIP_MEMORY_SCOPE_AGENT); }
+
+__device__ __forceinline__ bool hat_last_ticket(unsigned* counter, unsigned total) {
+    const unsigned t = __hip_atomic_fetch_add(counter, 1u, __ATOMIC_RELAXED, __HIP_MEMORY_SCOPE_AGENT);
+    if (t != total - 1u) return false;
+    __builtin_amdgcn_fence(__ATOMIC_ACQUIRE, "agent");
+    asm volatile("s_waitcnt vmcnt(0)" ::: "memory");
+    return true;
+}
+
+__device__ __forceinline__ void hat_esc_dk_sample(const float* gp, int nblk, float inv_npix, const float* __restrict__ w1,
+                                                  const float* __restrict__ b1, const float* __restrict__ w2,
+                                                  const float* __restrict__ b2, float* dk_out, int pdim, float* lds, int tid) {
+    float* part = lds;
+    float* pmean = lds + 1024;
+    float* hid = lds + 1024 + 32;
+    constexpr int gs = 16, np = 64;
+    const int ci = tid & (gs - 1);
+#pragma unroll 1
+    for (int h = 0; h < 2; ++h) {
+        float acc[2][8];
+#pragma unroll
+        for (int q = 0; q < 2; ++q)
+#pragma unroll
+            for (int u = 0; u < 8; ++u) acc[q][u] = 0.f;
+        const int pp0 = (tid >> 4) + 32 * h;
+        for (int kb = 0; kb < nblk; kb += np * 8 * 4) {
+            float v[2][4][8];
+#pragma unroll
+            for (int q = 0; q < 2; ++q)
+#pragma unroll
+                for (int it = 0; it < 4; ++it)
+#pragma unroll
+                    for (int u = 0; u < 8; ++u)
+                        v[q][it][u] = hat_load_agent(gp + (size_t)min(kb + pp0 + 16 * q + np * (8 * it + u), nblk - 1) * gs + ci);
+#pragma unroll
+            for (int q = 0; q < 2; ++q)
+#pragma unroll
+                for (int it = 0; it < 4; ++it)
+#pragma unroll
+                    for (int u = 0; u < 8; ++u) acc[q][u] += (kb + pp0 + 16 * q + np * (8 * it + u) < nblk) ? v[q][it][u] : 0.f;
+        }
+#pragma unroll
+        for (int q = 0; q < 2; ++q)
+            part[(pp0 + 16 * q) * gs + ci] = ((acc[q][0] + acc[q][1]) + (acc[q][2] + acc[q][3])) + ((acc[q][4] + acc[q][5]) + (acc[q][6] + acc[q][7]));
+    }
+    __syncthreads();
+    if (tid < gs) {
+        float s = 0.f;
+        for (int k = 0; k < np; ++k) s += part[k * gs + tid];
+        pmean[tid] = s * inv_npix;
+    }
+    __syncthreads();
+    const int hdim = pdim / 2;
+    if (tid < hdim) {
+        float s = b1[tid];
+        for (int c = 0; c < pdim; ++c) s += w1[tid * pdim + c] * pmean[c];
+        hid[tid] = gelu_erf(s);
+    }
+    __syncthreads();
+    if (tid < pdim * 9) {
+        float s = b2[tid];
+        for (int m = 0; m < hdim; ++m) s += w2[tid * hdim + m] * hid[m];
+        dk_out[tid] = s;
+    }
+}
+
+template <typename T, bool DIRECT>
+__device__ __forceinline__ void hat_cab_fold_sample(const HatCabFoldDesc& d, const int b) {
+    __shared__ float sm[256 * 5 + 256];
+    float* red = sm;
+    float (*part)[32] = reinterpret_cast<float (*)[32]>(sm + 256 * 5);
+    float* mean = sm;
+    float* scl = sm + 256;
+    __shared__ float bord[4][8];
+    __shared__ float S[9][8];
+    const int tid = threadIdx.x;
+    const int H = d.H, W = d.W, C = d.C, mid = d.mid;
+    const T* c1 = reinterpret_cast<const T*>(d.c1) + (size_t)b * H * W * d.ld1;
+    const float* st = d.stats ? d.stats + (size_t)b * 72 : nullptr;
+    if (st != nullptr) {
+        if (tid < 32) bord[tid >> 3][tid & 7] = st[8 + tid];
+        __syncthreads();
+    } else {
+        float a[4][8];
+#pragma unroll
+        for (int line = 0; line < 4; ++line)
+#pragma unroll
+            for (int c = 0; c < 8; ++c) a[line][c] = 0.f;
+        const int lmax = W > H ? W : H;
+        constexpr int BU = sizeof(T) == 2 ? 5 : 2;
+        for (int i0 = tid; i0 < lmax; i0 += 256 * BU) {
+            typename MT<T>::frag_t v[BU][4];
+#pragma unroll
+            for (int u = 0; u < BU; ++u)
+#pragma unroll
+                for (int line = 0; line < 4; ++line) {
+                    const int len = line < 2 ? W : H;
+                    const int i = min(i0 + u * 256, len - 1);
+                    const size_t pix = line == 0 ? (size_t)i : line == 1 ? (size_t)(H - 1) * W + i : line == 2 ? (size_t)i * W : (size_t)i * W + (W - 1);
+                    v[u][line] = MT<T>::load(c1 + pix * d.ld1);
+                }
+#pragma unroll
+            for (int u = 0; u < BU; ++u)
+#pragma unroll
+                for (int line = 0; line < 4; ++line) {
+                    const bool in = i0 + u * 256 < (line < 2 ? W : H);
+#pragma unroll
+                    for (int c = 0; c < 8; ++c) a[line][c] += in ? to_f(v[u][line][c]) : 0.f;
+                }
+        }
+#pragma unroll
+        for (int pass = 0; pass < 8; ++pass) {
+#pragma unroll
+            for (int k = 0; k < 4; ++k) red[tid * 5 + k] = a[pass >> 1][(pass & 1) * 4 + k];
+            __syncthreads();
+            if (tid < 32) {
+                const int v4 = tid & 3, pt = tid >> 2;
+                float sp = 0.f;
+                for (int i = 0; i < 32; ++i) sp += red[(pt * 32 + i) * 5 + v4];
+                part[pt][pass * 4 + v4] = sp;
+            }
+            __syncthreads();
+        }
+        if (tid < 32) {
+            float sp = 0.f;
+            for (int i = 0; i < 8; ++i) sp += part[i][tid];
+            bord[tid >> 3][tid & 7] = sp;
+        }
+        __syncthreads();
+    }
+    if (DIRECT && st == nullptr) {
+        const int c = tid & 7, sb = tid >> 3;
+        float a[8] = {0.f, 0.f, 0.f, 0.f, 0.f, 0.f, 0.f, 0.f};
+        for (int t = sb; t < d.tiles; t += 256) {
+#pragma unroll
+            for (int u = 0; u < 8; ++u) {
+                const int tt = t + 32 * u;
+                const float v = d.c1_colsum[((size_t)b * d.tiles + min(tt, d.tiles - 1)) * d.ldcs + c];
+                a[u] += tt < d.tiles ? v : 0.f;
+            }
+        }
+        part[c][sb] = ((a[0] + a[1]) + (a[2] + a[3])) + ((a[4] + a[5]) + (a[6] + a[7]));
+        __syncthreads();
+    }
+    if (tid < 72) {
+        const int tap = tid >> 3, c = tid & 7;
+        const int dy = tap / 3 - 1, dx = tap % 3 - 1;
+        float tot = 0.f;
+        if (st != nullptr) {
+            tot = st[c];
+        } else if constexpr (DIRECT) {
+            for (int p = 0; p < 32; ++p) tot += part[c][p];
+        } else {
+            for (int p = 0; p < 32; ++p) tot += d.tmp[((size_t)b * 32 + p) * d.ldcs + c];
+        }
+        float v = tot;
+        const int rl = dy == 1 ? 0 : dy == -1 ? 1 : -1, cl = dx == 1 ? 2 : dx == -1 ? 3 : -1;
+        if (rl >= 0) v -= bord[rl][c];
+        if (cl >= 0) v -= bord[cl][c];
+        if (rl >= 0 && cl >= 0) {
+            const size_t pix = (size_t)(rl == 0 ? 0 : H - 1) * W + (cl == 2 ? 0 : W - 1);
+            v += st != nullptr ? st[40 + (rl * 2 + (cl - 2)) * 8 + c] : to_f(c1[pix * d.ld1 + c]);
+        }
+        S[tap][c] = c < mid ? v : 0.f;
+    }
+    __syncthreads();
+    float m = 0.f;
+    {
+        const int co = tid < C ? tid : C - 1;
+        float wv[72];
+        if (d.w2f != nullptr) {
+            const f32x4* wf4 = reinterpret_cast<const f32x4*>(d.w2f) + (size_t)(co >> 4) * (3 * 64 * 2);
+            f32x4 w8[9][2];
+#pragma unroll
+            for (int tap = 0; tap < 9; ++tap) {
+                const int e = ((tap >> 2) * 64 + (tap & 3) * 16 + (co & 15)) * 2;
+                w8[tap][0] = wf4[e];
+                w8[tap][1] = wf4[e + 1];
+            }
+#pragma unroll
+            for (int q = 0; q < 72; ++q) { const int ci = q / 9, tap = q - ci * 9; wv[q] = w8[tap][ci >> 2][ci & 3]; }
+        } else {
+#pragma unroll
+            for (int q = 0; q < 72; ++q) wv[q] = d.w2[(size_t)co * mid * 9 + min(q, mid * 9 - 1)];
+        }
+        const float bb = d.b2[co];
+#pragma unroll
+        for (int q = 0; q < 72; ++q) {
+            const int ci = q / 9, tap = q - ci * 9;
+            if (q < mid * 9) m += wv[q] * S[tap][ci < 8 ? ci : 7];
+        }
+        m = tid < C ? m / ((float)H * (float)W) + bb : 0.f;
+    }
+    mean[tid] = m;
+    __syncthreads();
+    float sc = 0.f;
+    if (tid < C) {
+        float e = 0.f;
+        for (int j = 0; j < d.k; ++j) {
+            const int cc = tid + j - d.k / 2;
+            if (cc >= 0 && cc < C) e += d.wk[j] * mean[cc];
+        }
+        sc = d.conv_scale / (1.0f + expf(-e));
+        d.scale[(size_t)b * d.ld_scale + tid] = sc;
+    }
+    scl[tid] = sc;
+    __syncthreads();
+    const int nt = (C + 15) / 16;
+    for (int n = tid; n < nt * 16; n += 256) d.bias_out[(size_t)b * nt * 16 + n] = n < C ? d.bias_in[n] + scl[n] * d.b2[n] : 0.f;
+    T* wf = reinterpret_cast<T*>(d.wf) + (size_t)b * nt * 3 * 512;
+    if (d.w2f != nullptr) {
+        constexpr int MAXS = 16;
+        const int total4 = nt * 3 * 128;
+        for (int base = 0; base < total4; base += 256 * MAXS) {
+        f32x4 wq[MAXS];
+#pragma unroll
+        for (int st = 0; st < MAXS; ++st) wq[st] = reinterpret_cast<const f32x4*>(d.w2f)[min(base + tid + st * 256, total4 - 1)];
+#pragma unroll
+        for (int st = 0; st < MAXS; ++st) {
+            const int i4 = base + tid + st * 256;
+            if (i4 < total4) {
+                const int i = 4 * i4, j = i & 7, lane = (i >> 3) & 63, ks = (i >> 9) % 3, t = i / (3 * 512);
+                const int co = t * 16 + (lane & 15), tap = 4 * ks + (lane >> 4);
+                const int cov = min(co, C - 1);
+                const float sv = scl[cov];
+                f32x4 v = wq[st] * f32x4{sv, sv, sv, sv};
+                if (co < C && tap == 9 && j == 0) {
+                    const float bfull = d.bias_in[cov] + sv * d.b2[cov];
+                    v[0] = bfull;
+                    v[1] = bfull - to_f(to_T<T>(bfull));
+                }
+                Vec4<T>::store(wf + i, v);
+            }
+        }
+        }
+        return;
+    }
+    constexpr int FU = 18;
+    for (int i0 = tid; i0 < nt * 3 * 512; i0 += 256 * FU) {
+        float wv[FU], bi[FU], b2v[FU];
+        bool ok[FU];
+        int cov[FU], bsel[FU];
+#pragma unroll
+        for (int u = 0; u < FU; ++u) {
+            const int i = min(i0 + u * 256, nt * 3 * 512 - 1);
+            const int j = i & 7, lane = (i >> 3) & 63, ks = (i >> 9) % 3, t = i / (3 * 512);
+            const int co = t * 16 + (lane & 15), k = 32 * ks + 8 * (lane >> 4) + j;
+            const int tap = k >> 3, ci = k & 7;
+            ok[u] = co < C && tap < 9 && ci < mid;
+            bsel[u] = (co < C && tap == 9 && ci < 2) ? 1 + ci : 0;
+            cov[u] = min(co, C - 1);
+            wv[u] = d.w2[((size_t)cov[u] * mid + min(ci, mid - 1)) * 9 + min(tap, 8)];
+            bi[u] = d.bias_in[cov[u]];
+            b2v[u] = d.b2[cov[u]];
+        }
+#pragma unroll
+        for (int u = 0; u < FU; ++u) {
+            const int i = i0 + u * 256;
+            const float bfull = bi[u] + scl[cov[u]] * b2v[u];
+            const float bhead = to_f(to_T<T>(bfull));
+            const float v = bsel[u] == 1 ? bfull : (bsel[u] == 2 ? bfull - bhead : (ok[u] ? scl[cov[u]] * wv[u] : 0.f));
+            if (i < nt * 3 * 512) wf[i] = to_T<T>(v);
+        }
+    }
+}
diff --git a/super_resolution_amd/csrc/hat_tail3.hip b/super_resolution_amd/csrc/hat_tail3.hip
--- a/super_resolution_amd/csrc/hat_tail3.hip
+++ b/super_resolution_amd/csrc/hat_tail3.hip
@@ -1,4 +1,5 @@
 #include "hat_common.h"
+#include "hat_prologue.h"
 
 #ifndef T3_ISSUE_ALL
 #define T3_ISSUE_ALL 0
@@ -55,11 +56,18 @@
     const float* bias_b;
     int ldn;
 };
+struct T3Dk {
+    const float* w1; const float* b1; const float* w2; const float* b2;
+    float* dk_out;
+    unsigned* counter;
+    float inv_npix;
+    int pdim;
+};
 __device__ __attribute__((aligned(16))) unsigned hat_tail3_zero_page[4] = {0, 0, 0, 0};
 __device__ __attribute__((aligned(16))) unsigned hat_tail3_ones_page[4] = {0x3F803F80u, 0, 0, 0};
 
-template <int DBG, int TH = 0>
-__global__ __launch_bounds__(256, 2) void tail3_kernel(const HatFfnDesc d, const T3Aggr ag) {
+template <int DBG, int TH = 0, bool DK = false>
+__global__ __launch_bounds__(256, 2) void tail3_kernel(const HatFfnDesc d, const T3Aggr ag, const T3Dk ek) {
     constexpr int C = T3_C, NT = T3_NT, KS = T3_KS, NPH = T3_NPH, HALO_W = T3_HW;
     extern __shared__ __attribute__((aligned(16))) char smem[];
     const unsigned lds0 = (unsigned)(uintptr_t)(lds_char*)smem;
@@ -482,7 +490,23 @@
 #pragma unroll
             for (int w = 0; w < T3_WAVES; ++w) s += red[w * 16 + tid];
             const size_t tile = (size_t)blockIdx.y * gridDim.x + blockIdx.x;
-            d.gap_out[((size_t)b * gridDim.x * gridDim.y + tile) * 16 + tid] = tid < d.gap_c ? s : 0.f;
+            float* gp = d.gap_out + ((size_t)b * gridDim.x * gridDim.y + tile) * 16 + tid;
+            if constexpr (DK) hat_store_agent(gp, tid < d.gap_c ? s : 0.f);
+            else *gp = tid < d.gap_c ? s : 0.f;
+        }
+        if constexpr (DK) {
+            unsigned* lastf = reinterpret_cast<unsigned*>(smem + T3_WD_OFF + 1024);
+            if (wave == 0) {
+                asm volatile("s_waitcnt vmcnt(0)" ::: "memory");
+                if (tid == 0) *lastf = hat_last_ticket(ek.counter + b, gridDim.x * gridDim.y) ? 1u : 0u;
+            }
+            __syncthreads();
+            if (*lastf != 0u) {
+                const int nblk = (int)(gridDim.x * gridDim.y);
+                hat_esc_dk_sample(d.gap_out + (size_t)b * nblk * 16, nblk, ek.inv_npix, ek.w1, ek.b1, ek.w2, ek.b2,
+                                  ek.dk_out + (size_t)b * 144, ek.pdim, reinterpret_cast<float*>(smem), tid);
+                if (tid == 0) __hip_atomic_store(ek.counter + b, 0u, __ATOMIC_RELAXED, __HIP_MEMORY_SCOPE_AGENT);
+            }
         }
     }
 }
@@ -492,28 +516,42 @@
 #ifndef HAT_TAIL3_NO_ENTRY
 int hat_tail3_launch_c180(const HatHabTailDesc& h, void* stream);
 
-extern "C" int hat_hab_tail3(const HatHabTailDesc* dp, void* stream) {
+static int tail3_launch(const HatHabTailDesc* dp, const HatEscDkDesc* ep, void* stream) {
     if (!dp) return HAT_EINVAL;
     const HatHabTailDesc& h = *dp;
     const HatFfnDesc& d = h.ffn;
     if (!d.t_in || !d.t_out || d.t_in == d.t_out || !d.w1f || !d.dww || !d.w2f || !d.b2) return HAT_EINVAL;
     if (d.B < 1 || d.H < 1 || d.W < 1 || d.chunks < 1 || d.m_in) return HAT_EINVAL;
     if (d.dtype != HAT_BF16) return HAT_EUNSUPPORTED;
-    if (d.C == 180) return (d.chunks == 12 && h.reserved1 == 0) ? hat_tail3_launch_c180(h, stream) : HAT_EINVAL;
+    if (d.C == 180) return ep ? HAT_EUNSUPPORTED : ((d.chunks == 12 && h.reserved1 == 0) ? hat_tail3_launch_c180(h, stream) : HAT_EINVAL);
     if (d.C != T3_C) return HAT_EUNSUPPORTED;
     if (d.ln1_g && (!d.ln1_b || !d.n_out || d.ldn < d.C || d.ldn % 4 || d.gap_c < 0 || d.gap_c > 16 || d.gap_c % 4)) return HAT_EINVAL;
     if (!h.n || !h.y16 || !h.c1 || !h.w_aggr || !h.wf || !h.bias_b || h.ldn_in < T3_C || h.ldn_in % 8) return HAT_EINVAL;
+    T3Dk ek{};
+    if (ep) {
+        if (!ep->w1 || !ep->b1 || !ep->w2 || !ep->b2 || !ep->dk_out || !ep->counter || ep->pdim != 16) return HAT_EINVAL;
+        if (!d.ln1_g || !d.gap_out || d.gap_c != 16) return HAT_EINVAL;
+        ek = T3Dk{ep->w1, ep->b1, ep->w2, ep->b2, ep->dk_out, ep->counter, 1.0f / (float)((int64_t)d.H * (int64_t)d.W), ep->pdim};
+    }
     const T3Aggr ag{reinterpret_cast<const bf16_t*>(h.n), reinterpret_cast<const bf16_t*>(h.y16), reinterpret_cast<const bf16_t*>(h.c1),
                     reinterpret_cast<const char*>(h.w_aggr), reinterpret_cast<const char*>(h.wf), h.bias_b, h.ldn_in};
     const int th = h.reserved1 & 3;
     if ((h.reserved1 & ~3) != 0) return HAT_EINVAL;
     if ((th & 1) && reinterpret_cast<uintptr_t>(d.t_in) % 8) return HAT_EINVAL;
     if ((th & 2) && reinterpret_cast<uintptr_t>(d.t_out) % 16) return HAT_EINVAL;
-    void (*kern)(const HatFfnDesc, const T3Aggr) = th == 0 ? tail3_kernel<0, 0> : th == 1 ? tail3_kernel<0, 1> : th == 2 ? tail3_kernel<0, 2> : tail3_kernel<0, 3>;
+    void (*kern)(const HatFfnDesc, const T3Aggr, const T3Dk) =
+        ep ? (th == 0 ? tail3_kernel<0, 0, true> : th == 1 ? tail3_kernel<0, 1, true> : th == 2 ? tail3_kernel<0, 2, true> : tail3_kernel<0, 3, true>)
+           : (th == 0 ? tail3_kernel<0, 0> : th == 1 ? tail3_kernel<0, 1> : th == 2 ? tail3_kernel<0, 2> : tail3_kernel<0, 3>);
     hipError_t e = hipFuncSetAttribute(reinterpret_cast<const void*>(kern), hipFuncAttributeMaxDynamicSharedMemorySize, T3_LDS);
     if (e != hipSuccess) return (int)e;
     dim3 grid((d.W + 15) / 16, (d.H + T3_ROWS - 1) / T3_ROWS, d.B);
-    HAT_LAUNCH(kern, grid, dim3(256), T3_LDS, reinterpret_cast<hipStream_t>(stream), d, ag);
+    HAT_LAUNCH(kern, grid, dim3(256), T3_LDS, reinterpret_cast<hipStream_t>(stream), d, ag, ek);
     return hat_check_launch();
 }
-#endif
+
+extern "C" int hat_hab_tail3(const HatHabTailDesc* dp, void* stream) { return tail3_launch(dp, nullptr, stream); }
+
+extern "C" int hat_hab_tail3_dk(const HatHabTailDesc* dp, const HatEscDkDesc* ep, void* stream) {
+    return ep ? tail3_launch(dp, ep, stream) : HAT_EINVAL;
+}
+#endif
diff --git a/super_resolution_amd/engine.py b/super_resolution_amd/engine.py
--- a/super_resolution_amd/engine.py
+++ b/super_resolution_amd/engine.py
@@ -36,6 +36,7 @@
     no_cab_sweep: bool = False
     no_esc13: bool = False
     esc_side: bool = False
+    prologue_fuse: bool = False
     one_stream: bool = False
     no_attn_log2: bool = False
     no_ocab_mlp: bool = False
@@ -72,6 +73,7 @@
         self.aggr = None
         self.aggr_keys = (core + ".aggr.weight", core + ".aggr.bias")
         self.conv13 = False
+        self.wfrag = self.plk_ctr = None
 
 
 class _Packed:
@@ -87,6 +89,7 @@
     fold = ffn = ffn3 = fc1 = fc2 = bias256 = None
     tail = "aggr"
     next_ln = None
+    next_esc = None
     out16 = False
 
 
@@ -116,7 +119,7 @@
         self.geo = dict(B=B, H=H, W=W, dtype=eng.dtype)
         self.w, self.band, self.one_stream = w, band, one_stream
         self.t = self.gin = w["tA"]
-        self.have_n = self.have_n16 = False
+        self.have_n = self.have_n16 = self.have_dk = False
         self.nblk = ops.layernorm_blocks()
 
     def ln(self, src, dst, gb, out_f32=False, gap_c=0):
@@ -238,6 +241,8 @@
         esc = _ESC(sd, core, plk_key, pdim, ksize, self.C, self.dtype, self.dev)
         esc.aggr = self._lin(sd, *esc.aggr_keys)
         esc.conv13 = ops.esc_conv13_supported(pdim, ksize, self.dtype) and not self.opt.no_esc13
+        if esc.conv13 and self.opt.prologue_fuse:
+            esc.wfrag, esc.plk_ctr = ops.pack_esc13_static(esc.plk, self.dev)
         return esc
 
     def _run_lin(self, pw, x, out, **kw):
@@ -393,6 +398,8 @@
                 hb.next_ln = (nh.n1, nh.esc.pdim) if nh is not None else (oc.n1, oc.esc.pdim if oc.esc is not None else 0)
                 if hb.fold is not None:
                     hb.tail = "fused144" if hb.tail144_ok and not wide else "aggr_cab"
+                    if hb.tail == "fused144" and nh is not None and nh.esc.wfrag is not None and hb.ffn3 is not None and self.use_n16:
+                        hb.next_esc = nh.esc
                 else:
                     hb.tail = "fused180" if hb.tail180_ok and hb.next_ln[1] <= 16 else "aggr"
             G.to_conv = bool(G.conv is not None and dt == ops.HAT_BF16 and _r8(C) == C and oc.mlp2.frag and not self.opt.no_bf16_conv_in)
@@ -475,6 +482,8 @@
             w["sweep"] = "sq" in hab0.fold and W % 16 == 0 and cab0.npad == 16
             w["tiles1"] = ops.cab_squeeze_units(H, W) if w["sweep"] else ops.conv_tiles(cab0, H, W, self.dtype)
             w["colsum1"] = z(B, w["tiles1"], cab0.npad, dtype=f)
+            w["dk"] = z(B, 144, dtype=f)
+            w["tickets"] = torch.zeros(2, B, dtype=torch.int32, device=dev)
             w["wf"] = z(B, hab0.esc.aggr.nt * 3 * 512)
             w["bias_b"] = z(B, hab0.esc.aggr.npad, dtype=f)
         if tag is not None:
@@ -872,13 +881,30 @@
             with torch.cuda.stream(s1):
                 self._esc_conv(esc, w, w["n"], B, H, W, n16=n16)
             self._squeeze_chain(f, hb)
+        elif self._fuse_ok(f, hb):
+            fo = hb.fold
+            s1.wait_stream(s0)
+            with torch.cuda.stream(s1):
+                ops.cab_squeeze_fold(w["n"], fo["sq"][0], fo["sq"][1], w["c1"], w["colsum1"], w["tickets"][1], w["tiles1"], fo["w2"], fo["b2"],
+                                     hb.eca_w, hb.eca_w.numel(), fo["ba"], float(self.cfg["conv_scale"]), w["scale"], w["wf"], w["bias_b"],
+                                     B=B, H=H, W=W, C_=self.C, mid=hb.cab0.nout, ldx=f.ldc, dtype=f.dt, w2f=fo["w2f"])
+            if not f.have_dk:
+                ops.esc_dk(w["gap"], f.nblk, H * W, esc.w1, esc.b1, esc.w2, esc.b2, w["dk"], B=B, pdim=esc.pdim)
+            src, ldx = (n16, 16) if n16 is not None else (w["n"], _r8(self.C))
+            ops.esc_conv13_dk(src, esc.wfrag, esc.plk_ctr, w["dk"], w["y16"], B=B, H=H, W=W, ldx=ldx, dtype=self.dtype)
         else:
             s1.wait_stream(s0)
             with torch.cuda.stream(s1):
                 self._squeeze_chain(f, hb)
             self._esc_w(esc, w, B, H, W, f.nblk)
             self._esc_conv(esc, w, w["n"], B, H, W, n16=n16)
+        f.have_dk = False
         s0.wait_stream(s1)
+
+    def _fuse_ok(self, f: _Fwd, hb: _Hab) -> bool:
+        w = f.w
+        return (f.band is None and hb.esc.wfrag is not None and hb.esc.conv13 and hb.tail == "fused144" and w.get("sweep", False)
+                and w["tiles1"] <= 2048 and hb.cab0.npad == 16)
 
     def _fold_band(self, f: _Fwd, hb: _Hab, gst):
         w, bd, W, fo = f.w, f.band, f.W, hb.fold
@@ -928,9 +954,13 @@
         else:
             tout = w["tB"] if t is not w["tB"] else w["tC"]
         nxt, gap_c = hb.next_ln
+        ne, dk = hb.next_esc, None
+        if ne is not None and f.band is None and gap_c == 16 and w.get("sweep", False) and w["tiles1"] <= 2048:
+            dk = (ne.w1, ne.b1, ne.w2, ne.b2, w["dk"], w["tickets"][0])
         ops.hab_tail(hb.ffn3 if hb.ffn3 is not None else hb.ffn, hb.esc.aggr, t, tout, hb.n2[0], hb.n2[1], n=w["n"], ldn_in=f.ldc,
                      y16=w["y16"], c1=w["c1"], wf=w["wf"], bias_b=w["bias_b"], B=f.B, H=f.H, W=f.W, dtype=f.dt, ln1=nxt,
-                     n_out=w["n2b"], ldn=f.ldc, gap_out=w["gap"], gap_c=gap_c, n16_out=(w["n16"] if self.use_n16 else None))
+                     n_out=w["n2b"], ldn=f.ldc, gap_out=w["gap"], gap_c=gap_c, n16_out=(w["n16"] if self.use_n16 else None), dk=dk)
+        f.have_dk = dk is not None
         w["n"], w["n2b"] = w["n2b"], w["n"]
         if self.opt.emu_t16 is not None:
             tout.copy_(tout.to(self.opt.emu_t16).to(torch.float32))
diff --git a/super_resolution_amd/ops.py b/super_resolution_amd/ops.py
--- a/super_resolution_amd/ops.py
+++ b/super_resolution_amd/ops.py
@@ -8,12 +8,12 @@
 
 from . import _lib
 from ._lib import (ACT_GELU, ACT_LRELU, ACT_LRELU02, ACT_NONE, HAT_BF16, HAT_F32, O_NCHW_F32, O_NHWC_F32, O_NHWC_T, O_PIXSHUF_T,
-                   X_NCHW_F32_MEAN, X_NHWC_F32, X_NHWC_T, HatAggrCabDesc, HatCabFoldDesc, HatConvDesc, HatFfnDesc, HatHabTailDesc, HatMlpDesc, HatNafFoldDesc,
+                   X_NCHW_F32_MEAN, X_NHWC_F32, X_NHWC_T, HatAggrCabDesc, HatCabFoldDesc, HatEscDkDesc, HatConvDesc, HatFfnDesc, HatHabTailDesc, HatMlpDesc, HatNafFoldDesc,
                    HatNafHalfDesc, HatEscConvFfnDesc)
 from .packing import (ESC_HID_PAD, FP16_SAFE, KC, NAF_WIDTHS, TORCH_DTYPE, PackedConv, PackedEscFfn, PackedFFN, PackedMlp, PackedNafBlock, choose_nt,
                       esc_geo_ensemble, pack_esc_convffn, PackedEscRealSkip, dysample_fold, pack_escreal_skip, pack_nearest_conv,
                       choose_nt_linear, naf_ffn_fold, naf_frags, pack_naf_block,
-                      ffn_fp16_range_bound, pack_cab_squeeze, pack_cab_w2f, pack_conv_weight, pack_ffn, pack_ffn2, pack_ffn3,
+                      ffn_fp16_range_bound, pack_cab_squeeze, pack_cab_w2f, pack_esc13_static, pack_conv_weight, pack_ffn, pack_ffn2, pack_ffn3,
                       pack_linear_weight, pack_ocab_mlp, pack_ocab_qkv, pack_pointwise)
 
 DTYPE_CODE = {"f32": HAT_F32, "fp32": HAT_F32, "float32": HAT_F32, "bf16": HAT_BF16, "bfloat16": HAT_BF16}
@@ -172,6 +172,19 @@
     _timed("esc13_kernel", 2.0 * B * H * W * 169 * 256 + 2.0 * 9 * 16 * B * H * W, lambda: _lib.check(
         lib.hat_esc_conv13(_ptr(x), ldx, _ptr(wp), kpad, _ptr(y16), B, H, W, dtype, _stream()), "hat_esc_conv13"),
         tag=f"k13 16->16 {H}x{W} resident")
+
+
+def esc_dk(gap: torch.Tensor, nblk: int, npix: int, w1, b1, w2, b2, dk_out, *, B: int, pdim: int):
+    lib = _lib.load()
+    _timed("esc_dk_kernel", 0.0, lambda: _lib.check(
+        lib.hat_esc_dk(_ptr(gap), nblk, npix, _ptr(w1), _ptr(b1), _ptr(w2), _ptr(b2), _ptr(dk_out), B, pdim, _stream()), "hat_esc_dk"))
+
+
+def esc_conv13_dk(x, wfrag, plk_ctr, dk, y16, *, B: int, H: int, W: int, ldx: int, dtype: int):
+    lib = _lib.load()
+    _timed("esc13_kernel<dk>", 2.0 * B * H * W * 169 * 256 + 2.0 * 9 * 16 * B * H * W, lambda: _lib.check(
+        lib.hat_esc_conv13_dk(_ptr(x), ldx, _ptr(wfrag), _ptr(plk_ctr), _ptr(dk), _ptr(y16), B, H, W, dtype, _stream()), "hat_esc_conv13_dk"),
+        tag=f"k13 16->16 {H}x{W} static + dk")
 
 
 def eca_scale(colsum, tiles: int, ldc: int, npix: int, wk, k: int, conv_scale: float, tmp, scale, *, B: int, C_: int):
@@ -901,7 +914,7 @@
 
 def hab_tail(pf: PackedFFN, aggr: PackedConv, t_in, t_out, ln_g, ln_b, *, n, ldn_in: int, y16, c1=None, wf=None, bias_b, B: int, H: int,
              W: int, dtype: int, ln1=None, n_out=None, ldn: int = 0, gap_out=None, gap_c: int = 0, n16_out=None,
-             r2=None, ldr2: int = 0, r2scale=None, r2scale_bstride: int = 0):
+             r2=None, ldr2: int = 0, r2scale=None, r2scale_bstride: int = 0, dk=None):
     lib = _lib.load()
     h = HatHabTailDesc()
     d = h.ffn
@@ -922,6 +935,14 @@
         return
     flops = B * H * W * (2.0 * pf.C * (pf.C + 72) + 2.0 * pf.C * 2 * pf.hid + 2.0 * 9 * 2 * pf.hid + 2.0 * pf.hid * pf.C)
     nbytes = B * H * W * (2.0 * ldn_in + 32 + 16 + (2.0 if in_half else 4.0) * pf.C + (2.0 if out_half else 4.0) * pf.C + (2 * ldn if ln1 is not None else 0))
+    if dk is not None:
+        if pf.layout != "tail3":
+            raise RuntimeError("the dk epilogue belongs to hat_hab_tail3 at embed_dim 144")
+        e = HatEscDkDesc()
+        e.w1, e.b1, e.w2, e.b2, e.dk_out, e.counter, e.pdim = _ptr(dk[0]), _ptr(dk[1]), _ptr(dk[2]), _ptr(dk[3]), _ptr(dk[4]), _ptr(dk[5]), 16
+        _timed("tail3_kernel<dk>", flops, lambda: _lib.check(lib.hat_hab_tail3_dk(C.byref(h), C.byref(e), _stream()), "hat_hab_tail3_dk"),
+               nbytes=nbytes)
+        return
     if pf.layout == "tail3":
         _timed("tail3_kernel", flops, lambda: _lib.check(lib.hat_hab_tail3(C.byref(h), _stream()), "hat_hab_tail3"), nbytes=nbytes)
         return
@@ -1005,6 +1026,13 @@
 def cab_fold(c1, c1_colsum, tiles: int, ldcs: int, w2, b2, wk, k: int, bias_in, conv_scale: float, scale, wf, bias_out, tmp, *,
              B: int, H: int, W: int, C_: int, mid: int, dtype: int, stats=None, w2f=None):
     lib = _lib.load()
+    d = _cab_fold_desc(c1, c1_colsum, tiles, ldcs, w2, b2, wk, k, bias_in, conv_scale, scale, wf, bias_out, tmp, B=B, H=H, W=W, C_=C_,
+                       mid=mid, dtype=dtype, stats=stats, w2f=w2f)
+    _timed("cab_fold", 0.0, lambda: _lib.check(lib.hat_cab_fold(C.byref(d), _stream()), "hat_cab_fold"))
+
+
+def _cab_fold_desc(c1, c1_colsum, tiles, ldcs, w2, b2, wk, k, bias_in, conv_scale, scale, wf, bias_out, tmp, *, B, H, W, C_, mid, dtype,
+                   stats=None, w2f=None):
     d = HatCabFoldDesc()
     d.stats = _ptr(stats)
     d.w2f = _ptr(w2f)
@@ -1012,7 +1040,21 @@
     d.scale, d.wf, d.bias_out, d.tmp = _ptr(scale), _ptr(wf), _ptr(bias_out), _ptr(tmp)
     d.B, d.H, d.W, d.C, d.mid, d.ld1, d.tiles, d.ldcs, d.k, d.ld_scale, d.dtype = B, H, W, C_, mid, 8, tiles, ldcs, k, scale.shape[1], dtype
     d.conv_scale = conv_scale
-    _timed("cab_fold", 0.0, lambda: _lib.check(lib.hat_cab_fold(C.byref(d), _stream()), "hat_cab_fold"))
+    return d
+
+
+def cab_squeeze_fold_supported(H: int, W: int) -> bool:
+    return W % 16 == 0 and H >= 2 and cab_squeeze_units(H, W) <= 2048
+
+
+def cab_squeeze_fold(x, wpk, bias8, out, colsum, counter, tiles: int, w2, b2, wk, k: int, bias_in, conv_scale: float, scale, wf, bias_out, *,
+                     B: int, H: int, W: int, C_: int, mid: int, ldx: int, dtype: int, w2f=None):
+    lib = _lib.load()
+    d = _cab_fold_desc(out, colsum, tiles, 16, w2, b2, wk, k, bias_in, conv_scale, scale, wf, bias_out, None, B=B, H=H, W=W, C_=C_,
+                       mid=mid, dtype=dtype, w2f=w2f)
+    _timed("cab_squeeze_fold_kernel", 2.0 * B * H * W * 9 * C_ * 6, lambda: _lib.check(
+        lib.hat_cab_squeeze_fold(_ptr(x), _ptr(wpk), _ptr(bias8), _ptr(out), _ptr(colsum), C.byref(d), _ptr(counter), B, H, W, C_, ldx, dtype,
+                                 _stream()), "hat_cab_squeeze_fold"), tag=f"k3 {C_}->8 {H}x{W} row sweep + fold")
 
 
 def aggr_cab(pw: PackedConv, x, out, c1, wf, bias_b, *, B: int, H: int, W: int, dtype: int, ldx: int, ldo: int, x0=None,
diff --git a/super_resolution_amd/packing.py b/super_resolution_amd/packing.py
--- a/super_resolution_amd/packing.py
+++ b/super_resolution_amd/packing.py
@@ -174,6 +174,16 @@
     return frags(full.reshape(-1, 96)).contiguous().to(device)
 
 
+def pack_esc13_static(plk: torch.Tensor, device):
+    p = _f32(plk)[:16, :169 * 16].reshape(16, 13, 13, 16)
+    p14 = torch.zeros(16, 13, 14, 16)
+    p14[:, :, :13] = p
+    fr = p14.reshape(16, 13, 7, 2, 2, 8).permute(2, 1, 3, 4, 0, 5)
+    co = torch.arange(16)
+    ctr = p[co, 5:8, 5:8, co]
+    return (fr.reshape(91, 64, 8).to(torch.bfloat16).contiguous().to(device), ctr.reshape(144).contiguous().to(device))
+
+
 FP16_SAFE = 6.0e4
 
 
diff --git a/super_resolution_amd/plan.py b/super_resolution_amd/plan.py
--- a/super_resolution_amd/plan.py
+++ b/super_resolution_amd/plan.py
@@ -14,7 +14,7 @@
 FN_IDS = ["hat_conv", "hat_linear", "hat_conv3x3_small", "hat_cab_fold", "hat_aggr_cab", "hat_ffn", "hat_ffn2", "hat_hab_tail",
           "hat_layernorm", "hat_esc_weights", "hat_eca_scale", "hat_dwconv_gate", "hat_sgfn_gate", "hat_ocab_attention",
           "hat_window_attention", "hat_cab_squeeze", "hat_conv3x3_to_planes", "hat_add_f32", "hat_esc_conv13", "hat_ocab_keybias", "hat_ocab_attention_kb", "hat_ocab_mlp", "hat_ocab_qkv", "hat_hab_tail3", "hat_ocab_attention_log2", "hat_naf_half",
-          "hat_naf_fold"]
+          "hat_naf_fold", "hat_hab_tail3_dk", "hat_esc_dk", "hat_esc_conv13_dk", "hat_cab_squeeze_fold"]
 ARG_INT, ARG_FLOAT, ARG_PTR, ARG_STRUCT, ARG_HOST, ARG_STREAM = range(6)
 BUF_CONST, BUF_SCRATCH, BUF_INPUT, BUF_OUTPUT = range(4)
 NULL_BUF = 0xFFFFFFFF
```
